# WangFeng18/3d-gaussian-splatting

Hardware: AMD Instinct MI355X
Metric: render_fps (higher is better)
Workload: dtype f32; 1 GPU; cfg5: 2400000 Gaussians, 1920x1080, no SH, forward render, one frame in flight, one view per GPU -- north-star target scene (geometry of BASELINE configs[3]/[4]); n_gaussians=2400000, visible=1887982, tile_pairs=6950364, width=1920, height=1080, parallelism=view-sharded x1 (no data-path collective), frames_in_flight=1

## Files before the change

3d-gaussian-splatting_amd/csrc/gs_frame.hip:

```cpp
#include <math.h>
#include <stdarg.h>
#include <string.h>

#include <mutex>
#include <new>

#include "gs_common.h"
#include "gs_frame_layout.h"
#include "raster_bwd_common.h"

static thread_local char g_err[512] = "";

void gs_set_error(const char *fmt, ...) {
    va_list ap;
    va_start(ap, fmt);
    vsnprintf(g_err, sizeof(g_err), fmt, ap);
    va_end(ap);
}

extern "C" const char *gs_last_error(void) { return g_err; }
extern "C" int gs_abi_version(void) { return GS_ABI_VERSION; }
extern "C" int gs_culling(void) { return 0; }

static int tile_bits(int n_tiles) {
// ... 459 lines not shown
    GS_HIP(hipStreamWaitEvent(s, a->done, 0));
    *prepared = true;
    return 0;
}

extern "C" size_t gs_frame_contrib_workspace_bytes(int64_t max_pairs) {
    return max_pairs < 0 ? 0 : gs_contrib_workspace_bytes(max_pairs);
}

extern "C" int gs_frame_contrib(const gs_frame *f, const gs_contrib_opts *opts, gs_contrib_row *rows, void *workspace,
                                size_t workspace_bytes, gs_stream_t stream) {
    int rc = validate(f);
    if (rc) return rc;
    if ((rc = refuse_device_pose(f, __func__))) return rc;
    GS_CHECK_ARG(f->training && f->image_padded, "gs_frame_contrib needs a training forward (image_padded kept)");
    GS_CHECK_ARG(opts != nullptr, "opts is null");
    GS_CHECK_ARG(opts->w_min > 0.f && opts->w_min <= 1.f, "w_min must lie in (0, 1]");
    GS_CHECK_ARG(opts->accumulate == 0 || opts->accumulate == 1, "accumulate must be 0 or 1");
    GS_CHECK_ARG(f->N == 0 || rows != nullptr, "rows is null");
    GS_CHECK_ARG(((uintptr_t)rows & 15) == 0, "rows must be 16-byte aligned");
    GS_CHECK_ARG(workspace && ((uintptr_t)workspace & 255) == 0 &&
                     workspace_bytes >= gs_frame_contrib_workspace_bytes(f->max_pairs),
                 "workspace null, not 256-byte aligned or too small");
    if (f->N == 0) return 0;
    hipStream_t s = (hipStream_t)stream;
    gs_frame_ws ws = gs_frame_carve(f->workspace, f->N, f->max_pairs, f->width, f->height, f->color_dim, 1);
    uint64_t *skeys, *okeys;
    uint32_t *sids;
    sorted_buffers(f, ws, &skeys, &sids, &okeys);
    bool prepared = false;
    if ((rc = peek_prepared(f, s, &prepared))) return rc;
    return gs_stage_contrib(f, ws, sids, prepared, opts->w_min, opts->accumulate, rows, workspace, s);
}

static int zero_image(size_t bytes, const float **out) {
    static std::mutex mu;
    static struct { void *p; size_t bytes; } cache[64] = {};
    int dev = 0;
    GS_HIP(hipGetDevice(&dev));
    GS_CHECK_ARG(dev >= 0 && dev < 64, "device index out of range");
    std::lock_guard<std::mutex> lock(mu);
    if (cache[dev].bytes < bytes) {
        if (cache[dev].p) GS_HIP(hipFree(cache[dev].p));
        cache[dev].p = nullptr;
        cache[dev].bytes = 0;
        void *q = nullptr;
        GS_HIP(hipMalloc(&q, bytes));
        GS_HIP(hipMemset(q, 0, bytes));
        GS_HIP(hipDeviceSynchronize());
        cache[dev].p = q;
        cache[dev].bytes = bytes;
    }
    *out = (const float *)cache[dev].p;
    return 0;
}

static int frame_backward_adam_impl(const char *entry, const gs_frame *f, const float *grad_image, const gs_adam_fused *adam,
                                    hipStream_t s) {
    const bool aux = (f->flags & GS_FRAME_AUX) != 0, pose = (f->flags & GS_FRAME_POSE_GRAD) != 0;
    if (!(f->training && f->image_padded)) {
        gs_set_error("%s: invalid argument: %s needs a training forward (image_padded kept)", entry, entry);
        return GS_E_INVALID;
    }
    if (!(adam && (aux || grad_image))) {
        gs_set_error("%s: invalid argument: null pointer", entry);
        return GS_E_INVALID;
    }
    int rc = gs_validate_adam_fused(f, adam);
    if (rc) return rc;
    if (f->N == 0) return pose ? zero_pose_grad(f, s) : 0;
    if (!grad_image && (rc = zero_image(sizeof(float) * 3 * (size_t)f->width * (size_t)f->height, &grad_image))) return rc;
    gs_frame_ws ws = gs_frame_carve(f->workspace, f->N, f->max_pairs, f->width, f->height, f->color_dim, 1);
    if ((rc = raster_backward(f, ws, grad_image, s))) return rc;
    if ((rc = gs_stage_project_backward_adam(f, ws, adam, s))) return rc;
    return pose ? gs_stage_pose_finalize(f, ws, s) : 0;
}

static int refuse_flag(const char *entry, const char *flag) {
    gs_set_error("%s: %s frames are not supported (use gs_frame_backward + an optimizer step)", entry, flag);
    return GS_E_UNSUPPORTED;
}

extern "C" int gs_frame_backward_adam(const gs_frame *f, const float *grad_image, const gs_adam_fused *adam,
                                      gs_stream_t stream) {
    int rc = validate(f);
    if (rc) return rc;
    if ((rc = refuse_device_pose(f, __func__))) return rc;
    if (f->flags & GS_FRAME_AUX) return refuse_flag(__func__, "GS_FRAME_AUX");
    if (f->flags & GS_FRAME_POSE_GRAD) return refuse_flag(__func__, "GS_FRAME_POSE_GRAD");
    return frame_backward_adam_impl(__func__, f, grad_image, adam, (hipStream_t)stream);
}

extern "C" int gs_frame_backward_adam_aux(const gs_frame *f, const float *grad_image, const gs_adam_fused *adam,
                                          gs_stream_t stream) {
    int rc = validate(f);
    if (rc) return rc;
    if ((rc = refuse_device_pose(f, __func__))) return rc;
    GS_CHECK_ARG((f->flags & GS_FRAME_AUX) != 0, "the frame is not flagged GS_FRAME_AUX (gs_frame_backward_adam takes plain frames)");
    if (f->flags & GS_FRAME_POSE_GRAD) return refuse_flag(__func__, "GS_FRAME_POSE_GRAD");
    return frame_backward_adam_impl(__func__, f, grad_image, adam, (hipStream_t)stream);
}

extern "C" int gs_frame_backward_adam_pose(const gs_frame *f, const float *grad_image, const gs_adam_fused *adam,
                                           gs_stream_t stream) {
    int rc = validate(f);
    if (rc) return rc;
    if ((rc = refuse_device_pose(f, __func__))) return rc;
    GS_CHECK_ARG((f->flags & GS_FRAME_POSE_GRAD) != 0,
                 "the frame is not flagged GS_FRAME_POSE_GRAD (gs_frame_backward_adam / _adam_aux take frames without a pose gradient)");
    if (f->color_dim != 3) return refuse_sh_pose(__func__);
    return frame_backward_adam_impl(__func__, f, grad_image, adam, (hipStream_t)stream);
}

extern "C" int gs_frame_backward_pose(const gs_frame *f, const float *grad_image, int32_t part, gs_stream_t stream) {
    int rc = validate(f);
    if (rc) return rc;
    GS_CHECK_ARG(f->training && f->image_padded, "gs_frame_backward_pose needs a training forward (image_padded kept)");
    GS_CHECK_ARG(part == 0 || part == GS_BWD_GEOMETRY, "part must be 0 or GS_BWD_GEOMETRY");
    GS_CHECK_ARG((f->flags & GS_FRAME_POSE_GRAD) != 0,
                 "the frame is not flagged GS_FRAME_POSE_GRAD (there is no other gradient this entry point writes)");
    if (f->color_dim != 3) return refuse_sh_pose(__func__);
    GS_CHECK_ARG(part == GS_BWD_GEOMETRY || grad_image, "null pointer");
    hipStream_t s = (hipStream_t)stream;
    if (f->N == 0) return zero_pose_grad(f, s);
    gs_frame_ws ws = gs_frame_carve(f->workspace, f->N, f->max_pairs, f->width, f->height, f->color_dim, 1);
    if (part == 0 && (rc = raster_backward(f, ws, grad_image, s))) return rc;
    if ((rc = gs_stage_pose_only_backward(f, ws, s))) return rc;
    return gs_stage_pose_finalize(f, ws, s);
}

extern "C" int gs_frame_backward_part(const gs_frame *f, const float *grad_image, float *grad_pos, float *grad_quat,
                                      float *grad_scale, float *grad_opa, float *grad_rgb, int32_t part,
                                      gs_stream_t stream) {
    GS_CHECK_ARG(part == GS_BWD_RASTER || part == GS_BWD_GEOMETRY || part == GS_BWD_COLOR,
                 "part must be GS_BWD_RASTER, GS_BWD_GEOMETRY or GS_BWD_COLOR");
    return frame_backward_impl(f, grad_image, grad_pos, grad_quat, grad_scale, grad_opa, grad_rgb, part,
                               (hipStream_t)stream, nullptr);
}

extern "C" int gs_frame_backward_slice(const gs_frame *f, float *grad_pos, float *grad_quat, float *grad_scale,
                                       float *grad_opa, float *grad_rgb, int32_t part, int64_t g_begin, int64_t g_end,
                                       gs_stream_t stream) {
    GS_CHECK_ARG(part == GS_BWD_GEOMETRY || part == GS_BWD_COLOR || part == (GS_BWD_GEOMETRY | GS_BWD_COLOR),
                 "part must be GS_BWD_GEOMETRY, GS_BWD_COLOR or both");
    int rc = validate(f);
    if (rc) return rc;
    if ((rc = refuse_device_pose(f, __func__))) return rc;
    if (f->flags & GS_FRAME_POSE_GRAD) {
        gs_set_error("gs_frame_backward_slice: GS_FRAME_POSE_GRAD frames are not supported (use gs_frame_backward or "
                     "gs_frame_backward_part)");
        return GS_E_UNSUPPORTED;
    }
    if (part == (GS_BWD_GEOMETRY | GS_BWD_COLOR)) {
        GS_CHECK_ARG(grad_pos && grad_quat && grad_scale && grad_opa && grad_rgb, "null pointer");
        return frame_backward_impl(f, nullptr, grad_pos, grad_quat, grad_scale, grad_opa, grad_rgb, -1,
                                   (hipStream_t)stream, nullptr, g_begin, g_end);
    }
    return frame_backward_impl(f, nullptr, grad_pos, grad_quat, grad_scale, grad_opa, grad_rgb, part,
                               (hipStream_t)stream, nullptr, g_begin, g_end);
}

extern "C" int gs_frame_backward_profile(const gs_frame *f, const float *grad_image, float *grad_pos,
                                         float *grad_quat, float *grad_scale, float *grad_opa, float *grad_rgb,
                                         float *stage_ms_host, gs_stream_t stream) {
    GS_CHECK_ARG(stage_ms_host != nullptr, "stage_ms_host is null");
    return frame_backward_impl(f, grad_image, grad_pos, grad_quat, grad_scale, grad_opa, grad_rgb, 0,
                               (hipStream_t)stream, stage_ms_host);
}

extern "C" int gs_frame_stats_async(const gs_frame *f, int64_t *stats_host, gs_stream_t stream) {
    int rc = validate(f);
    if (rc) return rc;
    GS_CHECK_ARG(stats_host != nullptr, "stats_host is null");
    gs_frame_ws ws = gs_frame_carve(f->workspace, f->N, f->max_pairs, f->width, f->height, f->color_dim, f->training);
    GS_HIP(hipMemcpyAsync(stats_host, ws.counters, sizeof(int64_t) * 4, hipMemcpyDeviceToHost, (hipStream_t)stream));
    return 0;
}

extern "C" int gs_frame_overflow_flag(const gs_frame *f, const void **device_counter) {
    int rc = validate(f);
    if (rc) return rc;
    GS_CHECK_ARG(device_counter != nullptr, "device_counter is null");
    gs_frame_ws ws = gs_frame_carve(f->workspace, f->N, f->max_pairs, f->width, f->height, f->color_dim, f->training);
    *device_counter = ws.counters + GS_CNT_OVERFLOW;
    return 0;
}

extern "C" int gs_frame_longest_list_async(const gs_frame *f, int64_t *longest_host, gs_stream_t stream) {
    int rc = validate(f);
    if (rc) return rc;
    GS_CHECK_ARG(longest_host != nullptr, "longest_host is null");
    gs_frame_ws ws = gs_frame_carve(f->workspace, f->N, f->max_pairs, f->width, f->height, f->color_dim, f->training);
    GS_HIP(hipMemcpyAsync(longest_host, ws.counters + GS_CNT_MAXLIST, sizeof(int64_t), hipMemcpyDeviceToHost,
                          (hipStream_t)stream));
    return 0;
}

extern "C" int gs_frame_stats_tagged_async(const gs_frame *f, uint32_t tag, int64_t *stats_host, gs_stream_t stream) {
    int rc = validate(f);
    if (rc) return rc;
    GS_CHECK_ARG(stats_host != nullptr, "stats_host is null");
    gs_frame_ws ws = gs_frame_carve(f->workspace, f->N, f->max_pairs, f->width, f->height, f->color_dim, f->training);
    GS_HIP(hipMemsetD32Async((hipDeviceptr_t)(ws.counters + GS_CNT_TAG), (int)tag, 2, (hipStream_t)stream));
    GS_HIP(hipMemcpyAsync(stats_host, ws.counters, sizeof(int64_t) * GS_STATS_TAGGED_N, hipMemcpyDeviceToHost,
                          (hipStream_t)stream));
    return 0;
}

extern "C" int gs_frame_cull_fallback_async(const gs_frame *f, int64_t *ran_past_host, gs_stream_t stream) {
    int rc = validate(f);
    if (rc) return rc;
    GS_CHECK_ARG(ran_past_host != nullptr, "ran_past_host is null");
    gs_frame_ws ws = gs_frame_carve(f->workspace, f->N, f->max_pairs, f->width, f->height, f->color_dim, f->training);
    GS_HIP(hipMemcpyAsync(ran_past_host, ws.counters + GS_CNT_RANPAST, sizeof(int64_t), hipMemcpyDeviceToHost,
                          (hipStream_t)stream));
    return 0;
}

extern "C" int gs_frame_is_occlusion_culled(const gs_frame *f, int32_t *culled) {
    GS_CHECK_ARG(f && culled, "null argument");
    *culled = (effective_sort_mode(f) == 2 && gs_frame_occlusion_cull(f)) ? 1 : 0;
    return 0;
}

extern "C" int gs_frame_cull_second_pass(const gs_frame *f, int32_t *enqueued) {
    GS_CHECK_ARG(f && enqueued, "null argument");
    if (int rc = refuse_cull_repeat(f)) return rc;
    *enqueued = cull_second_pass(f) ? 1 : 0;
    return 0;
}

extern "C" int gs_frame_reads_scene_pack(const gs_frame *f) {
    if (!f || f->training || f->N <= 0 || effective_sort_mode(f) != 2) return 0;
    return gs_frame_uses_strips(f) ? 1 : 0;
}

extern "C" int gs_frame_debug_tile_nproc(const gs_frame *f, const uint32_t **tile_nproc) {
    int rc = validate(f);
    if (rc) return rc;
    GS_CHECK_ARG(tile_nproc != nullptr, "tile_nproc is null");
    GS_CHECK_ARG(f->training, "the per-tile processed counts are kept by training forwards only");
    gs_frame_ws ws = gs_frame_carve(f->workspace, f->N, f->max_pairs, f->width, f->height, f->color_dim, 1);
    *tile_nproc = ws.tile_nproc;
    return 0;
}

extern "C" int gs_frame_debug_bwd_exec_rows(const gs_frame *f, const uint32_t **exec_rows, int32_t *n_slots) {
    int rc = validate(f);
    if (rc) return rc;
    GS_CHECK_ARG(exec_rows != nullptr && n_slots != nullptr, "null pointer");
    GS_CHECK_ARG(f->training, "the executed-row counters are kept by training frames only");
    gs_frame_ws ws = gs_frame_carve(f->workspace, f->N, f->max_pairs, f->width, f->height, f->color_dim, 1);
    *exec_rows = ws.bwd_exec_rows;
    *n_slots = gs_bwd_mfma_slots(f->color_dim, gs_frame_geometry(f).n_tiles, ws.max_buckets);
    return 0;
}

extern "C" int gs_frame_binning_variant(const gs_frame *f) {
    int rc = validate(f);
    if (rc) return rc < 0 ? rc : -rc;
    const int mode = effective_sort_mode(f);
    if (mode != 2) return mode;
    if (gs_frame_uses_strips(f)) return 4;
    return (f->flags & GS_FRAME_SLICE_SORT) ? 3 : 2;
}

extern "C" int gs_frame_debug_rects(const gs_frame *f, const uint32_t **rects) {
    int rc = validate(f);
    if (rc) return rc;
    GS_CHECK_ARG(rects != nullptr, "rects is null");
    gs_frame_ws ws = gs_frame_carve(f->workspace, f->N, f->max_pairs, f->width, f->height, f->color_dim, f->training);
    *rects = reinterpret_cast<const uint32_t *>(ws.rects);
    return 0;
}

extern "C" int gs_frame_debug_cull_stage(const gs_frame *f, const uint64_t **entries, const uint32_t **tags,
                                         const uint32_t **slice_entries, int32_t *slices, int64_t *cap) {
    int rc = validate(f);
    if (rc) return rc;
    GS_CHECK_ARG(entries && tags && slice_entries && slices && cap, "null pointer");
    GS_CHECK_ARG(effective_sort_mode(f) == 2 && gs_frame_occlusion_cull(f), "not an occlusion-culled frame");
    gs_frame_ws ws = gs_frame_carve(f->workspace, f->N, f->max_pairs, f->width, f->height, f->color_dim, f->training);
    gs_frame_geom G = gs_frame_geometry(f);
    const gs_strip_plan plan = gs_strip_plan_for(f->N, G.ntx, G.nty);
    *entries = ws.keys_b;
    *tags = ws.vals_b;
    *slice_entries = ws.slice_entries;
    *slices = (int32_t)plan.slices;
    *cap = gs_cull_stage_cap(f->max_pairs, plan.slices);
    return 0;
}

extern "C" int gs_frame_debug_cut_table(const gs_frame *f, const uint32_t **cut, int32_t *n_tiles) {
    int rc = validate(f);
    if (rc) return rc;
    GS_CHECK_ARG(cut && n_tiles, "null pointer");
    GS_CHECK_ARG(!f->training, "the cut table is written by inference forwards only");
    gs_frame_ws ws = gs_frame_carve(f->workspace, f->N, f->max_pairs, f->width, f->height, f->color_dim, f->training);
    *cut = ws.cut;
    *n_tiles = gs_frame_geometry(f).n_tiles;
    return 0;
}

extern "C" int gs_frame_debug_views(const gs_frame *f, const uint64_t **sorted_keys, const uint32_t **sorted_ids,
                                    const int32_t **tile_ranges, const float **rec_geom, const float **rec_cov,
                                    const float **rec_color, const uint32_t **tiles_touched) {
    int rc = validate(f);
    if (rc) return rc;
    if ((rc = refuse_device_pose(f, __func__))) return rc;
    gs_frame_ws ws = gs_frame_carve(f->workspace, f->N, f->max_pairs, f->width, f->height, f->color_dim, f->training);
    uint64_t *skeys, *okeys;
    uint32_t *sids;
    sorted_buffers(f, ws, &skeys, &sids, &okeys);
    if (sorted_keys)
        *sorted_keys = (effective_sort_mode(f) == 2 && !(f->flags & GS_FRAME_EMIT_SORTED_KEYS)) ? nullptr : skeys;
    if (sorted_ids) *sorted_ids = sids;
    if (tile_ranges) *tile_ranges = ws.tile_ranges;
    if (rec_geom) *rec_geom = (const float *)ws.rec_geom;
    if (rec_cov) *rec_cov = (const float *)ws.rec_cov;
    if (rec_color) *rec_color = (const float *)ws.rec_color;
    if (tiles_touched) *tiles_touched = ws.tiles_touched;
    return 0;
}

#ifdef GS_DIAG_CKPT
extern "C" __attribute__((visibility("default"))) int gs_diag_ckpt(const gs_frame *f, const float **ckpt,
                                                                   int64_t *max_buckets) {
    int rc = validate(f);
    if (rc) return rc;
    gs_frame_ws ws = gs_frame_carve(f->workspace, f->N, f->max_pairs, f->width, f->height, f->color_dim, 1);
    *ckpt = reinterpret_cast<const float *>(ws.ckpt);
    *max_buckets = ws.max_buckets;
    return 0;
}
#endif
```

3d-gaussian-splatting_amd/csrc/gs_frame_layout.h:

```cpp
#pragma once
#include "gs_common.h"

enum { GS_CNT_VISIBLE = 0, GS_CNT_PAIRS = 1, GS_CNT_OVERFLOW = 2, GS_CNT_BUCKETS = 3, GS_CNT_TICKET = 4, GS_CNT_ENTRIES = 5, GS_CNT_BIG = 6, GS_CNT_SEGS = 7, GS_CNT_GROUPS = 8, GS_CNT_MAXLIST = 9, GS_CNT_RANPAST = 10, GS_CNT_TAG = 11, GS_CNT_EXCESS = 12, GS_CNT_MAXWALK = 13, GS_CNT_EXCESS_WALK = 14, GS_CNT_N = 16 };

#define GS_BUCKET 64
#define GS_SORT_TILE 2048
#define GS_BIN_SLICES 256
#define GS_BIN_MAX_TILES 32768
#define GS_BIN_MAX_SLICES 1024
#define GS_BIN_LDS_BYTES 160000

struct gs_bin_plan {
    int lds_sort;
    uint32_t slices;
    uint32_t per_slice;
    uint32_t cap;
};
static inline gs_bin_plan gs_bin_plan_for(int64_t N, int64_t max_pairs, int n_tiles, int want_lds_sort = 1) {
    gs_bin_plan p;
    const int64_t room = (int64_t)GS_BIN_LDS_BYTES - 4 * (int64_t)n_tiles;
    p.cap = room > 0 ? (uint32_t)(room / 8 / 64 * 64) : 0;
    p.lds_sort = want_lds_sort && p.cap >= 4096;
    const int64_t n = N > 0 ? N : 1;
    int64_t S = GS_BIN_SLICES;
    if (p.lds_sort) {
        const int64_t want = gs_div_up(max_pairs > 0 ? max_pairs : 1, (int64_t)p.cap * 95 / 100);
        S = gs_div_up(want, GS_BIN_SLICES) * GS_BIN_SLICES;
        if (S > GS_BIN_MAX_SLICES) S = GS_BIN_MAX_SLICES;
    }
    const int64_t per = gs_div_up(gs_div_up(n, S), 256) * 256;
    p.per_slice = (uint32_t)per;
    p.slices = (uint32_t)gs_div_up(n, per);
    return p;
}

#ifndef GS_STRIP_W
#define GS_STRIP_W 8
#endif
#define GS_STRIP_ID_BITS 26
#define GS_STRIP_MAX 8192
#define GS_LONGEST_MIN 1024
#ifndef GS_LONG_MIN
#define GS_LONG_MIN 512
#endif
#ifndef GS_SEG_LEN
#define GS_SEG_LEN 512
#endif
static inline bool gs_frame_long_lists(const gs_frame *f, int n_tiles) {
    (void)n_tiles;
    return (f->flags & GS_FRAME_LONG_LISTS) != 0;
}
static inline size_t gs_cull_pyramid_bytes(int ntx, int nty) {
    const int nsx = (ntx + 7) / 8;
    size_t b = (size_t)nsx * 8 * nty * 4;
    int w = ntx, h = nty;
    for (int l = 1; l < 4; ++l) {
        w = (w + 1) / 2, h = (h + 1) / 2;
        b += (size_t)w * h * 4;
    }
    return b;
}
static inline uint32_t gs_cull_stage_cap(int64_t max_pairs, uint32_t slices) {
    const int64_t c = max_pairs / (int64_t)(slices ? slices : 1);
    return c < 0x7fffffff ? (uint32_t)c : 0x7fffffffu;
}
#define GS_STAGE_OVER 0xffffffffu
#define GS_NO_CUT 0xffffffffu
#define GS_CUT_MARGIN 0.0625f
#define GS_CUT_DILATE_SCALE 1.375f
#define GS_CUT_DILATE_SCALE_NEAR 1.125f
static inline bool gs_frame_occlusion_cull(const gs_frame *f);

static inline bool gs_frame_long_sort(const gs_frame *f) {
    return (f->flags & (GS_FRAME_LONG_LISTS | GS_FRAME_LONG_SORT)) != 0;
}
static inline int64_t gs_seg_items_cap(int64_t max_pairs, int n_tiles) { return max_pairs / GS_SEG_LEN + n_tiles; }
static inline int64_t gs_group_queue_cap(int64_t max_pairs, int n_tiles) { return max_pairs / 256 + 4 * (int64_t)n_tiles; }
#define GS_STRIP_SORT_CAP 2048
struct gs_strip_geom {
    uint32_t ntx, nty, nsx, NS;
};
struct gs_strip_plan {
    int ok;
    gs_strip_geom geom;
    uint32_t slices;
    uint32_t per_slice;
    uint32_t cap;
};
static inline gs_strip_plan gs_strip_plan_for(int64_t N, int ntx, int nty) {
    gs_strip_plan p;
    p.geom.ntx = (uint32_t)ntx;
    p.geom.nty = (uint32_t)nty;
    p.geom.nsx = (uint32_t)((ntx + GS_STRIP_W - 1) / GS_STRIP_W);
    p.geom.NS = p.geom.nsx * (uint32_t)nty;
    p.ok = N < (1ll << GS_STRIP_ID_BITS) && p.geom.NS <= GS_STRIP_MAX;
    const int64_t n = N > 0 ? N : 1;
    const int64_t per = gs_div_up(gs_div_up(n, GS_BIN_SLICES), 256) * 256;
    p.per_slice = (uint32_t)per;
    p.slices = (uint32_t)gs_div_up(n, per);
    p.cap = p.ok ? (uint32_t)(((int64_t)GS_BIN_LDS_BYTES - 8 * (int64_t)p.geom.NS) / 8) : 0;
    return p;
}

#ifndef GS_STRIP_AUTO_MIN_N
#define GS_STRIP_AUTO_MIN_N 131072
#endif
static inline bool gs_frame_uses_strips(const gs_frame *f) {
    if (f->sort_mode != 2 || (f->flags & (GS_FRAME_SLICE_SORT | GS_FRAME_TABLE_BIN))) return false;
    const int ntx = (f->width + GS_TILE - 1) / GS_TILE, nty = (f->height + GS_TILE - 1) / GS_TILE;
    if (!gs_strip_plan_for(f->N, ntx, nty).ok) return false;
    if (f->flags & GS_FRAME_STRIP_BIN) return true;
    if (f->flags & (GS_FRAME_LONG_LISTS | GS_FRAME_LONG_SORT)) return true;
    return f->N >= GS_STRIP_AUTO_MIN_N || ntx * nty > GS_BIN_MAX_TILES;
}

static inline bool gs_frame_occlusion_cull(const gs_frame *f) {
    if (!((f->flags & GS_FRAME_OCCLUSION_CULL) && !f->training && f->N > 0 && f->tile_culling_method != 0 &&
          !(f->flags & (GS_FRAME_EMIT_SORTED_KEYS | GS_FRAME_LONG_LISTS | GS_FRAME_SERIAL_LONG_LISTS)) &&
          gs_frame_uses_strips(f)))
        return false;
    const int ntx = (f->width + GS_TILE - 1) / GS_TILE, nty = (f->height + GS_TILE - 1) / GS_TILE;
    const int64_t ns = (int64_t)((ntx + GS_STRIP_W - 1) / GS_STRIP_W) * nty;
    const int64_t room = (int64_t)GS_BIN_LDS_BYTES - 8 * 4096;
    return 8 * ns + (int64_t)gs_cull_pyramid_bytes(ntx, nty) + 2 * 16384 + 16 <= room;
}
static inline const gs_frame_scene *gs_frame_scene_fields(const gs_frame *f) {
    return reinterpret_cast<const gs_frame_scene *>(f);
}
static inline const gs_frame_pp *gs_frame_pp_fields(const gs_frame *f) { return reinterpret_cast<const gs_frame_pp *>(f); }
static inline const float *gs_frame_pose_dev(const gs_frame *f) {
    return (f->flags & GS_FRAME_DEVICE_POSE) ? reinterpret_cast<const gs_frame_dp *>(f)->pose_dev : nullptr;
}
static inline bool gs_frame_scene_pack(const gs_frame *f) {
    return (f->flags & GS_FRAME_SCENE_PACK) && !f->training && f->N > 0 && gs_frame_uses_strips(f);
}
static inline bool gs_frame_fused_table_count(const gs_frame *f) {
    const int ntx = (f->width + GS_TILE - 1) / GS_TILE, nty = (f->height + GS_TILE - 1) / GS_TILE;
    return f->sort_mode == 2 && !gs_frame_uses_strips(f) && !(f->flags & GS_FRAME_SLICE_SORT) &&
           ntx * nty <= GS_BIN_MAX_TILES;
}

static constexpr int gs_row_floats(int color_dim) {
    return color_dim == 3 ? 16 : color_dim == 27 ? 48 : color_dim == 48 ? 64 : (7 + color_dim + 3) / 4 * 4;
}
static constexpr int gs_row_geo(int color_dim, int m) { return color_dim == 27 ? (m < 4 ? 12 + m : 28 + (m - 4)) : m; }
static constexpr int gs_row_col(int color_dim, int c) {
    return color_dim == 27 ? 16 * (c / 9) + c % 9 : color_dim == 48 ? 16 + c : 7 + c;
}
static constexpr int gs_row_aux_depth(int color_dim) { return color_dim == 3 ? 10 : color_dim == 27 ? 31 : 7; }
static constexpr int gs_row_compact(int color_dim, int f) {
    if (color_dim == 27) {
        const int line = f / 16, o = f % 16;
        if (line > 2) return -1;
        if (o < 9) return 7 + 9 * line + o;
        if (o < 12) return -1;
        return line == 0 ? o - 12 : (line == 1 && o < 15) ? 4 + (o - 12) : -1;
    }
    if (color_dim == 48) return f < 7 ? f : f < 16 ? -1 : f < 64 ? 7 + (f - 16) : -1;
    return f < 7 + color_dim ? f : -1;
}
#define GS_BWD_EXEC_SLOTS 8
#define GS_MFMA_ITEM_BUCKETS 8

struct gs_frame_geom {
    int padW, padH, ntx, nty, n_tiles, crop_top, crop_left;
    float tlx, tly, leftmost, topmost;
};

static inline gs_frame_geom gs_frame_geometry_i(int W, int H) {
    gs_frame_geom G;
    G.padW = (W + GS_TILE - 1) / GS_TILE * GS_TILE;
    G.padH = (H + GS_TILE - 1) / GS_TILE * GS_TILE;
    G.ntx = G.padW / GS_TILE;
    G.nty = G.padH / GS_TILE;
    G.n_tiles = G.ntx * G.nty;
    G.crop_top = (G.padH - H) / 2;
    G.crop_left = (G.padW - W) / 2;
    G.tlx = G.tly = G.leftmost = G.topmost = 0.f;
    return G;
}
static inline gs_frame_geom gs_frame_geometry(const gs_frame *f) {
    gs_frame_geom G = gs_frame_geometry_i(f->width, f->height);
    G.tlx = f->tile_length_x;
    G.tly = f->tile_length_y;
    G.leftmost = f->leftmost;
    G.topmost = f->topmost;
    return G;
}
inline GsDistCull gs_frame_dist_cull(const gs_frame *f) {
    const gs_frame_geom G = gs_frame_geometry(f);
    return {(float)(G.padW / 2), (float)(G.padH / 2), f->focal_x, f->focal_y, f->thresh};
}

struct gs_frame_ws {
    unsigned long long *counters;
    float4 *rec_geom;
    float4 *rec_cov;
    float4 *rec_color;
    float4 *rec_conic;
    uint32_t *tiles_touched;
    uint4 *rects;
    uint32_t *slice_entries;
    uint32_t *block_sums;
    uint32_t *block_vis;
    uint32_t *block_offsets;
    uint32_t *pair_offsets;
    uint64_t *keys_a, *keys_b;
    uint32_t *vals_a, *vals_b;
    void *sort_tmp;
    size_t sort_tmp_bytes;
    int32_t *tile_ranges;
    uint32_t *cut;
    uint32_t *cut_dilated;
    uint32_t *bin_table;
    uint32_t *tile_count;
    uint32_t *slice_pairs, *slice_vis;
    uint64_t *strip_table;
    uint64_t *strip_tot;
    uint64_t *strip_base;
    uint32_t *big_tiles;
    uint32_t *tile_cost;
    uint32_t *tile_order;
    uint4 *group_queue;
    float4 *cont_state;
    uint32_t *cont_flag;
    uint32_t *seg_item_base;
    uint2 *seg_items;
    float *seg_P;
    float4 *seg_C;
    uint32_t *seg_nproc;
    uint32_t *tile_nproc;
    uint32_t *bucket_offsets;
    uint4 *bucket_info;
    float4 *ckpt;
    float *rows;
    uint4 *mfma_items;
    uint32_t *mfma_n_items;
    uint32_t *bwd_exec_rows;
    uint64_t *stop_keys;
    int64_t max_buckets;
    size_t zero_bytes;
    size_t total_bytes;
};

static inline int64_t gs_max_buckets(int64_t max_pairs, int n_tiles) {
    return max_pairs / GS_BUCKET + n_tiles + 1;
}

static inline gs_frame_ws gs_frame_carve(void *base, int64_t N, int64_t max_pairs, int W, int H, int color_dim,
                                         int training) {
    gs_frame_ws ws;
    gs_frame_geom G = gs_frame_geometry_i(W, H);
    size_t off = 0;
    auto take = [&](size_t bytes) -> void * {
        void *p = base ? (void *)((char *)base + off) : nullptr;
        off += gs_align_up(bytes ? bytes : 1, 256);
        return p;
    };
    const int64_t nblk = gs_div_up(N > 0 ? N : 1, 256);
    ws.counters = (unsigned long long *)take(sizeof(unsigned long long) * GS_CNT_N);
    ws.tile_ranges = (int32_t *)take(sizeof(int32_t) * 2 * G.n_tiles);
    ws.zero_bytes = off;
    ws.cut = (uint32_t *)take(sizeof(uint32_t) * G.n_tiles);
    ws.cut_dilated = (uint32_t *)take(sizeof(uint32_t) * G.n_tiles);
    ws.rec_geom = (float4 *)take(sizeof(float4) * GS_REC_STRIDE * N);
    ws.rec_cov = ws.rec_geom ? ws.rec_geom + 1 : nullptr;
    ws.rec_color = ws.rec_geom ? ws.rec_geom + 2 : nullptr;
    ws.rec_conic = ws.rec_geom ? ws.rec_geom + 3 : nullptr;
    ws.tiles_touched = (uint32_t *)take(sizeof(uint32_t) * N);
    ws.rects = (uint4 *)take(sizeof(uint4) * N);
    ws.slice_entries = (uint32_t *)take(sizeof(uint32_t) * GS_BIN_MAX_SLICES);
    ws.block_sums = (uint32_t *)take(sizeof(uint32_t) * nblk);
    ws.block_vis = (uint32_t *)take(sizeof(uint32_t) * nblk);
    ws.block_offsets = (uint32_t *)take(sizeof(uint32_t) * nblk);
    ws.pair_offsets = (uint32_t *)take(sizeof(uint32_t) * N);
    ws.keys_a = (uint64_t *)take(sizeof(uint64_t) * max_pairs);
    ws.keys_b = (uint64_t *)take(sizeof(uint64_t) * max_pairs);
    ws.vals_a = (uint32_t *)take(sizeof(uint32_t) * max_pairs);
    ws.vals_b = (uint32_t *)take(sizeof(uint32_t) * max_pairs);
    ws.sort_tmp_bytes = gs_sort_pairs_tmp_bytes(max_pairs);
    ws.sort_tmp = take(ws.sort_tmp_bytes);
    {
        const gs_bin_plan plan = gs_bin_plan_for(N, max_pairs, G.n_tiles);
        const size_t rows = plan.lds_sort && plan.slices > GS_BIN_SLICES ? plan.slices : GS_BIN_SLICES;
        ws.bin_table = (uint32_t *)take(sizeof(uint32_t) * rows * ((size_t)G.n_tiles + 1));
    }
    ws.tile_count = (uint32_t *)take(sizeof(uint32_t) * G.n_tiles);
    ws.slice_pairs = (uint32_t *)take(sizeof(uint32_t) * GS_BIN_MAX_SLICES);
    ws.slice_vis = (uint32_t *)take(sizeof(uint32_t) * GS_BIN_MAX_SLICES);
    {
        const gs_strip_plan sp = gs_strip_plan_for(N, G.ntx, G.nty);
        const size_t ns = sp.ok ? sp.geom.NS : 1;
        ws.strip_table = (uint64_t *)take(sizeof(uint64_t) * 2 * GS_BIN_SLICES * ns);
        ws.strip_tot = (uint64_t *)take(sizeof(uint64_t) * ns);
        ws.strip_base = (uint64_t *)take(sizeof(uint64_t) * ns);
        ws.big_tiles = (uint32_t *)take(sizeof(uint32_t) * (sp.ok ? (size_t)G.n_tiles : 1));
        ws.tile_cost = (uint32_t *)take(sizeof(uint32_t) * (sp.ok ? (size_t)G.n_tiles : 1));
        ws.tile_order = (uint32_t *)take(sizeof(uint32_t) * (sp.ok ? (size_t)G.n_tiles : 1));
    }
    if (gs_strip_plan_for(N, G.ntx, G.nty).ok) {
        const size_t cap = (size_t)gs_seg_items_cap(max_pairs, G.n_tiles);
        ws.group_queue = (uint4 *)take(sizeof(uint4) * (size_t)gs_group_queue_cap(max_pairs, G.n_tiles));
        ws.cont_state = (float4 *)take(sizeof(float4) * 256 * (size_t)G.n_tiles);
        ws.cont_flag = (uint32_t *)take(sizeof(uint32_t) * G.n_tiles);
        ws.seg_item_base = (uint32_t *)take(sizeof(uint32_t) * ((size_t)G.n_tiles + 1));
        ws.seg_items = (uint2 *)take(sizeof(uint2) * cap);
        ws.seg_P = (float *)take(sizeof(float) * 256 * cap);
        ws.seg_C = (float4 *)take(sizeof(float4) * 256 * cap);
        ws.seg_nproc = (uint32_t *)take(sizeof(uint32_t) * cap);
    } else {
        ws.group_queue = nullptr;
        ws.cont_state = nullptr;
        ws.cont_flag = nullptr;
        ws.seg_item_base = nullptr;
        ws.seg_items = nullptr;
        ws.seg_P = nullptr;
        ws.seg_C = nullptr;
        ws.seg_nproc = nullptr;
    }
    ws.max_buckets = gs_max_buckets(max_pairs, G.n_tiles);
    if (training) {
        ws.tile_nproc = (uint32_t *)take(sizeof(uint32_t) * G.n_tiles);
        ws.bucket_offsets = (uint32_t *)take(sizeof(uint32_t) * (G.n_tiles + 1));
        ws.bucket_info = (uint4 *)take(sizeof(uint4) * (size_t)(ws.max_buckets + 8));
        ws.ckpt = (float4 *)take(sizeof(float4) * 256 * (size_t)ws.max_buckets);
        ws.rows = (float *)take(sizeof(float) * (size_t)gs_row_floats(color_dim) * max_pairs);
        ws.bwd_exec_rows = (uint32_t *)take(sizeof(uint32_t) * GS_BWD_EXEC_SLOTS * (size_t)G.n_tiles);
        ws.mfma_items = (uint4 *)take(sizeof(uint4) * (color_dim == 3 ? 1 : (size_t)(G.n_tiles + ws.max_buckets / GS_MFMA_ITEM_BUCKETS + 8)));
        ws.mfma_n_items = (uint32_t *)take(sizeof(uint32_t));
        ws.stop_keys = (uint64_t *)take(sizeof(uint64_t) * G.n_tiles);
    } else {
        ws.tile_nproc = nullptr;
        ws.bucket_offsets = nullptr;
        ws.bucket_info = nullptr;
        ws.ckpt = nullptr;
        ws.rows = nullptr;
        ws.bwd_exec_rows = nullptr;
        ws.mfma_items = nullptr;
        ws.mfma_n_items = nullptr;
        ws.stop_keys = nullptr;
    }
    ws.total_bytes = off;
    return ws;
}

struct gs_frame_aux_ws {
    float2 *ckpt;
    size_t total_bytes;
};
static inline gs_frame_aux_ws gs_frame_aux_carve(void *base, int64_t max_pairs, int W, int H, int training) {
    gs_frame_aux_ws a;
    const gs_frame_geom G = gs_frame_geometry_i(W, H);
    size_t off = 256;
    a.ckpt = nullptr;
    if (training) {
        a.ckpt = base ? (float2 *)((char *)base + off) : nullptr;
        off += gs_align_up(sizeof(float2) * 256 * (size_t)gs_max_buckets(max_pairs, G.n_tiles), 256);
    }
    a.total_bytes = off;
    return a;
}
static inline gs_frame_aux_ws gs_frame_aux(const gs_frame *f) {
    return gs_frame_aux_carve((f->flags & GS_FRAME_AUX) ? f->aux_workspace : nullptr, f->max_pairs, f->width, f->height,
                              f->training);
}

struct gs_frame_pose_ws {
    float *proj, *aux;
    int64_t rows;
    size_t total_bytes;
};
static inline gs_frame_pose_ws gs_frame_pose_carve(void *base, int64_t N) {
    gs_frame_pose_ws p;
    p.rows = gs_div_up(N > 0 ? N : 0, 256);
    p.proj = base ? (float *)((char *)base + 256) : nullptr;
    p.aux = p.proj ? p.proj + p.rows * 12 : nullptr;
    p.total_bytes = 256 + gs_align_up(sizeof(float) * 12 * 2 * (size_t)p.rows, 256);
    return p;
}

static inline const uint32_t *gs_frame_cut_table(const gs_frame *f, const gs_frame_ws &ws) {
    return (f->flags & GS_FRAME_CULL_DILATE) ? ws.cut_dilated : ws.cut;
}
int gs_stage_cut_dilate(const gs_frame *f, const gs_frame_ws &ws, hipStream_t stream);
int gs_stage_project(const gs_frame *f, const gs_frame_ws &ws, hipStream_t stream, int slice_begin = 0, int slice_end = -1,
                     bool second_pass = false);
int gs_stage_project_backward(const gs_frame *f, const gs_frame_ws &ws, float *grad_pos, float *grad_quat,
                              float *grad_scale, float *grad_opa, float *grad_rgb, int part, int64_t g_begin,
                              int64_t g_end, hipStream_t stream);
int gs_stage_project_backward_adam(const gs_frame *f, const gs_frame_ws &ws, const gs_adam_fused *a, hipStream_t stream);
int gs_validate_adam_fused(const gs_frame *f, const gs_adam_fused *a);
int gs_stage_scan_emit(const gs_frame *f, const gs_frame_ws &ws, hipStream_t stream);
int gs_stage_tile_sort(const gs_frame *f, const gs_frame_ws &ws, uint64_t *keys, uint32_t *ids, uint64_t *scratch,
                       hipStream_t stream);
int gs_stage_tile_bin(const gs_frame *f, const gs_frame_ws &ws, hipStream_t stream);
int gs_stage_strip_bin(const gs_frame *f, const gs_frame_ws &ws, hipStream_t stream, bool second_pass = false);
int gs_stage_strip_sort(const gs_frame *f, const gs_frame_ws &ws, const uint64_t *entries, uint64_t *scratch,
                        uint64_t *keys_out, uint32_t *ids_out, hipStream_t stream, bool second_pass = false);
int gs_stage_tile_sort_packed(const gs_frame *f, const gs_frame_ws &ws, uint64_t *packed, uint64_t *keys_out,
                              uint32_t *ids_out, hipStream_t stream);
int gs_stage_tile_sort_gather(const gs_frame *f, const gs_frame_ws &ws, const uint64_t *slice_pairs_buf,
                              uint64_t *big_scratch, uint64_t *keys_out, uint32_t *ids_out, hipStream_t stream);
int gs_stage_tile_ranges(const gs_frame *f, const gs_frame_ws &ws, const uint64_t *sorted_keys, hipStream_t stream);
int gs_stage_raster_forward(const gs_frame *f, const gs_frame_ws &ws, const uint32_t *sorted_ids, hipStream_t stream,
                            bool second_pass = false);
int gs_stage_backward_prepare(const gs_frame *f, const gs_frame_ws &ws, const uint32_t *sorted_ids, hipStream_t stream);
int gs_stage_sh_big_rows(const gs_frame *f, const gs_frame_ws &ws, hipStream_t stream);
int gs_stage_contrib_prepare(const gs_frame *f, const gs_frame_ws &ws, const uint32_t *sorted_ids, bool prepared,
                             unsigned long long *n_buckets_own, hipStream_t stream);
int gs_stage_contrib(const gs_frame *f, const gs_frame_ws &ws, const uint32_t *sorted_ids, bool prepared, float w_min,
                     int accumulate, gs_contrib_row *rows, void *workspace, hipStream_t stream);
size_t gs_contrib_workspace_bytes(int64_t max_pairs);
int gs_stage_aux_depth_backward(const gs_frame *f, const gs_frame_ws &ws, float *grad_pos, int64_t g_begin, int64_t g_end,
                                hipStream_t stream);
int gs_stage_project_backward_pose(const gs_frame *f, const gs_frame_ws &ws, float *grad_pos, float *grad_quat,
                                   float *grad_scale, float *grad_opa, float *grad_rgb, int part, hipStream_t stream);
int gs_stage_aux_depth_pose_backward(const gs_frame *f, const gs_frame_ws &ws, float *grad_pos, hipStream_t stream);
int gs_stage_pose_only_backward(const gs_frame *f, const gs_frame_ws &ws, hipStream_t stream);
int gs_stage_pose_finalize(const gs_frame *f, const gs_frame_ws &ws, hipStream_t stream);
int gs_stage_raster_backward(const gs_frame *f, const gs_frame_ws &ws, const uint32_t *sorted_ids,
                             const float *grad_image, hipStream_t stream, bool prepared);
```

3d-gaussian-splatting_amd/csrc/raster_fwd.hip:

```cpp
#include <stdlib.h>

#include <atomic>
#include <type_traits>

#include "raster_common.h"

namespace {

typedef float f2 __attribute__((ext_vector_type(2)));

constexpr int FWD_THREADS = 64;
constexpr int NPP = 2;
#ifndef GS_FWD_WAVES_PER_SIMD
#define GS_FWD_WAVES_PER_SIMD 8
#endif

template <int CDIM>
struct FwdSmem {
    static constexpr int CH = 64;
    static constexpr int NB = CDIM / 3;
    static constexpr int SHS = CDIM == 27 ? 28 : CDIM + 4;
    enum { X, Y, A, B, C, NLOP, DH, DL, NFIELD };
    static constexpr int NBUF = 1;
    float f[NBUF][NFIELD][CH] __attribute__((aligned(16)));
    float sh[NBUF][CH][SHS] __attribute__((aligned(16)));
};
template <>
struct FwdSmem<3> {
    static constexpr int CH = 64;
    enum { X, Y, A, B, C, NLOP, R, G, BL, DH, DL, NFIELD };
    static constexpr int NBUF = 2;
    float f[NBUF][NFIELD][CH] __attribute__((aligned(16)));
};

__device__ __forceinline__ f2 splat(float v) { return f2{v, v}; }
__device__ __forceinline__ f2 pk_fma(f2 a, f2 b, f2 c) { return __builtin_elementwise_fma(a, b, c); }

extern "C" __device__ float gs_fmul_legacy(float, float) __asm("llvm.amdgcn.fmul.legacy");
__device__ __forceinline__ float mul_legacy(float a, float b) { return gs_fmul_legacy(a, b); }

#define GS_LIVE_SCALE 1.2676506002282294e30f
__device__ __forceinline__ f2 live_mask(f2 t, f2 scale, f2 bias) {
    f2 m;
    asm("v_pk_fma_f32 %0, %1, %2, %3 clamp" : "=v"(m) : "v"(t), "v"(scale), "v"(bias));
    return m;
}

#ifndef GS_FWD_RGB_WPE
#define GS_FWD_RGB_WPE 4
#endif
#ifndef GS_FWD_SH27_WPE
#define GS_FWD_SH27_WPE 3
#endif
#ifndef GS_FWD_SH48_WPE
#define GS_FWD_SH48_WPE 2
#endif
struct AuxFwdOut {
    float2 *padded;
    float *depth;
    float *alpha;
    float2 *ckpt;
};

template <int CDIM, bool FRAME, bool CKPT, bool SIG, bool WN, bool EXACT, bool AUX>
__device__ __forceinline__ void raster_forward_body(RasterSrc S, RasterGeom G,
                                                    const int32_t *__restrict__ ranges,
                                                    float *__restrict__ out_padded,
                                                    float *__restrict__ out_image,
                                                    float4 *__restrict__ ckpt,
                                                    uint32_t *__restrict__ tile_nproc,
                                                    uint32_t n_tiles,
                                                    float4 *__restrict__ cont_state,
                                                    uint32_t *__restrict__ cont_flag,
                                                    const uint32_t *__restrict__ tile_order,
                                                    uint32_t *__restrict__ tile_cost,
                                                    const uint32_t *cut_in, uint32_t *cut_out,
                                                    unsigned long long *__restrict__ ranpast,
                                                    const unsigned long long *__restrict__ gate,
                                                    const AuxFwdOut &X) {
    static_assert(!AUX || (FRAME && !SIG && !WN && !EXACT), "depth / alpha maps belong to the frame path");
    static_assert(!(EXACT && FRAME), "the exact-exp flavour belongs to the reference API (gs_draw, fast = 0)");
    if (FRAME && gate && *gate == 0) return;
    using SM = FwdSmem<CDIM>;
    constexpr int CH = SM::CH;
#ifndef GS_FWD_GROUP
#define GS_FWD_GROUP 4
#endif
    constexpr uint32_t GROUP = CDIM == 3 ? GS_FWD_GROUP : 4;
    static_assert(GROUP == 4 || GROUP == 2, "GROUP");
#ifndef GS_FWD_LIVE_EVERY
#define GS_FWD_LIVE_EVERY 8
#endif
    constexpr uint32_t LIVE_EVERY = CDIM == 3 ? GS_FWD_LIVE_EVERY : 4;
    __shared__ SM sm;
    __shared__ float s_dep[AUX ? SM::NBUF : 1][AUX ? CH : 1] __attribute__((aligned(16)));
    const int lane = threadIdx.x;

    auto range_of = [&](uint32_t t, uint32_t &s0, uint32_t &cnt) {
        s0 = cnt = 0;
        if (t < n_tiles) {
            s0 = (uint32_t)(FRAME ? ranges[2 * t] : ranges[t]);
            cnt = (uint32_t)(FRAME ? ranges[2 * t + 1] : ranges[t + 1]) - s0;
        }
    };
    auto tile_at = [&](uint32_t li) {
        return li < n_tiles ? (tile_order ? (uint32_t)__builtin_amdgcn_readfirstlane(tile_order[li]) : li) : n_tiles;
    };
    auto next_index = [&](uint32_t li) { return li + gridDim.x; };
    uint32_t li = blockIdx.x, nli = next_index(li);
    uint32_t tile = tile_at(li), ntile = tile_at(nli), start, n, nstart, nn;
    range_of(tile, start, n);
    range_of(ntile, nstart, nn);

    GaussianRec g;
    float r0 = 0, r1 = 0, r2 = 0;
    float4 cq = make_float4(0.f, 0.f, 0.f, 0.f);
    float dz = 0.f;
    uint32_t gid = 0, gj = 0;
    bool have = false;
    auto fetch = [&](uint32_t s0, uint32_t cnt, uint32_t base) {
        have = base + lane < cnt;
        if (have) {
            gj = s0 + base + lane;
            gid = raster_load<FRAME>(S, gj, g);
            if (FRAME) cq = S.conic4[(size_t)gid * GS_REC_STRIDE];
            if constexpr (AUX) dz = S.geom[(size_t)gid * GS_REC_STRIDE].z;
            if (CDIM == 3) raster_load_rgb<FRAME>(S, gj, gid, r0, r1, r2);
        }
    };
    fetch(start, n, 0);
    int k = 0;

    for (; li < n_tiles; li = nli, nli = next_index(nli), tile = ntile, ntile = tile_at(nli), start = nstart, n = nn,
                         range_of(ntile, nstart, nn)) {
    const uint32_t tx = tile % (uint32_t)G.ntx, ty = tile / (uint32_t)G.ntx;
    const uint32_t id_x = tx * 16 + (lane & 15), id_y0 = ty * 16 + (lane >> 4);
    const float px = raster_pixel_coord(id_x, G.padW, G.focal_x);
    f2 py2[NPP];
#pragma unroll
    for (int h = 0; h < NPP; ++h)
        py2[h] = f2{raster_pixel_coord(id_y0 + 8 * h, G.padH, G.focal_y),
                    raster_pixel_coord(id_y0 + 8 * h + 4, G.padH, G.focal_y)};
    constexpr int NB = CDIM > 3 ? CDIM / 3 : 1;
    f2 SH[NPP][NB];
    if (CDIM > 3) {
#pragma unroll
        for (int h = 0; h < NPP; ++h) {
            float a9[NB], b9[NB];
            raster_pixel_sh<NB>(id_x, id_y0 + 8 * h, G, a9);
            raster_pixel_sh<NB>(id_x, id_y0 + 8 * h + 4, G, b9);
            constexpr float KS = -GS_LOG2E;
#pragma unroll
            for (int k9 = 0; k9 < NB; ++k9) SH[h][k9] = f2{KS * a9[k9], KS * b9[k9]};
        }
    }

    f2 T[NPP], cr[NPP], cg[NPP], cb[NPP], accw[NPP];
#pragma unroll
    for (int h = 0; h < NPP; ++h) {
        T[h] = f2{1.0f, 1.0f};
        cr[h] = cg[h] = cb[h] = accw[h] = f2{0.f, 0.f};
    }
    f2 cd[AUX ? NPP : 1], ca[AUX ? NPP : 1];
    if constexpr (AUX) {
#pragma unroll
        for (int h = 0; h < NPP; ++h) cd[h] = ca[h] = f2{0.f, 0.f};
    }
    f2 live_scale = splat(GS_LIVE_SCALE), live_bias = splat(-GS_T_STOP * GS_LIVE_SCALE);
    asm volatile("" : "+v"(live_scale), "+v"(live_bias));
    uint32_t nproc = 0, steps = 0;

    auto write_ckpt = [&](uint32_t idx_in_tile) {
        float4 *c = ckpt + raster_ckpt_slot(start, tile, idx_in_tile / GS_BUCKET) * 256;
#pragma unroll
        for (int h = 0; h < NPP; ++h) {
            c[128 * h + lane] = make_float4(T[h].x, cr[h].x, cg[h].x, cb[h].x);
            c[128 * h + 64 + lane] = make_float4(T[h].y, cr[h].y, cg[h].y, cb[h].y);
        }
        if constexpr (AUX) {
            float2 *a = X.ckpt + raster_ckpt_slot(start, tile, idx_in_tile / GS_BUCKET) * 256;
#pragma unroll
            for (int h = 0; h < NPP; ++h) {
                a[128 * h + lane] = make_float2(cd[h].x, ca[h].x);
                a[128 * h + 64 + lane] = make_float2(cd[h].y, ca[h].y);
            }
        }
    };
    auto any_live = [&]() {
        f2 sum = T[0];
#pragma unroll
        for (int h = 1; h < NPP; ++h) sum += T[h];
        return __ballot(sum.x + sum.y > 0.0f) != 0ull;
    };

    bool done = false, staged_next = false;
    bool continues = false;
    for (uint32_t base = 0; base < n && !done; base += CH, ++k) {
        if (FRAME && cont_flag && base == (uint32_t)GS_LONG_MIN) {
            if (any_live()) {
                float4 *c = cont_state + (size_t)tile * 256;
#pragma unroll
                for (int h = 0; h < NPP; ++h) {
                    c[128 * h + lane] = make_float4(T[h].x, cr[h].x, cg[h].x, cb[h].x);
                    c[128 * h + 64 + lane] = make_float4(T[h].y, cr[h].y, cg[h].y, cb[h].y);
                }
                continues = true;
            }
            if (continues) break;
        }
        const int buf = k & (SM::NBUF - 1);
        bool suspicious = false;
        if (have) {
            float A, B, C;
            if (FRAME) {
                A = cq.x;
                B = cq.y;
                C = cq.z;
            } else {
                raster_conic(g, A, B, C);
            }
            {
                const float chk = ((g.x + g.y) + (A + B + C)) + ((r0 + r1 + r2) + g.opa);
                suspicious = !(fabsf(chk) < 3.0e38f) || !(A >= 0.f && A < 1.0e8f) || !(C >= 0.f && C < 1.0e8f) ||
                             !(4.f * A * C >= B * B) ||
                             !FRAME || CDIM != 3;
            }
            float opa = g.opa;
            if (SIG)
                opa *= 1.5707963268f * rsqrtf(raster_det(g.a, g.b, g.c, g.d) + 1e-7f);
            sm.f[buf][SM::X][lane] = g.x;
            sm.f[buf][SM::Y][lane] = g.y;
            if constexpr (EXACT) {
                const double den = (double)(2.0f * raster_det(g.a, g.b, g.c, g.d)) + 1e-14;
                const float dh = (float)den;
                sm.f[buf][SM::A][lane] = g.a;
                sm.f[buf][SM::B][lane] = g.b + g.c;
                sm.f[buf][SM::C][lane] = g.d;
                sm.f[buf][SM::DH][lane] = dh;
                sm.f[buf][SM::DL][lane] = (float)(den - (double)dh);
            } else {
                sm.f[buf][SM::A][lane] = A;
                sm.f[buf][SM::B][lane] = B;
                sm.f[buf][SM::C][lane] = C;
            }
            sm.f[buf][SM::NLOP][lane] = FRAME ? -__log2f(opa) : opa;
            if constexpr (AUX) s_dep[buf][lane] = dz;
            if constexpr (CDIM == 3) {
                if (r0 != r0 || r1 != r1 || r2 != r2) {
                    sm.f[buf][SM::NLOP][lane] = __builtin_nanf("");
                    r0 = r1 = r2 = 0.f;
                }
                sm.f[buf][SM::R][lane] = r0;
                sm.f[buf][SM::G][lane] = r1;
                sm.f[buf][SM::BL][lane] = r2;
            } else {
                const float *src = raster_sh_ptr<FRAME, CDIM>(S, gj, gid);
#pragma unroll
                for (int q = 0; q < CDIM; ++q) sm.sh[buf][lane][q] = src[q];
            }
        } else if (base + lane < ((n + (GROUP - 1u)) & ~(GROUP - 1u))) {
#pragma unroll
            for (int q = 0; q < SM::NFIELD; ++q)
                sm.f[buf][q][lane] = (FRAME && q == SM::NLOP) ? 1e30f : (EXACT && q == SM::DH) ? 1.0f : 0.f;
            if constexpr (AUX) s_dep[buf][lane] = 0.f;
            if constexpr (CDIM > 3) {
#pragma unroll
                for (int q = 0; q < CDIM; ++q) sm.sh[buf][lane][q] = 0.f;
            }
        }
        __builtin_amdgcn_fence(__ATOMIC_ACQ_REL, "wavefront");
        __builtin_amdgcn_wave_barrier();
        staged_next = base + CH >= n;
        if (staged_next)
            fetch(nstart, nn, 0);
        else
            fetch(start, n, base + CH);
        const uint32_t cnt = (n - base) < (uint32_t)CH ? (n - base) : (uint32_t)CH;
        if (CKPT && base > 0) write_ckpt(base);
        const bool chunk_legacy = __ballot(suspicious) != 0ull;
        auto composite_chunk = [&](auto legacy_tag) {
        constexpr bool LEGACY = decltype(legacy_tag)::value;
        uint32_t stop = cnt;
#pragma unroll 1
        for (uint32_t i = 0; i < cnt; i += GROUP) {
            if ((i & (LIVE_EVERY - 1)) == 0 && !any_live()) {
                done = true;
                stop = i;
                break;
            }
            {
            constexpr uint32_t i4 = 0;
            struct Vg {
                float v[GROUP];
            };
            auto ld4 = [&](int q) {
                Vg r;
                if constexpr (GROUP == 4) {
                    const float4 t = *(const float4 *)__builtin_assume_aligned(&sm.f[buf][q][i + i4], 16);
                    r.v[0] = t.x; r.v[1] = t.y; r.v[2] = t.z; r.v[3] = t.w;
                } else {
                    const float2 t = *(const float2 *)__builtin_assume_aligned(&sm.f[buf][q][i + i4], 8);
                    r.v[0] = t.x; r.v[1] = t.y;
                }
                return r;
            };
            const Vg X = ld4(SM::X), Y = ld4(SM::Y), A4 = ld4(SM::A), B4 = ld4(SM::B), C4 = ld4(SM::C);
            const Vg O4 = ld4(SM::NLOP);
            Vg DH4 = {}, DL4 = {};
            if constexpr (EXACT) {
                DH4 = ld4(SM::DH);
                DL4 = ld4(SM::DL);
            }
            Vg R4 = {}, G4 = {}, L4 = {}, D4 = {};
            if constexpr (AUX) {
                static_assert(GROUP == 4, "AUX: the depths are read four at a time");
                const float4 t = *(const float4 *)__builtin_assume_aligned(&s_dep[buf][i + i4], 16);
                D4.v[0] = t.x; D4.v[1] = t.y; D4.v[2] = t.z; D4.v[3] = t.w;
            }
            if constexpr (CDIM == 3) {
                R4 = ld4(SM::R);
                G4 = ld4(SM::G);
                L4 = ld4(SM::BL);
            }
#pragma unroll
            for (int u = 0; u < (int)GROUP; ++u) {
                const float gx = X.v[u], gy = Y.v[u], cA = A4.v[u], cB = B4.v[u], cC = C4.v[u], nlop = O4.v[u];
                const float dx = px - gx;
                const float bdx = cB * dx;
                const float f = FRAME ? fmaf(cA * dx, dx, nlop) : cA * dx * dx;
#pragma unroll
                for (int h = 0; h < NPP; ++h) {
                    const f2 dy = py2[h] - splat(gy);
                    f2 al;
                    if constexpr (EXACT) {
                        const double den = (double)DH4.v[u] + (double)DL4.v[u];
                        auto exact_alpha = [&](float y) {
                            const float t1 = __fmul_rn(__fmul_rn(cC, dx), dx);
                            const float t2 = __fmul_rn(__fmul_rn(cB, dx), y);
                            const float t3 = __fmul_rn(__fmul_rn(cA, y), y);
                            const float num = -__fadd_rn(__fsub_rn(t1, t2), t3);
                            return (float)exp((double)num / den);
                        };
                        al.x = exact_alpha(dy.x);
                        al.y = exact_alpha(dy.y);
                    } else {
                        const f2 q = pk_fma(pk_fma(splat(cC), dy, splat(-bdx)), dy, splat(f));
                        al.x = gs_exp2(-q.x);
                        al.y = gs_exp2(-q.y);
                    }
                    if (!FRAME) al = al * splat(nlop);
                    if (SIG) {
                        al.x = gs_squash_alpha(al.x);
                        al.y = gs_squash_alpha(al.y);
                    }
                    f2 w;
                    if constexpr (LEGACY && FRAME && CDIM == 3) {
                        al.x = T[h].x == 0.f ? 0.f : al.x;
                        al.y = T[h].y == 0.f ? 0.f : al.y;
                        w = al * T[h];
                    } else if constexpr (LEGACY)
                        w = f2{mul_legacy(al.x, T[h].x), mul_legacy(al.y, T[h].y)};
                    else
                        w = al * T[h];
                    if constexpr (CDIM == 3) {
                        cr[h] = pk_fma(splat(R4.v[u]), w, cr[h]);
                        cg[h] = pk_fma(splat(G4.v[u]), w, cg[h]);
                        cb[h] = pk_fma(splat(L4.v[u]), w, cb[h]);
                    } else {
                        const float *co = sm.sh[buf][i + i4 + u];
                        f2 v0 = {0.f, 0.f}, v1 = {0.f, 0.f}, v2 = {0.f, 0.f};
#pragma unroll
                        for (int k9 = 0; k9 < NB; ++k9) {
                            v0 = pk_fma(SH[h][k9], splat(co[k9]), v0);
                            v1 = pk_fma(SH[h][k9], splat(co[NB + k9]), v1);
                            v2 = pk_fma(SH[h][k9], splat(co[2 * NB + k9]), v2);
                        }
                        auto sg = [](float v) { return gs_rcp(1.0f + gs_exp2(v)); };
                        const f2 c0 = {sg(v0.x), sg(v0.y)}, c1 = {sg(v1.x), sg(v1.y)}, c2 = {sg(v2.x), sg(v2.y)};
                        cr[h] = pk_fma(w, c0, cr[h]);
                        cg[h] = pk_fma(w, c1, cg[h]);
                        cb[h] = pk_fma(w, c2, cb[h]);
                    }
                    if (WN) accw[h] += w;
                    if constexpr (AUX) {
                        cd[h] = pk_fma(splat(D4.v[u]), w, cd[h]);
                        f2 wr = w;
                        asm("" : "+v"(wr));
                        ca[h] += wr;
                    }
                    const f2 t = T[h] - w;
                    T[h] = t * live_mask(t, live_scale, live_bias);
                }
            }
            }
        }
        return stop;
        };
        steps = base + (chunk_legacy ? composite_chunk(std::true_type{}) : composite_chunk(std::false_type{}));
        nproc = base + cnt;
    }
    if (!staged_next) fetch(nstart, nn, 0);
    if (FRAME && !CKPT && cut_out) {
        const bool sat = !continues && steps > 0 && (done || !any_live());
        if (lane == 0) {
            uint32_t c = GS_NO_CUT, dlast = GS_NO_CUT;
            if (sat) {
                const uint32_t last = S.ids[start + steps - 1];
                const float zl = S.geom[(size_t)last * GS_REC_STRIDE].z;
                dlast = __float_as_uint(zl);
                c = __float_as_uint(zl * (1.0f + GS_CUT_MARGIN));
            }
            if (cut_in) {
                const uint32_t ci = cut_in[tile];
                if (ci != GS_NO_CUT && dlast > ci) *ranpast = 1ull;
            }
            cut_out[tile] = c;
        }
    }
    if (tile_nproc && lane == 0) tile_nproc[tile] = nproc;
    if (FRAME && tile_cost && lane == 0) tile_cost[tile] = steps;
    if (FRAME && ranpast && lane == 0 && steps > (uint32_t)GS_LONG_MIN) {
        atomicAdd(ranpast + (GS_CNT_EXCESS_WALK - GS_CNT_RANPAST), (unsigned long long)(steps - (uint32_t)GS_LONG_MIN));
        if (steps > (uint32_t)GS_LONGEST_MIN) atomicMax(ranpast + (GS_CNT_MAXWALK - GS_CNT_RANPAST), (unsigned long long)steps);
    }
    if (FRAME && cont_flag && lane == 0) cont_flag[tile] = continues ? 1u : 0u;

#pragma unroll
    for (int h = 0; h < NPP; ++h)
#pragma unroll
        for (int e = 0; e < 2; ++e) {
            const uint32_t id_y = id_y0 + 8 * h + 4 * e;
            float aw = e ? accw[h].y : accw[h].x;
            if (!WN || aw < 0.01f) aw = 1.0f;
            const float o0 = (e ? cr[h].y : cr[h].x) / aw, o1 = (e ? cg[h].y : cg[h].x) / aw,
                        o2 = (e ? cb[h].y : cb[h].x) / aw;
            if constexpr (AUX) {
                const float dv = e ? cd[h].y : cd[h].x, av = e ? ca[h].y : ca[h].x;
                if (X.padded) X.padded[(size_t)id_y * G.padW + id_x] = make_float2(dv, av);
                const int ox = (int)id_x - G.crop_left, oy = (int)id_y - G.crop_top;
                if (ox >= 0 && ox < G.width && oy >= 0 && oy < G.height) {
                    if (X.depth) X.depth[(size_t)oy * G.width + ox] = dv;
                    if (X.alpha) X.alpha[(size_t)oy * G.width + ox] = av;
                }
            }
            if (out_padded) {
                float *o = out_padded + ((size_t)id_y * G.padW + id_x) * 3;
                o[0] = o0;
                o[1] = o1;
                o[2] = o2;
            }
            if (out_image) {
                const int ox = (int)id_x - G.crop_left, oy = (int)id_y - G.crop_top;
                if (ox >= 0 && ox < G.width && oy >= 0 && oy < G.height) {
                    float *o = out_image + ((size_t)oy * G.width + ox) * 3;
                    o[0] = o0 > 1.f ? 1.f : (o0 < 0.f ? 0.f : o0);
                    o[1] = o1 > 1.f ? 1.f : (o1 < 0.f ? 0.f : o1);
                    o[2] = o2 > 1.f ? 1.f : (o2 < 0.f ? 0.f : o2);
                }
            }
        }
    }
}

template <int CDIM, bool FRAME, bool CKPT, bool SIG, bool WN, bool EXACT = false>
__global__ void __launch_bounds__(FWD_THREADS)
__attribute__((amdgpu_waves_per_eu(CDIM == 48 ? GS_FWD_SH48_WPE : CDIM == 27 ? GS_FWD_SH27_WPE
                                               : (SIG || WN || EXACT) ? 1 : GS_FWD_RGB_WPE)))
raster_forward_kernel(RasterSrc S, RasterGeom G, const int32_t *__restrict__ ranges, float *__restrict__ out_padded,
                      float *__restrict__ out_image, float4 *__restrict__ ckpt, uint32_t *__restrict__ tile_nproc,
                      uint32_t n_tiles, float4 *__restrict__ cont_state, uint32_t *__restrict__ cont_flag,
                      const uint32_t *__restrict__ tile_order, uint32_t *__restrict__ tile_cost, const uint32_t *cut_in,
                      uint32_t *cut_out, unsigned long long *__restrict__ ranpast,
                      const unsigned long long *__restrict__ gate) {
    raster_forward_body<CDIM, FRAME, CKPT, SIG, WN, EXACT, false>(S, G, ranges, out_padded, out_image, ckpt, tile_nproc,
                                                                  n_tiles, cont_state, cont_flag, tile_order, tile_cost,
                                                                  cut_in, cut_out, ranpast, gate, AuxFwdOut{});
}

#ifndef GS_FWD_AUX_RGB_WPE
#define GS_FWD_AUX_RGB_WPE 3
#endif
#ifndef GS_FWD_AUX_SH27_WPE
#define GS_FWD_AUX_SH27_WPE GS_FWD_SH27_WPE
#endif
template <int CDIM, bool CKPT>
__global__ void __launch_bounds__(FWD_THREADS)
__attribute__((amdgpu_waves_per_eu(CDIM == 48 ? GS_FWD_SH48_WPE : CDIM == 27 ? GS_FWD_AUX_SH27_WPE : GS_FWD_AUX_RGB_WPE)))
raster_aux_forward_kernel(RasterSrc S, RasterGeom G, const int32_t *__restrict__ ranges, float *__restrict__ out_padded,
                          float *__restrict__ out_image, float4 *__restrict__ ckpt, uint32_t *__restrict__ tile_nproc,
                          uint32_t n_tiles, const uint32_t *__restrict__ tile_order, uint32_t *__restrict__ tile_cost,
                          const uint32_t *cut_in, uint32_t *cut_out, unsigned long long *__restrict__ ranpast,
                          const unsigned long long *__restrict__ gate, AuxFwdOut X) {
    raster_forward_body<CDIM, true, CKPT, false, false, false, true>(S, G, ranges, out_padded, out_image, ckpt, tile_nproc,
                                                                     n_tiles, nullptr, nullptr, tile_order, tile_cost,
                                                                     cut_in, cut_out, ranpast, gate, X);
}

__global__ void __launch_bounds__(1024) seg_scan_kernel(const uint32_t *__restrict__ cont_flag,
                                                        const int32_t *__restrict__ ranges, uint32_t n_tiles,
                                                        uint32_t items_cap, uint32_t *__restrict__ item_base,
                                                        uint2 *__restrict__ items,
                                                        unsigned long long *__restrict__ n_items) {
    __shared__ uint32_t s_wave[16];
    __shared__ uint32_t s_carry;
    if (threadIdx.x == 0) s_carry = 0;
    __syncthreads();
    const int lane = threadIdx.x & 63, wave = threadIdx.x >> 6;
    for (uint32_t base = 0; base < n_tiles; base += 1024) {
        const uint32_t t = base + threadIdx.x;
        uint32_t ns = 0;
        if (t < n_tiles && cont_flag[t]) {
            const uint32_t n = (uint32_t)(ranges[2 * t + 1] - ranges[2 * t]);
            ns = (n - GS_LONG_MIN + GS_SEG_LEN - 1) / GS_SEG_LEN;
        }
        const uint32_t incl = gs_wave_incl_scan_u32(ns);
        if (lane == 63) s_wave[wave] = incl;
        __syncthreads();
        uint32_t off = s_carry, tot = 0;
#pragma unroll
        for (int w = 0; w < 16; ++w) {
            off += w < wave ? s_wave[w] : 0;
            tot += s_wave[w];
        }
        const uint32_t first = off + incl - ns;
        if (t < n_tiles) {
            item_base[t] = first;
            for (uint32_t q = 0; q < ns && first + q < items_cap; ++q) items[first + q] = make_uint2(t, q);
        }
        __syncthreads();
        if (threadIdx.x == 0) s_carry += tot;
        __syncthreads();
    }
    if (threadIdx.x == 0) {
        item_base[n_tiles] = s_carry;
        *n_items = s_carry < items_cap ? s_carry : items_cap;
    }
}

template <int CDIM, bool CKPT, int PHASE>
__global__ void __launch_bounds__(FWD_THREADS) raster_segment_kernel(
    RasterSrc S, RasterGeom G, const int32_t *__restrict__ ranges, const uint2 *__restrict__ items,
    const unsigned long long *__restrict__ n_items, const float4 *__restrict__ cont_state, float *__restrict__ seg_P,
    float4 *__restrict__ seg_C, uint32_t *__restrict__ seg_nproc, float4 *__restrict__ ckpt) {
    using SM = FwdSmem<CDIM>;
    constexpr int CH = SM::CH;
    constexpr int NB = CDIM > 3 ? CDIM / 3 : 1;
    __shared__ SM sm;
    const int lane = threadIdx.x;
    const uint32_t item = blockIdx.x;
    if (item >= (uint32_t)*n_items) return;
    const uint2 it = items[item];
    const uint32_t tile = it.x, seg = it.y;
    const uint32_t start = (uint32_t)ranges[2 * tile], n_all = (uint32_t)ranges[2 * tile + 1] - start;
    const uint32_t seg_begin = GS_LONG_MIN + seg * GS_SEG_LEN;
    const uint32_t n = n_all - seg_begin < (uint32_t)GS_SEG_LEN ? n_all - seg_begin : (uint32_t)GS_SEG_LEN;
    const uint32_t tx = tile % (uint32_t)G.ntx, ty = tile / (uint32_t)G.ntx;
    const uint32_t id_x = tx * 16 + (lane & 15), id_y0 = ty * 16 + (lane >> 4);
    const float px = raster_pixel_coord(id_x, G.padW, G.focal_x);
    f2 py2[NPP], SH[NPP][NB];
#pragma unroll
    for (int h = 0; h < NPP; ++h) {
        py2[h] = f2{raster_pixel_coord(id_y0 + 8 * h, G.padH, G.focal_y),
                    raster_pixel_coord(id_y0 + 8 * h + 4, G.padH, G.focal_y)};
        if (CDIM > 3 && PHASE == 2) {
            float a9[NB], b9[NB];
            raster_pixel_sh<NB>(id_x, id_y0 + 8 * h, G, a9);
            raster_pixel_sh<NB>(id_x, id_y0 + 8 * h + 4, G, b9);
            constexpr float KS = -GS_LOG2E;
#pragma unroll
            for (int k9 = 0; k9 < NB; ++k9) SH[h][k9] = f2{KS * a9[k9], KS * b9[k9]};
        }
    }
    f2 T[NPP], cr[NPP], cg[NPP], cb[NPP];
#pragma unroll
    for (int h = 0; h < NPP; ++h) {
        T[h] = f2{1.0f, 1.0f};
        cr[h] = cg[h] = cb[h] = f2{0.f, 0.f};
    }
    if (PHASE == 2) {
        const float4 *c0 = cont_state + (size_t)tile * 256;
        const float *Pp = seg_P + (size_t)(item - seg) * 256;
#pragma unroll
        for (int h = 0; h < NPP; ++h) {
            float t0 = c0[128 * h + lane].x, t1 = c0[128 * h + 64 + lane].x;
            for (uint32_t q = 0; q < seg; ++q) {
                t0 *= Pp[(size_t)q * 256 + 128 * h + lane];
                t1 *= Pp[(size_t)q * 256 + 128 * h + 64 + lane];
            }
            T[h] = f2{t0 > GS_T_STOP ? t0 : 0.f, t1 > GS_T_STOP ? t1 : 0.f};
        }
    }
    auto any_live = [&]() {
        f2 sum = T[0];
#pragma unroll
        for (int h = 1; h < NPP; ++h) sum += T[h];
        return __ballot(sum.x + sum.y > 0.0f) != 0ull;
    };
    f2 live_scale = splat(GS_LIVE_SCALE), live_bias = splat(-GS_T_STOP * GS_LIVE_SCALE);
    asm volatile("" : "+v"(live_scale), "+v"(live_bias));
    uint32_t nproc = 0;
    bool done = PHASE == 2 && !any_live();
    for (uint32_t base = 0; base < n && !done; base += CH) {
        {
            const bool have = base + lane < n;
            __builtin_amdgcn_fence(__ATOMIC_ACQ_REL, "wavefront");
            __builtin_amdgcn_wave_barrier();
            if (have) {
                GaussianRec g;
                const uint32_t gj = start + seg_begin + base + lane;
                const uint32_t gid = raster_load<true>(S, gj, g);
                const float4 cq = S.conic4[(size_t)gid * GS_REC_STRIDE];
                sm.f[0][SM::X][lane] = g.x;
                sm.f[0][SM::Y][lane] = g.y;
                sm.f[0][SM::A][lane] = cq.x;
                sm.f[0][SM::B][lane] = cq.y;
                sm.f[0][SM::C][lane] = cq.z;
                sm.f[0][SM::NLOP][lane] = -__log2f(g.opa);
                if constexpr (CDIM == 3) {
                    float r0, r1, r2;
                    raster_load_rgb<true>(S, gj, gid, r0, r1, r2);
                    if (r0 != r0 || r1 != r1 || r2 != r2) {
                        sm.f[0][SM::NLOP][lane] = __builtin_nanf("");
                        r0 = r1 = r2 = 0.f;
                    }
                    sm.f[0][SM::R][lane] = r0;
                    sm.f[0][SM::G][lane] = r1;
                    sm.f[0][SM::BL][lane] = r2;
                } else if (PHASE == 2) {
                    const float *src = raster_sh_ptr<true, CDIM>(S, gj, gid);
#pragma unroll
                    for (int q = 0; q < CDIM; ++q) sm.sh[0][lane][q] = src[q];
                }
            }
            __builtin_amdgcn_fence(__ATOMIC_ACQ_REL, "wavefront");
            __builtin_amdgcn_wave_barrier();
        }
        const uint32_t cnt = (n - base) < (uint32_t)CH ? (n - base) : (uint32_t)CH;
        if (PHASE == 2 && CKPT) {
            float4 *c = ckpt + raster_ckpt_slot(start, tile, (seg_begin + base) / GS_BUCKET) * 256;
#pragma unroll
            for (int h = 0; h < NPP; ++h) {
                c[128 * h + lane] = make_float4(T[h].x, cr[h].x, cg[h].x, cb[h].x);
                c[128 * h + 64 + lane] = make_float4(T[h].y, cr[h].y, cg[h].y, cb[h].y);
            }
        }
#pragma unroll 1
        for (uint32_t i = 0; i < cnt; ++i) {
            if (PHASE == 2 && (i & 7) == 0 && !any_live()) {
                done = true;
                break;
            }
            const float gx = sm.f[0][SM::X][i], gy = sm.f[0][SM::Y][i], cA = sm.f[0][SM::A][i], cB = sm.f[0][SM::B][i];
            const float cC = sm.f[0][SM::C][i], nlop = sm.f[0][SM::NLOP][i];
            const float dx = px - gx;
            const float bdx = cB * dx;
            const float f = fmaf(cA * dx, dx, nlop);
#pragma unroll
            for (int h = 0; h < NPP; ++h) {
                const f2 dy = py2[h] - splat(gy);
                const f2 q = pk_fma(pk_fma(splat(cC), dy, splat(-bdx)), dy, splat(f));
                const f2 al = {gs_exp2(-q.x), gs_exp2(-q.y)};
                const f2 w = {mul_legacy(al.x, T[h].x), mul_legacy(al.y, T[h].y)};
                if (PHASE == 2) {
                    if constexpr (CDIM == 3) {
                        cr[h] = pk_fma(splat(sm.f[0][SM::R][i]), w, cr[h]);
                        cg[h] = pk_fma(splat(sm.f[0][SM::G][i]), w, cg[h]);
                        cb[h] = pk_fma(splat(sm.f[0][SM::BL][i]), w, cb[h]);
                    } else {
                        const float *co = sm.sh[0][i];
                        f2 v0 = {0.f, 0.f}, v1 = {0.f, 0.f}, v2 = {0.f, 0.f};
#pragma unroll
                        for (int k9 = 0; k9 < NB; ++k9) {
                            v0 = pk_fma(SH[h][k9], splat(co[k9]), v0);
                            v1 = pk_fma(SH[h][k9], splat(co[NB + k9]), v1);
                            v2 = pk_fma(SH[h][k9], splat(co[2 * NB + k9]), v2);
                        }
                        auto sg = [](float v) { return gs_rcp(1.0f + gs_exp2(v)); };
                        const f2 c0 = {sg(v0.x), sg(v0.y)}, c1 = {sg(v1.x), sg(v1.y)}, c2 = {sg(v2.x), sg(v2.y)};
                        cr[h] = pk_fma(w, c0, cr[h]);
                        cg[h] = pk_fma(w, c1, cg[h]);
                        cb[h] = pk_fma(w, c2, cb[h]);
                    }
                }
                const f2 t = T[h] - w;
                T[h] = PHASE == 2 ? t * live_mask(t, live_scale, live_bias) : t;
            }
        }
        nproc = base + cnt;
    }
    if (PHASE == 1) {
        float *P = seg_P + (size_t)item * 256;
#pragma unroll
        for (int h = 0; h < NPP; ++h) {
            P[128 * h + lane] = T[h].x;
            P[128 * h + 64 + lane] = T[h].y;
        }
    } else {
        float4 *C = seg_C + (size_t)item * 256;
#pragma unroll
        for (int h = 0; h < NPP; ++h) {
            C[128 * h + lane] = make_float4(T[h].x, cr[h].x, cg[h].x, cb[h].x);
            C[128 * h + 64 + lane] = make_float4(T[h].y, cr[h].y, cg[h].y, cb[h].y);
        }
        if (lane == 0) seg_nproc[item] = nproc;
    }
}

template <bool CKPT>
__global__ void __launch_bounds__(256) seg_combine_kernel(RasterGeom G, const int32_t *__restrict__ ranges,
                                                          const uint32_t *__restrict__ cont_flag,
                                                          const uint32_t *__restrict__ item_base,
                                                          const float4 *__restrict__ cont_state,
                                                          const float4 *__restrict__ seg_C,
                                                          const uint32_t *__restrict__ seg_nproc,
                                                          float4 *__restrict__ ckpt, uint32_t *__restrict__ tile_nproc,
                                                          float *__restrict__ out_padded, float *__restrict__ out_image) {
    constexpr uint32_t SEGS_PER_BLOCK = 8;
    const uint32_t tile = blockIdx.x;
    if (!cont_flag[tile]) return;
    const uint32_t i0 = item_base[tile], i1 = item_base[tile + 1];
    const uint32_t nseg = i1 - i0;
    if (blockIdx.y > 0 && (!CKPT || blockIdx.y * SEGS_PER_BLOCK >= nseg)) return;
    const uint32_t p = threadIdx.x, lane = p & 63, k = p >> 6;
    const uint32_t start = (uint32_t)ranges[2 * tile], n_all = (uint32_t)ranges[2 * tile + 1] - start;
    const float4 s0 = cont_state[(size_t)tile * 256 + p];
    float c0 = s0.y, c1 = s0.z, c2 = s0.w;
    uint32_t nproc = GS_LONG_MIN;
    for (uint32_t sidx = 0; sidx < nseg; ++sidx) {
        const uint32_t it = i0 + sidx;
        const uint32_t np = seg_nproc[it];
        if (np == 0) break;
        const uint32_t seg_begin = GS_LONG_MIN + sidx * GS_SEG_LEN;
        if (CKPT && (sidx / SEGS_PER_BLOCK) % gridDim.y == blockIdx.y) {
            for (uint32_t b = 0; b * GS_BUCKET < np; ++b) {
                float4 *c = ckpt + raster_ckpt_slot(start, tile, seg_begin / GS_BUCKET + b) * 256 + p;
                float4 v = *c;
                v.y += c0;
                v.z += c1;
                v.w += c2;
                *c = v;
            }
        }
        const float4 sc = seg_C[(size_t)it * 256 + p];
        c0 += sc.y;
        c1 += sc.z;
        c2 += sc.w;
        nproc += np;
        const uint32_t seg_len = n_all - seg_begin < (uint32_t)GS_SEG_LEN ? n_all - seg_begin : (uint32_t)GS_SEG_LEN;
        if (np < seg_len) break;
    }
    if (blockIdx.y > 0) return;
    if (tile_nproc && p == 0) tile_nproc[tile] = nproc;
    const uint32_t tx = tile % (uint32_t)G.ntx, ty = tile / (uint32_t)G.ntx;
    const uint32_t id_x = tx * 16 + (lane & 15), id_y2 = ty * 16 + (lane >> 4) + 8 * (k >> 1) + 4 * (k & 1);
    if (out_padded) {
        float *o = out_padded + ((size_t)id_y2 * G.padW + id_x) * 3;
        o[0] = c0;
        o[1] = c1;
        o[2] = c2;
    }
    if (out_image) {
        const int ox = (int)id_x - G.crop_left, oy = (int)id_y2 - G.crop_top;
        if (ox >= 0 && ox < G.width && oy >= 0 && oy < G.height) {
            float *o = out_image + ((size_t)oy * G.width + ox) * 3;
            o[0] = c0 > 1.f ? 1.f : (c0 < 0.f ? 0.f : c0);
            o[1] = c1 > 1.f ? 1.f : (c1 < 0.f ? 0.f : c1);
            o[2] = c2 > 1.f ? 1.f : (c2 < 0.f ? 0.f : c2);
        }
    }
}

struct FwdPlan {
    int slots;
    int order;
};
static const FwdPlan &fwd_plan() {
    static const FwdPlan plan = [] {
        FwdPlan p;
        hipDeviceProp_t prop;
        int dev = 0, wps = GS_FWD_WAVES_PER_SIMD, cus = 256;
        if (const char *e = getenv("GS_FWD_WAVES_PER_SIMD")) wps = atoi(e) > 0 ? atoi(e) : wps;
        if (hipGetDevice(&dev) == hipSuccess && hipGetDeviceProperties(&prop, dev) == hipSuccess)
            cus = prop.multiProcessorCount;
        p.slots = cus * 4 * wps;
        const char *o = getenv("GS_FWD_ORDER");
        p.order = o ? atoi(o) != 0 : 1;
        return p;
    }();
    return plan;
}
static uint32_t fwd_grid(uint32_t n_tiles) {
    const FwdPlan &p = fwd_plan();
    const uint32_t rounds = (n_tiles + p.slots - 1) / p.slots;
    return rounds ? (n_tiles + rounds - 1) / rounds : 1;
}

template <int CDIM, bool FRAME, bool CKPT, bool SIG, bool EXACT = false>
void launch_fwd(const RasterSrc &S, const RasterGeom &G, const int32_t *ranges, float *out_padded, float *out_image,
                float4 *ckpt, uint32_t *tile_nproc, int wn, hipStream_t stream, float4 *cont_state = nullptr,
                uint32_t *cont_flag = nullptr, const uint32_t *tile_order = nullptr, uint32_t *tile_cost = nullptr,
                const uint32_t *cut_in = nullptr, uint32_t *cut_out = nullptr, unsigned long long *ranpast = nullptr,
                const unsigned long long *gate = nullptr) {
    if (!fwd_plan().order) tile_order = nullptr;
    const uint32_t T = (uint32_t)(G.ntx * G.nty);
    const uint32_t grid = gate ? (T < 1024u ? T : 1024u) : fwd_grid(T);
    if (wn)
        hipLaunchKernelGGL((raster_forward_kernel<CDIM, FRAME, CKPT, SIG, true, EXACT>), dim3(grid), dim3(FWD_THREADS),
                           0, stream, S, G, ranges, out_padded, out_image, ckpt, tile_nproc, T, cont_state, cont_flag,
                           tile_order, tile_cost, cut_in, cut_out, ranpast, gate);
    else
        hipLaunchKernelGGL((raster_forward_kernel<CDIM, FRAME, CKPT, SIG, false, EXACT>), dim3(grid), dim3(FWD_THREADS),
                           0, stream, S, G, ranges, out_padded, out_image, ckpt, tile_nproc, T, cont_state, cont_flag,
                           tile_order, tile_cost, cut_in, cut_out, ranpast, gate);
}

}

template <int CDIM, bool CKPT>
static void fwd_ref_dispatch(const RasterSrc &S, const RasterGeom &G, const int32_t *accum, float *res, int sigmoid,
                             int weight_normalize, int exact, float4 *ckpt, uint32_t *tile_nproc, hipStream_t stream) {
    if (sigmoid) {
        if (exact)
            launch_fwd<CDIM, false, CKPT, true, true>(S, G, accum, res, nullptr, ckpt, tile_nproc, weight_normalize, stream);
        else
            launch_fwd<CDIM, false, CKPT, true, false>(S, G, accum, res, nullptr, ckpt, tile_nproc, weight_normalize, stream);
    } else {
        if (exact)
            launch_fwd<CDIM, false, CKPT, false, true>(S, G, accum, res, nullptr, ckpt, tile_nproc, weight_normalize, stream);
        else
            launch_fwd<CDIM, false, CKPT, false, false>(S, G, accum, res, nullptr, ckpt, tile_nproc, weight_normalize, stream);
    }
}
int gs_raster_forward_ref(const RasterSrc &S, const RasterGeom &G, const int32_t *accum, float *res, int use_sh,
                          int sigmoid, int weight_normalize, float4 *ckpt, uint32_t *tile_nproc,
                          hipStream_t stream, int exact) {
    if (ckpt) {
        if (use_sh)
            fwd_ref_dispatch<27, true>(S, G, accum, res, sigmoid, weight_normalize, exact, ckpt, tile_nproc, stream);
        else
            fwd_ref_dispatch<3, true>(S, G, accum, res, sigmoid, weight_normalize, exact, ckpt, tile_nproc, stream);
    } else {
        if (use_sh)
            fwd_ref_dispatch<27, false>(S, G, accum, res, sigmoid, weight_normalize, exact, nullptr, nullptr, stream);
        else
            fwd_ref_dispatch<3, false>(S, G, accum, res, sigmoid, weight_normalize, exact, nullptr, nullptr, stream);
    }
    return 0;
}

int gs_ref_raster_args(const char *entry, const float *pos, const float *rgb, const float *opa, const float *cov, int32_t h,
                       int32_t w, float focal_x, float focal_y, int use_sh_coeff, const float *rays_o,
                       const float *lefttop_pos, const float *vec_dx, const float *vec_dy, RasterSrc &S, RasterGeom &G) {
    S = {};
    S.pos = pos;
    S.rgb = rgb;
    S.opa = opa;
    S.cov = cov;
    G = {};
    G.padW = w;
    G.padH = h;
    G.ntx = w / 16;
    G.nty = h / 16;
    G.focal_x = focal_x;
    G.focal_y = focal_y;
    if (use_sh_coeff) {
        if (!(rays_o && lefttop_pos && vec_dx && vec_dy)) {
            gs_set_error("%s: invalid argument: %s", entry, "SH needs the ray basis");
            return GS_E_INVALID;
        }
        G.dev_rays_o = rays_o;
        G.dev_lefttop = lefttop_pos;
        G.dev_vdx = vec_dx;
        G.dev_vdy = vec_dy;
    }
    return 0;
}

extern "C" int gs_draw(const float *pos, const float *rgb, const float *opa, const float *cov,
                       const int32_t *tile_n_point_accum, float *res, int32_t h, int32_t w, int64_t M,
                       float focal_x, float focal_y, int weight_normalize, int sigmoid, int fast,
                       const float *rays_o, const float *lefttop_pos, const float *vec_dx, const float *vec_dy,
                       int use_sh_coeff, gs_stream_t stream) {
    GS_CHECK_ARG(h > 0 && w > 0 && (h % 16) == 0 && (w % 16) == 0, "h, w must be positive multiples of 16");
    GS_CHECK_ARG(M >= 0, "M < 0");
    GS_CHECK_ARG(tile_n_point_accum && res, "null pointer");
    GS_CHECK_ARG(M == 0 || (pos && rgb && opa && cov), "null pointer");
    GS_CHECK_ARG(((uintptr_t)cov & 15) == 0, "cov must be 16-byte aligned");
    RasterSrc S;
    RasterGeom G;
    int rc = gs_ref_raster_args(__func__, pos, rgb, opa, cov, h, w, focal_x, focal_y, use_sh_coeff, rays_o, lefttop_pos, vec_dx,
                                vec_dy, S, G);
    if (rc) return rc;
    rc = gs_raster_forward_ref(S, G, tile_n_point_accum, res, use_sh_coeff, sigmoid, weight_normalize, nullptr, nullptr,
                               (hipStream_t)stream, fast ? 0 : 1);
    if (rc) {
        gs_set_error("gs_draw: unsupported flag combination");
        return rc;
    }
    GS_CHECK_LAUNCH();
    return 0;
}

int gs_stage_raster_forward(const gs_frame *f, const gs_frame_ws &ws, const uint32_t *sorted_ids,
                            hipStream_t stream, bool second_pass) {
    gs_frame_geom FG = gs_frame_geometry(f);
    RasterSrc S;
    RasterGeom G;
    gs_frame_raster_args(f, ws, sorted_ids, S, G);
    const bool aux = (f->flags & GS_FRAME_AUX) != 0;
    const bool dense = gs_frame_long_lists(f, FG.n_tiles) && ws.cont_state != nullptr &&
                       !(f->flags & GS_FRAME_SERIAL_LONG_LISTS) && !aux;
    float4 *cs = dense ? ws.cont_state : nullptr;
    uint32_t *cf = dense ? ws.cont_flag : nullptr;
    const bool ordered = gs_frame_uses_strips(f) && f->N > 0 && ws.tile_order != nullptr;
    const uint32_t *order = ordered ? ws.tile_order : nullptr;
    uint32_t *cost = ordered ? ws.tile_cost : nullptr;
    const bool culled = gs_frame_occlusion_cull(f);
    const uint32_t *cut_in = culled && !second_pass ? gs_frame_cut_table(f, ws) : nullptr;
    unsigned long long *ranpast = ws.counters + GS_CNT_RANPAST;
    const unsigned long long *gate = second_pass ? ranpast : nullptr;
    if (aux) {
        if (!fwd_plan().order) order = nullptr;
        const uint32_t T = (uint32_t)FG.n_tiles;
        const uint32_t grid = gate ? (T < 1024u ? T : 1024u) : fwd_grid(T);
        const gs_frame_aux_ws aw = gs_frame_aux(f);
        AuxFwdOut X = {(float2 *)f->aux_padded, f->depth, f->alpha, aw.ckpt};
        gs_for_color_dim(f->color_dim, [&](auto cd) {
            constexpr int CD = decltype(cd)::value;
            if (f->training)
                hipLaunchKernelGGL((raster_aux_forward_kernel<CD, true>), dim3(grid), dim3(FWD_THREADS), 0, stream, S, G,
                                   ws.tile_ranges, f->image_padded, f->image, ws.ckpt, ws.tile_nproc, T, order, cost, nullptr,
                                   nullptr, ranpast, nullptr, X);
            else
                hipLaunchKernelGGL((raster_aux_forward_kernel<CD, false>), dim3(grid), dim3(FWD_THREADS), 0, stream, S, G,
                                   ws.tile_ranges, f->image_padded, f->image, nullptr, nullptr, T, order, cost, cut_in, ws.cut,
                                   ranpast, gate, X);
        });
    } else {
        gs_for_color_dim(f->color_dim, [&](auto cd) {
            constexpr int CD = decltype(cd)::value;
            if (f->training)
                launch_fwd<CD, true, true, false>(S, G, ws.tile_ranges, f->image_padded, f->image, ws.ckpt, ws.tile_nproc, 0,
                                                  stream, cs, cf, order, cost, nullptr, nullptr, ranpast, nullptr);
            else
                launch_fwd<CD, true, false, false>(S, G, ws.tile_ranges, f->image_padded, f->image, nullptr, nullptr, 0, stream,
                                                   cs, cf, order, cost, cut_in, ws.cut, ranpast, gate);
        });
    }
    GS_CHECK_LAUNCH();
    if (dense) {
        const uint32_t T = (uint32_t)FG.n_tiles, cap = (uint32_t)gs_seg_items_cap(f->max_pairs, FG.n_tiles);
        unsigned long long *n_items = ws.counters + GS_CNT_SEGS;
        hipLaunchKernelGGL(seg_scan_kernel, dim3(1), dim3(1024), 0, stream, ws.cont_flag, ws.tile_ranges, T, cap,
                           ws.seg_item_base, ws.seg_items, n_items);
        GS_CHECK_LAUNCH();
        gs_for_color_dim(f->color_dim, [&](auto cd) {
            constexpr int CD = decltype(cd)::value;
            auto launch = [&](auto ck) {
                constexpr bool CK = decltype(ck)::value;
                hipLaunchKernelGGL((raster_segment_kernel<CD, CK, 1>), dim3(cap), dim3(FWD_THREADS), 0, stream, S, G,
                                   ws.tile_ranges, ws.seg_items, n_items, ws.cont_state, ws.seg_P, ws.seg_C, ws.seg_nproc, ws.ckpt);
                hipLaunchKernelGGL((raster_segment_kernel<CD, CK, 2>), dim3(cap), dim3(FWD_THREADS), 0, stream, S, G,
                                   ws.tile_ranges, ws.seg_items, n_items, ws.cont_state, ws.seg_P, ws.seg_C, ws.seg_nproc, ws.ckpt);
                hipLaunchKernelGGL((seg_combine_kernel<CK>), dim3(T, CK ? 16 : 1), dim3(256), 0, stream, G, ws.tile_ranges,
                                   ws.cont_flag, ws.seg_item_base, ws.cont_state, ws.seg_C, ws.seg_nproc, ws.ckpt, ws.tile_nproc,
                                   f->image_padded, f->image);
            };
            if (f->training)
                launch(std::true_type{});
            else
                launch(std::false_type{});
        });
    }
    GS_CHECK_LAUNCH();
    return 0;
}
```

3d-gaussian-splatting_amd/gaussian/_lib.py:

```python
from __future__ import annotations

import ctypes as C
import os

_HERE = os.path.dirname(os.path.abspath(__file__))
LIB_PATH = os.environ.get("GS_AMD_LIB") or os.path.join(os.path.dirname(_HERE), "csrc", "libgs_amd.so")

if not os.path.exists(LIB_PATH):
    raise ImportError(
        f"libgs_amd.so not found at {LIB_PATH}: build it with `python __graft_entry__.py` "
        "(hipcc --offload-arch=gfx950).  There is no CPU fallback for the rasterizer.")

lib = C.CDLL(LIB_PATH)

vp, i64, i32, f32, ci, sz = C.c_void_p, C.c_int64, C.c_int32, C.c_float, C.c_int, C.c_size_t


class GsFrame(C.Structure):

    _fields_ = [
        ("N", i64), ("color_dim", i32), ("scale_activation", i32),
        ("pos", vp), ("quat", vp), ("scale", vp), ("opa", vp), ("rgb", vp),
        ("rot", f32 * 9), ("tran", f32 * 3),
        ("near_plane", f32), ("half_width", f32), ("half_height", f32),
        ("width", i32), ("height", i32),
        ("focal_x", f32), ("focal_y", f32),
        ("tile_length_x", f32), ("tile_length_y", f32), ("leftmost", f32), ("topmost", f32),
        ("thresh", f32),
        ("rays_o", f32 * 3), ("lefttop", f32 * 3), ("vec_dx", f32 * 3), ("vec_dy", f32 * 3),
        ("max_pairs", i64), ("workspace", vp), ("workspace_bytes", sz),
        ("image", vp), ("image_padded", vp),
        ("training", i32), ("sort_mode", i32), ("tile_culling_method", i32),
        ("async_", vp), ("flags", i32),
        ("depth", vp), ("alpha", vp), ("aux_padded", vp), ("aux_workspace", vp), ("aux_workspace_bytes", sz),
        ("grad_depth", vp), ("grad_alpha", vp),
        ("grad_rot", vp), ("grad_tran", vp), ("pose_workspace", vp), ("pose_workspace_bytes", sz),
    ]


class GsFrameScene(GsFrame):

    _fields_ = [("scene_pack_a", vp), ("scene_pack_b", vp), ("scene_pack_a_bytes", sz), ("scene_pack_b_bytes", sz)]


class GsFramePP(GsFrameScene):

    _fields_ = [("pp_dx", C.c_double), ("pp_dy", C.c_double)]


class GsFrameDP(GsFramePP):

    _fields_ = [("pose_dev", vp)]


GS_FRAME_EMIT_SORTED_KEYS = 1
GS_FRAME_SLICE_SORT = 2
GS_FRAME_TABLE_BIN = 4
GS_FRAME_SERIAL_LONG_LISTS = 8
GS_FRAME_LONG_LISTS = 16
GS_FRAME_STRIP_BIN = 32
GS_FRAME_BWD_ROWS = 64
GS_FRAME_LONG_SORT = 128
GS_FRAME_OCCLUSION_CULL = 256
GS_FRAME_CULL_DILATE = 512
GS_FRAME_CULL_DILATE_NEAR = 1024
GS_FRAME_AUX = 2048
GS_FRAME_POSE_GRAD = 4096
GS_FRAME_SCENE_PACK = 8192
GS_FRAME_PRINCIPAL_POINT = 16384
GS_FRAME_DEVICE_POSE = 32768
GS_FRAME_CULL_REPEAT = 65536


def _sig(name, restype, *argtypes):
    fn = getattr(lib, name)
    fn.restype = restype
    fn.argtypes = list(argtypes)
    return fn


gs_last_error = _sig("gs_last_error", C.c_char_p)
gs_abi_version = _sig("gs_abi_version", ci)
gs_culling = _sig("gs_culling", ci)
gs_world2camera = _sig("gs_world2camera", ci, vp, vp, vp, vp, i64, vp)
gs_world2camera_backward = _sig("gs_world2camera_backward", ci, vp, vp, vp, i64, vp)
gs_jacobian = _sig("gs_jacobian", ci, vp, vp, i64, vp)
gs_global_culling = _sig("gs_global_culling", ci, vp, vp, vp, vp, vp, i64, f32, f32, f32, vp, vp, vp, vp)
gs_global_culling_backward = _sig("gs_global_culling_backward", ci, vp, vp, vp, vp, vp, i64, vp, vp, vp, vp, vp,
                                  vp, vp)
gs_calc_tile_list = _sig("gs_calc_tile_list", ci, vp, vp, i64, vp, vp, vp, vp, vp, vp, i64, f32, ci, f32, f32,
                         i32, i32, f32, f32, vp)
gs_gather_gaussians = _sig("gs_gather_gaussians", ci, vp, vp, vp, vp, i64, i64, i64, vp)
gs_draw = _sig("gs_draw", ci, vp, vp, vp, vp, vp, vp, i32, i32, i64, f32, f32, ci, ci, ci, vp, vp, vp, vp, ci, vp)
gs_draw_backward_workspace_bytes = _sig("gs_draw_backward_workspace_bytes", sz, i64, i32, i32)
gs_draw_backward = _sig("gs_draw_backward", ci, vp, vp, vp, vp, vp, vp, vp, vp, vp, vp, vp, i32, i32, i64, f32, f32,
                        ci, ci, ci, vp, vp, vp, vp, ci, vp, sz, vp)
gs_sort_pairs_tmp_bytes = _sig("gs_sort_pairs_tmp_bytes", sz, i64)
gs_sort_pairs = _sig("gs_sort_pairs", ci, vp, vp, vp, vp, vp, i64, ci, vp, sz, C.POINTER(ci), vp)
gs_sort_pairs_bits = _sig("gs_sort_pairs_bits", ci, vp, vp, vp, vp, vp, i64, ci, ci, vp, sz, C.POINTER(ci), vp)
gs_frame_workspace_bytes = _sig("gs_frame_workspace_bytes", sz, i64, i64, i32, i32, i32, i32)
gs_frame_aux_workspace_bytes = _sig("gs_frame_aux_workspace_bytes", sz, i64, i32, i32, i32)
gs_frame_pose_workspace_bytes = _sig("gs_frame_pose_workspace_bytes", sz, i64)
gs_scene_pack_bytes = _sig("gs_scene_pack_bytes", sz, i64, C.POINTER(sz), C.POINTER(sz))
gs_scene_pack_build = _sig("gs_scene_pack_build", ci, vp, vp, vp, vp, vp, i64, i32, i32, vp, vp, vp)
gs_frame_reads_scene_pack = _sig("gs_frame_reads_scene_pack", ci, C.POINTER(GsFrame))
gs_frame_forward = _sig("gs_frame_forward", ci, C.POINTER(GsFrame), vp)
gs_frame_backward = _sig("gs_frame_backward", ci, C.POINTER(GsFrame), vp, vp, vp, vp, vp, vp, vp)
gs_frame_backward_part = _sig("gs_frame_backward_part", ci, C.POINTER(GsFrame), vp, vp, vp, vp, vp, vp, i32, vp)
GS_BWD_RASTER, GS_BWD_GEOMETRY, GS_BWD_COLOR = 1, 2, 4
gs_frame_backward_slice = _sig("gs_frame_backward_slice", ci, C.POINTER(GsFrame), vp, vp, vp, vp, vp, i32, i64, i64, vp)
gs_frame_project_slices = _sig("gs_frame_project_slices", ci, C.POINTER(GsFrame), C.POINTER(i32), C.POINTER(i64))
gs_frame_forward_project = _sig("gs_frame_forward_project", ci, C.POINTER(GsFrame), i32, i32, vp)
gs_frame_forward_rest = _sig("gs_frame_forward_rest", ci, C.POINTER(GsFrame), vp)
gs_frame_forward_profile = _sig("gs_frame_forward_profile", ci, C.POINTER(GsFrame), C.POINTER(f32), vp)
gs_frame_backward_profile = _sig("gs_frame_backward_profile", ci, C.POINTER(GsFrame), vp, vp, vp, vp, vp, vp,
                                 C.POINTER(f32), vp)
gs_frame_stats_async = _sig("gs_frame_stats_async", ci, C.POINTER(GsFrame), vp, vp)
gs_frame_longest_list_async = _sig("gs_frame_longest_list_async", ci, C.POINTER(GsFrame), vp, vp)
gs_frame_stats_tagged_async = _sig("gs_frame_stats_tagged_async", ci, C.POINTER(GsFrame), C.c_uint32, vp, vp)
gs_frame_cull_fallback_async = _sig("gs_frame_cull_fallback_async", ci, C.POINTER(GsFrame), vp, vp)
gs_frame_is_occlusion_culled = _sig("gs_frame_is_occlusion_culled", ci, C.POINTER(GsFrame), C.POINTER(C.c_int32))
gs_frame_cull_second_pass = _sig("gs_frame_cull_second_pass", ci, C.POINTER(GsFrame), C.POINTER(C.c_int32))
gs_frame_debug_cut_table = _sig("gs_frame_debug_cut_table", ci, C.POINTER(GsFrame), C.POINTER(vp), C.POINTER(C.c_int32))
GS_STATS_TAGGED_N = 15
gs_frame_debug_views = _sig("gs_frame_debug_views", ci, C.POINTER(GsFrame), C.POINTER(vp), C.POINTER(vp),
                            C.POINTER(vp), C.POINTER(vp), C.POINTER(vp), C.POINTER(vp), C.POINTER(vp))

gs_frame_binning_variant = _sig("gs_frame_binning_variant", ci, C.POINTER(GsFrame))
gs_frame_debug_rects = _sig("gs_frame_debug_rects", ci, C.POINTER(GsFrame), C.POINTER(vp))
gs_frame_debug_cull_stage = _sig("gs_frame_debug_cull_stage", ci, C.POINTER(GsFrame), C.POINTER(vp), C.POINTER(vp), C.POINTER(vp),
                                 C.POINTER(i32), C.POINTER(i64))
class GsAdamFused(C.Structure):

    _fields_ = [("exp_avg", vp * 5), ("exp_avg_sq", vp * 5), ("lr", C.c_float * 5),
                ("beta1", C.c_float), ("beta2", C.c_float), ("eps", C.c_float), ("step", i64),
                ("grad_stat", vp), ("stat_mode", i32), ("skip_if_nonzero", vp)]


gs_frame_backward_adam = _sig("gs_frame_backward_adam", ci, C.POINTER(GsFrame), vp, C.POINTER(GsAdamFused), vp)
gs_frame_backward_adam_aux = _sig("gs_frame_backward_adam_aux", ci, C.POINTER(GsFrame), vp, C.POINTER(GsAdamFused), vp)
gs_frame_backward_adam_pose = _sig("gs_frame_backward_adam_pose", ci, C.POINTER(GsFrame), vp, C.POINTER(GsAdamFused), vp)
gs_frame_backward_pose = _sig("gs_frame_backward_pose", ci, C.POINTER(GsFrame), vp, i32, vp)
gs_frame_debug_tile_nproc = _sig("gs_frame_debug_tile_nproc", ci, C.POINTER(GsFrame), C.POINTER(vp))
gs_frame_debug_bwd_exec_rows = _sig("gs_frame_debug_bwd_exec_rows", ci, C.POINTER(GsFrame), C.POINTER(vp), C.POINTER(C.c_int32))

gs_adam_step = _sig("gs_adam_step", ci, vp, vp, vp, vp, i64, i32, C.POINTER(i64), C.POINTER(f32), f32, f32, f32, i64,
                    vp, i64, i64, i32, vp)
gs_adam_step_range = _sig("gs_adam_step_range", ci, vp, vp, vp, vp, i64, i64, i64, i32, C.POINTER(i64), C.POINTER(f32),
                          f32, f32, f32, i64, vp, i64, i64, i32, vp)
gs_adam_step_sharded = _sig("gs_adam_step_sharded", ci, vp, vp, vp, vp, i64, i64, i64, i64, i32, C.POINTER(i64),
                            C.POINTER(f32), f32, f32, f32, i64, vp, i64, i64, i32, vp, vp)
gs_adam_step_multi = _sig("gs_adam_step_multi", ci, vp, vp, vp, vp, i64, i32, C.POINTER(i64), C.POINTER(i64),
                          C.POINTER(i64), i32, C.POINTER(i64), C.POINTER(f32), f32, f32, f32, i64, vp, i64, i64, i32, vp,
                          f32, vp)
gs_frame_overflow_flag = _sig("gs_frame_overflow_flag", ci, C.POINTER(GsFrame), C.POINTER(vp))
gs_grad_stat_update = _sig("gs_grad_stat_update", ci, vp, vp, i64, i32, vp)
gs_frame_async_create = _sig("gs_frame_async_create", ci, C.POINTER(vp))
gs_frame_async_wait = _sig("gs_frame_async_wait", ci, vp, vp)
gs_frame_async_destroy = _sig("gs_frame_async_destroy", ci, vp)
gs_loss_workspace_bytes = _sig("gs_loss_workspace_bytes", sz, i32, i32)
gs_loss_l1_ssim = _sig("gs_loss_l1_ssim", ci, vp, vp, i32, i32, f32, vp, vp, vp, sz, vp)
gs_loss_depth_workspace_bytes = _sig("gs_loss_depth_workspace_bytes", sz, i32, i32)
gs_loss_depth = _sig("gs_loss_depth", ci, vp, vp, vp, i32, i32, i32, f32, f32, vp, vp, vp, vp, sz, vp)
gs_loss_track_workspace_bytes = _sig("gs_loss_track_workspace_bytes", sz, i32, i32)
gs_loss_track = _sig("gs_loss_track", ci, vp, vp, vp, vp, vp, i32, i32, f32, f32, f32, f32, f32, vp, vp, vp, vp, vp, sz, vp)
gs_loss_track_gated_workspace_bytes = _sig("gs_loss_track_gated_workspace_bytes", sz, i32, i32)
gs_loss_track_gated = _sig("gs_loss_track_gated", ci, vp, vp, vp, vp, vp, i32, i32, f32, f32, f32, f32, f32, f32, f32, i32, f32,
                           vp, vp, vp, vp, vp, vp, vp, sz, vp)
gs_track_gate_mask_workspace_bytes = _sig("gs_track_gate_mask_workspace_bytes", sz, i32, i32)
gs_track_gate_mask = _sig("gs_track_gate_mask", ci, vp, vp, vp, vp, vp, i32, i32, f32, f32, f32, f32, f32, i32, vp, vp, vp, vp,
                          vp, vp, sz, vp)
gs_loss_l1_ssim_weighted = _sig("gs_loss_l1_ssim_weighted", ci, vp, vp, vp, i32, i32, f32, C.c_double, C.c_double, vp, vp, vp,
                                sz, vp)


class GsDensifyOpts(C.Structure):

    _fields_ = [("taus", f32), ("delete_thresh", f32), ("grad_thresh", f32), ("clone_dt", f32),
                ("scale_activation", i32), ("grad_aggregation", i32), ("use_clone", i32), ("use_split", i32),
                ("color_dim", i32)]


gs_densify_workspace_bytes = _sig("gs_densify_workspace_bytes", sz, i64)
gs_densify_classify = _sig("gs_densify_classify", ci, vp, vp, vp, i64, C.POINTER(GsDensifyOpts), vp, vp, sz, vp)
gs_densify_apply = _sig("gs_densify_apply", ci, vp, vp, vp, vp, vp, vp, i64, C.POINTER(GsDensifyOpts), vp, vp, i64,
                        vp, vp, vp, vp, vp, i64, vp, vp, sz, vp)


class GsSeedOpts(C.Structure):

    _fields_ = [("stride", i32), ("alpha_thresh", f32), ("front_rel", f32), ("scale_factor", f32), ("opa_init", f32),
                ("scale_activation", i32), ("color_dim", i32)]


class GsSeedCamera(C.Structure):

    _fields_ = [("rot", f32 * 9), ("tran", f32 * 3), ("focal_x", f32), ("focal_y", f32), ("width", i32), ("height", i32)]


class GsSeedCameraPP(C.Structure):

    _fields_ = [("cam", GsSeedCamera), ("pp_dx", f32), ("pp_dy", f32)]


gs_seed_workspace_bytes = _sig("gs_seed_workspace_bytes", sz, i32, i32)
gs_seed_classify = _sig("gs_seed_classify", ci, vp, vp, vp, i32, i32, C.POINTER(GsSeedOpts), vp, vp, sz, vp)
gs_seed_apply = _sig("gs_seed_apply", ci, vp, vp, C.POINTER(GsSeedCamera), C.POINTER(GsSeedOpts), vp, vp, vp, vp, vp, i64,
                     i64, vp, vp, sz, vp)
gs_seed_apply_pp = _sig("gs_seed_apply_pp", ci, vp, vp, C.POINTER(GsSeedCameraPP), C.POINTER(GsSeedOpts), vp, vp, vp, vp, vp,
                        i64, i64, vp, vp, sz, vp)

GS_OVERLAP_MAX_VIEWS = 256


class GsOverlapOpts(C.Structure):

    _fields_ = [("stride", i32), ("near", f32), ("border", i32)]


gs_view_overlap_workspace_bytes = _sig("gs_view_overlap_workspace_bytes", sz, i32, i32, i32, i32)
gs_view_overlap_check_view = _sig("gs_view_overlap_check_view", ci, C.POINTER(GsSeedCamera), i32)
gs_view_overlap = _sig("gs_view_overlap", ci, vp, C.POINTER(GsSeedCamera), vp, i32, C.POINTER(GsOverlapOpts), vp, vp, sz, vp)
gs_view_overlap_pp = _sig("gs_view_overlap_pp", ci, vp, C.POINTER(GsSeedCameraPP), vp, vp, i32, C.POINTER(GsOverlapOpts), vp,
                          vp, sz, vp)

GS_REDUNDANCY_BINS = 8
gs_view_redundancy_workspace_bytes = _sig("gs_view_redundancy_workspace_bytes", sz, i32, i32, i32)
gs_view_redundancy = _sig("gs_view_redundancy", ci, vp, C.POINTER(GsSeedCamera), vp, i32, i32, C.POINTER(GsOverlapOpts), vp, vp,
                          sz, vp)
gs_view_redundancy_pp = _sig("gs_view_redundancy_pp", ci, vp, C.POINTER(GsSeedCameraPP), vp, vp, i32, i32,
                             C.POINTER(GsOverlapOpts), vp, vp, sz, vp)

GS_PRUNE_MAX_ARRAYS = 16


class GsPruneOpts(C.Structure):

    _fields_ = [("opa_logit_min", f32), ("scale_max", f32), ("scale_activation", i32)]


class GsPruneArrays(C.Structure):

    _fields_ = [("n", i32), ("width", i32 * GS_PRUNE_MAX_ARRAYS), ("src", vp * GS_PRUNE_MAX_ARRAYS),
                ("dst", vp * GS_PRUNE_MAX_ARRAYS)]


gs_prune_workspace_bytes = _sig("gs_prune_workspace_bytes", sz, i64)
gs_prune_classify = _sig("gs_prune_classify", ci, vp, vp, i64, C.POINTER(GsPruneOpts), vp, vp, sz, vp)
gs_prune_apply = _sig("gs_prune_apply", ci, C.POINTER(GsPruneArrays), i64, i64, i64, vp, vp, sz, vp)
gs_densify_apply_state = _sig("gs_densify_apply_state", ci, C.POINTER(GsPruneArrays), i64, i64, vp, vp, sz, vp)


class GsContribOpts(C.Structure):

    _fields_ = [("w_min", f32), ("accumulate", i32)]


class GsPruneContribOpts(C.Structure):

    _fields_ = [("weight_max_min", f32), ("pixels_min", C.c_uint32), ("views_min", C.c_uint32)]


gs_frame_contrib_workspace_bytes = _sig("gs_frame_contrib_workspace_bytes", sz, i64)
gs_frame_contrib = _sig("gs_frame_contrib", ci, C.POINTER(GsFrame), C.POINTER(GsContribOpts), vp, vp, sz, vp)
gs_prune_classify_contrib = _sig("gs_prune_classify_contrib", ci, vp, vp, vp, i64, C.POINTER(GsPruneOpts),
                                 C.POINTER(GsPruneContribOpts), vp, vp, sz, vp)

GS_PYRAMID_MAX_LEVELS = 4


class GsPyramidOpts(C.Structure):

    _fields_ = [("min_valid", i32), ("edge_rel", f32)]


gs_pyramid_down = _sig("gs_pyramid_down", ci, vp, vp, i32, i32, C.POINTER(GsPyramidOpts), vp, vp, vp)

GS_ICP_LOG_DOUBLES = 40
GS_ICP_OK, GS_ICP_TOO_FEW, GS_ICP_NOT_POSITIVE = 0, 1, 2


class GsIcpModelOpts(C.Structure):

    _fields_ = [("alpha_min", f32), ("edge_rel", f32), ("normal_step", i32)]


class GsIcpOpts(C.Structure):

    _fields_ = [("stride", i32), ("dist_max", f32), ("cos_min", f32), ("min_count", i32), ("damping", C.c_double)]


class GsIcpState(C.Structure):

    _fields_ = [("R", C.c_double * 9), ("t", C.c_double * 3), ("iteration", i32), ("reserved", i32)]


gs_icp_model_bytes = _sig("gs_icp_model_bytes", sz, i32, i32)
gs_icp_workspace_bytes = _sig("gs_icp_workspace_bytes", sz, i32, i32, i32)
gs_icp_log_bytes = _sig("gs_icp_log_bytes", sz, i32)
gs_icp_model_maps = _sig("gs_icp_model_maps", ci, vp, vp, C.POINTER(GsSeedCameraPP), C.POINTER(GsIcpModelOpts), vp, vp, vp)
gs_icp_reset = _sig("gs_icp_reset", ci, vp, vp, i32, C.POINTER(C.c_double), C.POINTER(C.c_double), vp)
gs_icp_step = _sig("gs_icp_step", ci, vp, C.POINTER(GsSeedCameraPP), vp, vp, C.POINTER(GsSeedCameraPP), C.POINTER(GsIcpOpts),
                   vp, vp, i32, i32, vp, sz, vp)

GS_POSE_LOG_HEAD = 24


class GsPoseState(C.Structure):

    _fields_ = [("R", C.c_double * 9), ("t", C.c_double * 3), ("m", C.c_double * 6), ("v", C.c_double * 6),
                ("best_R", C.c_double * 9), ("best_t", C.c_double * 3), ("best_loss", C.c_double),
                ("steps", i32), ("best_row", i32), ("skipped", i32), ("bad", i32)]


class GsPoseStepOpts(C.Structure):

    _fields_ = [("lr_rot", C.c_double), ("lr_tran", C.c_double), ("lr_scale", C.c_double), ("beta1", C.c_double),
                ("beta2", C.c_double), ("eps", C.c_double), ("track_best", i32), ("n_values", i32)]


gs_pose_log_bytes = _sig("gs_pose_log_bytes", sz, i32, i32)
gs_pose_reset = _sig("gs_pose_reset", ci, vp, vp, vp, i32, i32, C.POINTER(C.c_double), C.POINTER(C.c_double), vp)
gs_pose_step = _sig("gs_pose_step", ci, vp, vp, vp, vp, C.POINTER(GsPoseStepOpts), vp, vp, vp, i32, i32, vp)

EXPORTS = [
    "gs_last_error", "gs_abi_version", "gs_culling", "gs_world2camera", "gs_world2camera_backward",
    "gs_jacobian", "gs_global_culling", "gs_global_culling_backward", "gs_calc_tile_list",
    "gs_gather_gaussians", "gs_draw", "gs_draw_backward_workspace_bytes", "gs_draw_backward",
    "gs_sort_pairs_tmp_bytes", "gs_sort_pairs", "gs_sort_pairs_bits", "gs_frame_workspace_bytes",
    "gs_frame_aux_workspace_bytes", "gs_frame_pose_workspace_bytes", "gs_frame_forward",
    "gs_frame_stats_async", "gs_frame_longest_list_async", "gs_frame_stats_tagged_async", "gs_frame_cull_fallback_async", "gs_frame_is_occlusion_culled", "gs_frame_cull_second_pass", "gs_frame_debug_cut_table", "gs_frame_debug_views", "gs_frame_debug_rects", "gs_frame_debug_cull_stage", "gs_frame_binning_variant", "gs_frame_debug_tile_nproc", "gs_frame_debug_bwd_exec_rows", "gs_frame_backward", "gs_frame_backward_adam", "gs_frame_forward_profile",
    "gs_frame_backward_part", "gs_frame_async_create", "gs_frame_async_wait", "gs_frame_async_destroy",
    "gs_frame_backward_slice", "gs_frame_project_slices", "gs_frame_forward_project", "gs_frame_forward_rest",
    "gs_adam_step_multi",
    "gs_frame_backward_profile", "gs_adam_step", "gs_adam_step_range", "gs_adam_step_sharded", "gs_frame_overflow_flag", "gs_grad_stat_update", "gs_loss_workspace_bytes", "gs_loss_l1_ssim",
    "gs_loss_depth_workspace_bytes", "gs_loss_depth", "gs_frame_backward_adam_aux", "gs_frame_backward_adam_pose",
    "gs_frame_backward_pose",
    "gs_densify_workspace_bytes", "gs_densify_classify", "gs_densify_apply", "gs_densify_apply_state",
    "gs_seed_workspace_bytes", "gs_seed_classify", "gs_seed_apply",
    "gs_loss_track_workspace_bytes", "gs_loss_track",
    "gs_loss_track_gated_workspace_bytes", "gs_loss_track_gated",
    "gs_track_gate_mask_workspace_bytes", "gs_track_gate_mask", "gs_loss_l1_ssim_weighted",
    "gs_view_overlap_workspace_bytes", "gs_view_overlap_check_view", "gs_view_overlap",
    "gs_scene_pack_bytes", "gs_scene_pack_build", "gs_frame_reads_scene_pack",
    "gs_prune_workspace_bytes", "gs_prune_classify", "gs_prune_apply",
    "gs_seed_apply_pp", "gs_view_overlap_pp",
    "gs_frame_contrib_workspace_bytes", "gs_frame_contrib", "gs_prune_classify_contrib",
    "gs_pyramid_down",
    "gs_icp_model_bytes", "gs_icp_workspace_bytes", "gs_icp_log_bytes", "gs_icp_model_maps", "gs_icp_reset", "gs_icp_step",
    "gs_view_redundancy_workspace_bytes", "gs_view_redundancy", "gs_view_redundancy_pp",
    "gs_pose_log_bytes", "gs_pose_reset", "gs_pose_step",
]


def check(rc: int, what: str):
    if rc != 0:
        msg = gs_last_error()
        raise RuntimeError(f"{what} failed (code {rc}): {msg.decode() if msg else ''}")


def call(name: str, *args):
    check(globals()[name](*args), name)
```

3d-gaussian-splatting_amd/gs_frame.py:

```python
from __future__ import annotations

import copy
import ctypes as C
import os
import sys
import warnings
import weakref
from dataclasses import dataclass
from typing import Optional

import numpy as np
import torch

from gaussian import _lib
from gs_call import check_tensor, require_hip
from gs_geometry import RayBasis, TileGrid, pose_ctypes, principal_point_offset

SCALE_ACT = {"abs": 0, "exp": 1}
TILE_CULLING = {"dist": 0, "prob": 1, "prob2": 2}


@dataclass
class FrameStats:
    visible: int
# ... 566 lines not shown
            if self.auto_grow == "async" and self._async_event is None:
                _lib.check(_lib.gs_frame_stats_tagged_async(C.byref(f), self._frame_serial & 0xffffffff,
                                                            self._async_host.data_ptr(), stream),
                           "gs_frame_stats_tagged_async")
                self._async_event = torch.cuda.Event()
                self._async_event.record(self._stream())
                self._async_serial = self._frame_serial
            break
        return image, padded

    def _aux_outputs(self, f, training):
        g = self._grid
        depth = torch.empty(g.height, g.width, device=self.device, dtype=torch.float32)
        alpha = torch.empty(g.height, g.width, device=self.device, dtype=torch.float32)
        aux_padded = torch.empty(g.padded_height, g.padded_width, 2, device=self.device,
                                 dtype=torch.float32) if training else None
        f.depth, f.alpha = depth.data_ptr(), alpha.data_ptr()
        f.aux_padded = aux_padded.data_ptr() if aux_padded is not None else None
        f.grad_depth = f.grad_alpha = None
        return depth, alpha, aux_padded

    def forward_begin(self, pos, quat, scale, opa, rgb, camera, slice_begin: int, slice_end: int,
                      expect_per_slice: int = None) -> bool:
        with torch.cuda.device(self.device):
            stream = self._stream().cuda_stream
            if slice_begin == 0:
                self._begun = None
                cur = self._frame
                if (cur is None or not cur.training or self.auto_grow is True or not self._checked_once
                        or cur.max_pairs != self.max_pairs or cur.N != pos.shape[0]):
                    return False
                self._pack_cur = None
                self._repeat_drop()
                f = self._describe(pos, quat, scale, opa, rgb, camera, True)
                if f.workspace != cur.workspace:
                    return False
                n_sl, per = C.c_int32(), C.c_int64()
                g = self._grid
                image = torch.empty(g.height, g.width, 3, device=self.device, dtype=torch.float32)
                padded = torch.empty(g.padded_height, g.padded_width, 3, device=self.device, dtype=torch.float32)
                f.image, f.image_padded = image.data_ptr(), padded.data_ptr()
                _lib.check(_lib.gs_frame_project_slices(C.byref(f), C.byref(n_sl), C.byref(per)), "gs_frame_project_slices")
                if n_sl.value == 0:
                    return False
                if expect_per_slice is not None and int(expect_per_slice) != per.value:
                    import warnings

                    warnings.warn(f"forward_begin: the caller cut the Gaussian array into project slices of "
                                  f"{expect_per_slice}, the library's plan says {per.value}; rendering from scratch")
                    return False
                self._begun = {"f": f, "image": image, "padded": padded, "keep": (pos, quat, scale, opa, rgb),
                               "camera": camera, "slices": n_sl.value, "per_slice": per.value, "done": 0}
            b = getattr(self, "_begun", None)
            if b is None:
                return False
            if expect_per_slice is not None and int(expect_per_slice) != b["per_slice"]:
                self._begun = None
                return False
            slice_end = min(int(slice_end), b["slices"])
            if slice_end <= slice_begin:
                return True
            _lib.check(_lib.gs_frame_forward_project(C.byref(b["f"]), int(slice_begin), slice_end, stream),
                       "gs_frame_forward_project")
            b["done"] += slice_end - slice_begin
            return True

    def begun_frame_matches(self, pos, quat, scale, opa, rgb, camera) -> bool:
        b = getattr(self, "_begun", None)
        return (b is not None and b["done"] == b["slices"] and b["camera"] is camera
                and all(x is y for x, y in zip(b["keep"], (pos, quat, scale, opa, rgb))))

    def forward_abandon(self):
        self._begun = None

    def forward_finish(self):
        b = getattr(self, "_begun", None)
        if b is None or b["done"] != b["slices"]:
            raise RuntimeError("forward_finish() needs a frame whose project stage was issued completely")
        self._begun = None
        with torch.cuda.device(self.device):
            stream = self._stream().cuda_stream
            if self.auto_grow == "async":
                self._poll_async_counters()
            f = b["f"]
            rows = self.bwd_rows or (self.bwd_rows is None and self._bwd_rows_seen)
            f.flags = (f.flags & ~_lib.GS_FRAME_BWD_ROWS) | (_lib.GS_FRAME_BWD_ROWS if rows else 0)
            _lib.check(_lib.gs_frame_forward_rest(C.byref(f), stream), "gs_frame_forward_rest")
            self._repeat_drop()
            self._frame = f
            self._frame_serial += 1
            self._keep = (*b["keep"], b["image"], b["padded"])
            self._note_cut_table(f)
            if self.auto_grow == "async" and self._async_event is None:
                _lib.check(_lib.gs_frame_stats_tagged_async(C.byref(f), self._frame_serial & 0xffffffff,
                                                            self._async_host.data_ptr(), stream),
                           "gs_frame_stats_tagged_async")
                self._async_event = torch.cuda.Event()
                self._async_event.record(self._stream())
                self._async_serial = self._frame_serial
        return b["image"], b["padded"]

    def backward_slice(self, out, g_begin: int, g_end: int, part: int = None):
        f = self._training_frame("backward_slice")
        if part is None:
            part = _lib.GS_BWD_GEOMETRY | _lib.GS_BWD_COLOR
        with torch.cuda.device(self.device):
            _lib.check(_lib.gs_frame_backward_slice(C.byref(f), *(t.data_ptr() for t in out), int(part), int(g_begin),
                                                    int(g_end), self._stream().cuda_stream), "gs_frame_backward_slice")
        return out

    def _aux_grad_maps(self, f, grad_depth, grad_alpha):
        maps = []
        for name, t in (("grad_depth", grad_depth), ("grad_alpha", grad_alpha)):
            if t is not None:
                t = t.contiguous()
                if t.dtype != torch.float32 or tuple(t.shape) != (f.height, f.width):
                    raise RuntimeError(f"{name} must be float32 [H,W]")
            maps.append(t)
        grad_depth, grad_alpha = maps
        f.grad_depth = grad_depth.data_ptr() if grad_depth is not None else None
        f.grad_alpha = grad_alpha.data_ptr() if grad_alpha is not None else None
        return grad_depth, grad_alpha

    @staticmethod
    def _checked_grad_image(f, grad_image, none_ok: bool):
        if grad_image is None:
            if not none_ok:
                raise RuntimeError("grad_image may be None for frames rendered with aux=True only")
            return None
        grad_image = grad_image.contiguous()
        if grad_image.dtype != torch.float32 or tuple(grad_image.shape) != (f.height, f.width, 3):
            raise RuntimeError("grad_image must be float32 [H,W,3]")
        return grad_image

    def backward_adam(self, grad_image, adam, grad_depth=None, grad_alpha=None, grad_pose=None):
        f = self._training_frame("backward_adam")
        aux = bool(f.flags & _lib.GS_FRAME_AUX)
        if not aux and (grad_depth is not None or grad_alpha is not None):
            raise RuntimeError("grad_depth / grad_alpha need a preceding forward(..., aux=True)")
        for ptr, t in zip((f.pos, f.quat, f.scale, f.opa, f.rgb), self._keep[:5]):
            if int(ptr or 0) != t.data_ptr():
                raise RuntimeError("backward_adam(): the frame was rendered from tensors that are no longer alive")
        if aux:
            grad_depth, grad_alpha = self._aux_grad_maps(f, grad_depth, grad_alpha)
        grad_image = self._checked_grad_image(f, grad_image, none_ok=aux)
        if grad_pose is not None:
            f = self._pose_frame(f, grad_pose, 0)
        name = "gs_frame_backward_adam" + ("_pose" if grad_pose is not None else "_aux" if aux else "")
        with torch.cuda.device(self.device):
            _lib.call(name, C.byref(f), grad_image.data_ptr() if grad_image is not None else None, C.byref(adam),
                      self._stream().cuda_stream)
        torch.autograd.graph.increment_version(self._keep[:5])
        self._bwd_serial = self._frame_serial

    def backward(self, grad_image, out=None, part: int = 0, grad_depth=None, grad_alpha=None, grad_pose=None):
        f = self._training_frame("backward")
        pos, quat, scale, opa, rgb = self._keep[:5]
        if out is None:
            out = tuple(torch.empty_like(t) for t in (pos, quat, scale, opa, rgb))
        grad_image, grad_depth, grad_alpha = self._raster_inputs(f, part, grad_image, grad_depth, grad_alpha)
        for t, ref in zip(out, (pos, quat, scale, opa, rgb)):
            if t.shape != ref.shape or t.dtype != torch.float32 or not t.is_contiguous():
                raise RuntimeError("gradient destinations must match the parameters")
        if grad_pose is not None:
            f = self._pose_frame(f, grad_pose, part)
        with torch.cuda.device(self.device):
            if part == 0:
                _lib.check(_lib.gs_frame_backward(C.byref(f), grad_image.data_ptr(), *(t.data_ptr() for t in out),
                                                  self._stream().cuda_stream), "gs_frame_backward")
            else:
                _lib.check(_lib.gs_frame_backward_part(C.byref(f), grad_image.data_ptr() if grad_image is not None
                                                       else None, *(t.data_ptr() for t in out), int(part),
                                                       self._stream().cuda_stream), "gs_frame_backward_part")
        if part in (0, _lib.GS_BWD_RASTER):
            self._bwd_serial = self._frame_serial
        return out

    def backward_pose(self, grad_image, grad_pose, part: int = 0, grad_depth=None, grad_alpha=None, pose_dev=None):
        f = self._training_frame("backward_pose")
        if pose_dev is not None and pose_dev is not self._pose_dev_keep:
            raise RuntimeError("backward_pose(pose_dev=...) must be the tensor the frame's forward was given")
        grad_image, grad_depth, grad_alpha = self._raster_inputs(f, part, grad_image, grad_depth, grad_alpha)
        f = self._pose_frame(f, grad_pose, part)
        with torch.cuda.device(self.device):
            _lib.call("gs_frame_backward_pose", C.byref(f), grad_image.data_ptr() if grad_image is not None else None,
                      int(part), self._stream().cuda_stream)
        if part == 0:
            self._bwd_serial = self._frame_serial
        return grad_pose

    def _training_frame(self, who: str):
        f = self._frame
        if f is None or not f.training:
            raise RuntimeError(f"{who}() needs a preceding forward(training=True)")
        return f

    def _raster_inputs(self, f, part, grad_image, grad_depth, grad_alpha):
        aux = bool(f.flags & _lib.GS_FRAME_AUX)
        if not aux and (grad_depth is not None or grad_alpha is not None):
            raise RuntimeError("grad_depth / grad_alpha need a preceding forward(..., aux=True)")
        if part in (0, _lib.GS_BWD_RASTER):
            if aux:
                grad_depth, grad_alpha = self._aux_grad_maps(f, grad_depth, grad_alpha)
            grad_image = self._checked_grad_image(f, grad_image, none_ok=aux)
            if grad_image is None:
                grad_image = torch.zeros(f.height, f.width, 3, device=self.device, dtype=torch.float32)
        return grad_image, grad_depth, grad_alpha

    def _pose_frame(self, f, grad_pose, part):
        if part not in (0, _lib.GS_BWD_GEOMETRY):
            raise RuntimeError("grad_pose is written by backward(part=0) or backward(part=GS_BWD_GEOMETRY) only")
        if int(f.color_dim) != 3:
            raise RuntimeError("pose gradients need rgb colours: with SH colours the image also depends on the pose through "
                               "each pixel's ray direction, which the backward does not differentiate")
        grad_rot, grad_tran = grad_pose
        for name, t, shape in (("grad_rot", grad_rot, (3, 3)), ("grad_tran", grad_tran, (3,))):
            check_tensor(name, t, shape, device=self.device)
        need = _lib.gs_frame_pose_workspace_bytes(int(f.N))
        if self._pose_ws is None or self._pose_ws.numel() < need + 256:
            self._pose_ws = torch.empty(int(need) + 256, dtype=torch.uint8, device=self.device)
        g = _lib.GsFrameDP()
        C.memmove(C.byref(g), C.byref(f), C.sizeof(_lib.GsFrameDP))
        base = self._pose_ws.data_ptr()
        g.pose_workspace = (base + 255) // 256 * 256
        g.pose_workspace_bytes = self._pose_ws.numel() - (g.pose_workspace - base)
        g.grad_rot, g.grad_tran = grad_rot.data_ptr(), grad_tran.data_ptr()
        g.flags |= _lib.GS_FRAME_POSE_GRAD
        return g

    def profile_forward(self, pos, quat, scale, opa, rgb, camera, training: Optional[bool] = None, aux: bool = False):
        training = self.training if training is None else training
        self._begun = None
        with torch.cuda.device(self.device):
            self._scene_pack_step(pos, quat, scale, opa, rgb, training)
        f = self._describe(pos, quat, scale, opa, rgb, camera, training, aux)
        with torch.cuda.device(self.device):
            self._repeat_step(f, training, aux)
        g = self._grid
        image = torch.empty(g.height, g.width, 3, device=self.device, dtype=torch.float32)
        padded = torch.empty(g.padded_height, g.padded_width, 3, device=self.device,
                             dtype=torch.float32) if training else None
        f.image = image.data_ptr()
        f.image_padded = padded.data_ptr() if padded is not None else None
        self._aux_keep = self._aux_outputs(f, training) if aux else None
        ms = (C.c_float * 6)()
        with torch.cuda.device(self.device):
            _lib.call("gs_frame_forward_profile", C.byref(f), ms, self._stream().cuda_stream)
        self._frame = f
        self._frame_serial += 1
        self._note_cut_table(f)
        self._keep = (pos, quat, scale, opa, rgb, image, padded)
        return dict(zip(("project", "scan_emit", "sort", "ranges", "raster", "total"), (float(x) for x in ms)))

    def profile_backward(self, grad_image):
        f = self._frame
        if f is None or not f.training:
            raise RuntimeError("profile_backward() needs a preceding training forward")
        pos, quat, scale, opa, rgb = self._keep[:5]
        out = tuple(torch.empty_like(t) for t in (pos, quat, scale, opa, rgb))
        ms = (C.c_float * 3)()
        with torch.cuda.device(self.device):
            _lib.call("gs_frame_backward_profile", C.byref(f), grad_image.contiguous().data_ptr(),
                      *(t.data_ptr() for t in out), ms, self._stream().cuda_stream)
        self._bwd_serial = self._frame_serial
        return dict(zip(("raster_bwd", "project_bwd", "total"), (float(x) for x in ms)))

    def stats(self) -> FrameStats:
        if self._frame is None:
            raise RuntimeError("no frame rendered yet")
        stream = self._stream()
        tag = self._frame_serial & 0xffffffff
        _lib.call("gs_frame_stats_tagged_async", C.byref(self._frame), tag, self._stats_host.data_ptr(), stream.cuda_stream)
        stream.synchronize()
        h = self._stats_host.tolist()
        v, m, o, b, longest, ran_past, walk, xwalk = (int(h[k]) for k in (0, 1, 2, 3, 9, 10, 13, 14))
        assert (int(h[11]) & 0xffffffff) == tag, "gs_frame_stats_tagged_async: the tag did not come back"
        self._note_lists(longest, m, walk, xwalk)
        bwd_done = getattr(self, "_bwd_serial", -1) == self._frame_serial and int(self._frame.color_dim) == 3
        if bwd_done:
            self._note_buckets(b)
        culled = bool(self._frame.flags & _lib.GS_FRAME_OCCLUSION_CULL)
        flagged = culled and bool(self._frame.flags & _lib.GS_FRAME_CULL_REPEAT)
        if flagged and ran_past:
            self._broken_promise(self._frame_serial, self._repeat_epoch)
        return FrameStats(v, m, o, (b & 0xffffffff) if bwd_done else 0, longest, (b >> 32) if bwd_done else 0,
                          bool(ran_past) and culled and not flagged, bool(ran_past) and flagged)

    def binning_variant(self) -> str:
        if self._frame is None:
            raise RuntimeError("no frame rendered yet")
        v = _lib.gs_frame_binning_variant(C.byref(self._frame))
        if v < 0:
            raise RuntimeError(f"gs_frame_binning_variant failed (code {v})")
        return ("radix64", "radix_tile_bits", "table", "slice", "strip")[v]

    def overflow_flag(self) -> Optional[int]:
        if self._frame is None:
            return None
        ptr = C.c_void_p()
        _lib.call("gs_frame_overflow_flag", C.byref(self._frame), C.byref(ptr))
        return ptr.value

    def cut_table(self) -> torch.Tensor:
        f = self._frame
        if f is None:
            raise RuntimeError("no frame rendered yet")
        ptr, n = C.c_void_p(), C.c_int32()
        _lib.call("gs_frame_debug_cut_table", C.byref(f), C.byref(ptr), C.byref(n))
        off = ptr.value - self._ws.data_ptr()
        return self._ws[off:off + 4 * n.value].view(torch.int32)

    def _rects(self, allow_culled: bool = False) -> torch.Tensor:
        f = self._frame
        if f is None:
            raise RuntimeError("no frame rendered yet")
        culled = C.c_int32(0)
        _lib.call("gs_frame_is_occlusion_culled", C.byref(f), C.byref(culled))
        if culled.value and not allow_culled:
            raise RuntimeError("the rectangle records of an occlusion-culled frame cover its projected Gaussians only: "
                               "render with FrameRenderer(occlusion_cull=False) for debug_views()")
        ptr = C.c_void_p()
        _lib.call("gs_frame_debug_rects", C.byref(f), C.byref(ptr))
        off = ptr.value - self._ws.data_ptr()
        return self._ws[off:off + 16 * f.N].view(torch.int32).reshape(f.N, 4)

    def culling_mask(self) -> torch.Tensor:
        f = self._frame
        if f is None:
            raise RuntimeError("no frame rendered yet")
        culled = C.c_int32(0)
        _lib.call("gs_frame_is_occlusion_culled", C.byref(f), C.byref(culled))
        if culled.value:
            import gaussian
            pos, quat, scale = self._keep[:3]
            n = pos.shape[0]
            rot = torch.tensor(list(f.rot), dtype=torch.float32, device=self.device).reshape(3, 3)
            tran = torch.tensor(list(f.tran), dtype=torch.float32, device=self.device)
            mask = torch.zeros(n, dtype=torch.int64, device=self.device)
            pos_i = torch.empty_like(pos)
            pp = bool(f.flags & _lib.GS_FRAME_PRINCIPAL_POINT)
            half = (float("inf"), float("inf")) if pp else (float(f.half_width), float(f.half_height))
            with torch.cuda.device(self.device):
                gaussian.global_culling(pos, quat, scale, rot, tran, pos_i,
                                        torch.empty((n, 2, 2), dtype=torch.float32, device=self.device), mask,
                                        float(f.near_plane), *half)
            if pp:
                sx = float(np.float32(float(f.pp_dx) / float(f.focal_x))), float(np.float32(float(f.pp_dy) / float(f.focal_y)))
                inside = ((pos_i[:, 0] + sx[0]).abs() < float(f.half_width)) & ((pos_i[:, 1] + sx[1]).abs() < float(f.half_height))
                return (mask != 0) & inside
            return mask != 0
        return self._rects()[:, 2] != 0

    def composited_steps(self) -> int:
        f = self._frame
        if f is None or not f.training:
            raise RuntimeError("composited_steps() needs a preceding training forward")
        ptr = C.c_void_p()
        _lib.call("gs_frame_debug_tile_nproc", C.byref(f), C.byref(ptr))
        off = ptr.value - self._ws.data_ptr()
        T = self._grid.n_tiles
        return int(self._ws[off:off + 4 * T].view(torch.int32).to(torch.int64).sum().item())

    def contributions(self, w_min: float = CONTRIB_W_MIN, out: Optional[Contributions] = None,
                      accumulate: bool = False) -> Contributions:
        f = self._frame
        if f is None or not f.training:
            raise RuntimeError("contributions() needs a preceding training forward")
        n = int(f.N)
        if out is None:
            if accumulate:
                raise RuntimeError("contributions(accumulate=True) needs `out`")
            out = Contributions.empty(n, self.device, w_min)
        elif accumulate and float(out.w_min) != float(w_min):
            raise RuntimeError(f"contributions(accumulate=True): `out` was counted at w_min {out.w_min!r}, not {float(w_min)!r}")
        rows = out.rows
        check_tensor("contributions(): the rows of `out`", rows, (n, 4), device=self.device)
        need = int(_lib.gs_frame_contrib_workspace_bytes(int(f.max_pairs)))
        if self._contrib_ws is None or self._contrib_ws.numel() < need + 256:
            self._contrib_ws = torch.empty(need + 256, dtype=torch.uint8, device=self.device)
        base = (self._contrib_ws.data_ptr() + 255) // 256 * 256
        opts = _lib.GsContribOpts(float(w_min), 1 if accumulate else 0)
        with torch.cuda.device(self.device):
            _lib.call("gs_frame_contrib", C.byref(f), C.byref(opts), rows.data_ptr() or None, base, need,
                      self._stream().cuda_stream)
        out.w_min = float(w_min)
        return out

    def executed_row_steps(self) -> int:
        f = self._frame
        if f is None or not f.training:
            raise RuntimeError("executed_row_steps() needs a preceding training forward + backward")
        ptr, n = C.c_void_p(), C.c_int32()
        _lib.call("gs_frame_debug_bwd_exec_rows", C.byref(f), C.byref(ptr), C.byref(n))
        if n.value == 0:
            return 0
        off = ptr.value - self._ws.data_ptr()
        return int(self._ws[off:off + 4 * n.value].view(torch.int32).to(torch.int64).sum().item())

    def debug_views(self):
        f = self._frame
        ptrs = [C.c_void_p() for _ in range(7)]
        _lib.call("gs_frame_debug_views", C.byref(f), *[C.byref(p) for p in ptrs])
        st = self.stats()
        n, m, T = f.N, st.pairs, self._grid.n_tiles

        def view(ptr, nbytes, dtype, shape):
            off = ptr.value - self._ws.data_ptr()
            return self._ws[off:off + nbytes].view(dtype).reshape(shape)

        ids = view(ptrs[1], 4 * m, torch.int32, (m,))
        ranges = view(ptrs[2], 8 * T, torch.int32, (T, 2))
        if ptrs[0].value:
            keys = view(ptrs[0], 8 * m, torch.int64, (m,))
        else:
            counts = (ranges[:, 1] - ranges[:, 0]).to(torch.int64)
            tiles = torch.repeat_interleave(torch.arange(T, device=self.device, dtype=torch.int64), counts)
            depth = view(ptrs[3], 64 * n, torch.int32, (n, 16))[:, 2].to(torch.int64) & 0xffffffff
            keys = (tiles << 32) | depth[ids.to(torch.int64)]
        visible = self.culling_mask()
        raw = view(ptrs[3], 64 * n, torch.float32, (n, 16))
        rec = torch.where(visible.unsqueeze(1), raw, torch.zeros_like(raw))
        out = {
            "sorted_keys": keys,
            "sorted_ids": ids,
            "tile_ranges": ranges,
            "visible": visible,
            "rec_geom": rec[:, 0:4],
            "rec_cov": rec[:, 4:8],
            "tiles_touched": self._rects()[:, 3],
        }
        if f.color_dim == 3:
            out["rec_color"] = rec[:, 8:12]
        return out

    @staticmethod
    def _posed_camera(camera, pose, rgb):
        if pose is None:
            return camera, False
        rot, tran = pose
        if tuple(rot.shape) != (3, 3) or tuple(tran.shape) != (3,):
            raise RuntimeError("pose must be (rot [3,3], tran [3])")
        grad = torch.is_grad_enabled() and (rot.requires_grad or tran.requires_grad)
        if grad and (rgb.dim() != 2 or rgb.shape[1] != 3):
            raise RuntimeError("pose gradients need rgb colours ([N,3]): with SH colours the image also depends on the pose "
                               "through each pixel's ray direction, which the backward does not differentiate")
        cam = copy.copy(camera)
        cam.rot = rot.detach().to("cpu", torch.float32).numpy().astype(np.float32)
        cam.tran = tran.detach().to("cpu", torch.float32).numpy().astype(np.float32)
        return cam, grad

    def render(self, pos, quat, scale, opa, rgb, camera, pose=None):
        cam, pose_grad = self._posed_camera(camera, pose, rgb)
        if pose_grad:
            return _FrameFunction.apply(pos, quat, scale, opa, rgb, self, cam, pose[0], pose[1])
        if torch.is_grad_enabled() and any(t.requires_grad for t in (pos, quat, scale, opa, rgb)):
            return _FrameFunction.apply(pos, quat, scale, opa, rgb, self, cam)
        return self.forward(pos, quat, scale, opa, rgb, cam, training=False)[0]

    def render_aux(self, pos, quat, scale, opa, rgb, camera, pose=None):
        cam, pose_grad = self._posed_camera(camera, pose, rgb)
        if pose_grad:
            return _FrameAuxFunction.apply(pos, quat, scale, opa, rgb, self, cam, pose[0], pose[1])
        if torch.is_grad_enabled() and any(t.requires_grad for t in (pos, quat, scale, opa, rgb)):
            return _FrameAuxFunction.apply(pos, quat, scale, opa, rgb, self, cam)
        image, _, depth, alpha = self.forward(pos, quat, scale, opa, rgb, cam, training=False, aux=True)
        return image, depth, alpha


def _pose_grad_buffers(renderer):
    return (torch.empty(3, 3, device=renderer.device, dtype=torch.float32),
            torch.empty(3, device=renderer.device, dtype=torch.float32))


def _pose_grads_out(ctx, gp):
    if gp is None:
        return None, None
    return tuple(g.to(device=d, dtype=t) if need else None
                 for g, d, t, need in zip(gp, ctx.pose_devices, ctx.pose_dtypes, ctx.needs_input_grad[7:9]))


class _FrameFunction(torch.autograd.Function):
    @staticmethod
    def forward(ctx, pos, quat, scale, opa, rgb, renderer, camera, rot=None, tran=None):
        image, _ = renderer.forward(pos.detach(), quat.detach(), scale.detach(), opa.detach(), rgb.detach(), camera,
                                    training=True)
        ctx.renderer = renderer
        ctx.frame_serial = renderer._frame_serial
        ctx.has_pose = rot is not None
        if ctx.has_pose:
            ctx.pose_devices, ctx.pose_dtypes = (rot.device, tran.device), (rot.dtype, tran.dtype)
        return image

    @staticmethod
    def backward(ctx, grad_image):
        r = ctx.renderer
        if r._frame_serial != ctx.frame_serial:
            raise RuntimeError("FrameRenderer workspace was reused by another forward before backward()")
        gp = _pose_grad_buffers(r) if ctx.has_pose else None
        g = r.backward(grad_image, grad_pose=gp)
        if not ctx.has_pose:
            return (*g, None, None)
        return (*g, None, None, *_pose_grads_out(ctx, gp))


class _FrameAuxFunction(torch.autograd.Function):
    @staticmethod
    def forward(ctx, pos, quat, scale, opa, rgb, renderer, camera, rot=None, tran=None):
        image, _, depth, alpha = renderer.forward(pos.detach(), quat.detach(), scale.detach(), opa.detach(), rgb.detach(),
                                                  camera, training=True, aux=True)
        ctx.renderer = renderer
        ctx.frame_serial = renderer._frame_serial
        ctx.has_pose = rot is not None
        if ctx.has_pose:
            ctx.pose_devices, ctx.pose_dtypes = (rot.device, tran.device), (rot.dtype, tran.dtype)
        return image, depth, alpha

    @staticmethod
    def backward(ctx, grad_image, grad_depth, grad_alpha):
        r = ctx.renderer
        if r._frame_serial != ctx.frame_serial:
            raise RuntimeError("FrameRenderer workspace was reused by another forward before backward()")
        gp = _pose_grad_buffers(r) if ctx.has_pose else None
        g = r.backward(grad_image, grad_depth=grad_depth, grad_alpha=grad_alpha, grad_pose=gp)
        if not ctx.has_pose:
            return (*g, None, None)
        return (*g, None, None, *_pose_grads_out(ctx, gp))
```

include/gs_abi.h:

```cpp
#ifndef GS_ABI_H
#define GS_ABI_H

#include <stddef.h>
#include <stdint.h>

#ifdef __cplusplus
extern "C" {
#endif
#if defined(__GNUC__)
#pragma GCC visibility push(default)
#endif

#define GS_ABI_VERSION 8

#define GS_E_INVALID (-1)
#define GS_E_UNSUPPORTED (-2)
#define GS_E_CAPACITY (-3)

typedef void *gs_stream_t;

const char *gs_last_error(void);
int gs_abi_version(void);


int gs_culling(void);

int gs_world2camera(const float *pos, const float *rot, const float *tran, float *res, int64_t B,
                    gs_stream_t stream);

int gs_world2camera_backward(const float *grad_out, const float *rot, float *grad_inp, int64_t B,
                             gs_stream_t stream);

int gs_jacobian(const float *pos_cam, float *jac, int64_t B, gs_stream_t stream);

int gs_global_culling(const float *pos, const float *quat, const float *scale, const float *rot,
                      const float *tran, int64_t N, float near_plane, float half_width,
                      float half_height, float *res_pos, float *res_cov, int64_t *culling_mask,
                      gs_stream_t stream);

int gs_global_culling_backward(const float *pos, const float *quat, const float *scale,
                               const float *rot, const float *tran, int64_t N,
                               const float *gradout_pos, const float *gradout_cov,
                               const int64_t *culling_mask, float *gradinput_pos,
                               float *gradinput_quat, float *gradinput_scale, gs_stream_t stream);

int gs_calc_tile_list(const float *pos, const float *cov, int64_t n_point, const float *tile_top,
                      const float *tile_bottom, const float *tile_left, const float *tile_right,
                      int32_t *tile_n_point, int32_t *tile_gaussian_list,
                      int64_t max_points_per_tile, float thresh, int method, float tile_length_x,
                      float tile_length_y, int32_t n_tiles_x, int32_t n_tiles_y, float leftmost,
                      float topmost, gs_stream_t stream);

int gs_gather_gaussians(const int32_t *tile_n_point_accum, const int32_t *tile_gaussian_list,
                        int32_t *gathered_list, int32_t *tile_ids_for_points, int64_t n_tiles,
                        int64_t max_points_for_tile, int64_t list_row_size, gs_stream_t stream);

int gs_draw(const float *pos, const float *rgb, const float *opa, const float *cov,
            const int32_t *tile_n_point_accum, float *res, int32_t h, int32_t w, int64_t M,
            float focal_x, float focal_y, int weight_normalize, int sigmoid, int fast,
            const float *rays_o, const float *lefttop_pos, const float *vec_dx,
            const float *vec_dy, int use_sh_coeff, gs_stream_t stream);

size_t gs_draw_backward_workspace_bytes(int64_t M, int32_t h, int32_t w);
int gs_draw_backward(const float *pos, const float *rgb, const float *opa, const float *cov,
                     const int32_t *tile_n_point_accum, const float *output,
                     const float *grad_output, float *grad_pos, float *grad_rgb, float *grad_opa,
                     float *grad_cov, int32_t h, int32_t w, int64_t M, float focal_x,
                     float focal_y, int weight_normalize, int sigmoid, int fast,
                     const float *rays_o, const float *lefttop_pos, const float *vec_dx,
                     const float *vec_dy, int use_sh_coeff, void *workspace,
                     size_t workspace_bytes, gs_stream_t stream);


size_t gs_sort_pairs_tmp_bytes(int64_t capacity);
int gs_sort_pairs(uint64_t *keys0, uint32_t *vals0, uint64_t *keys1, uint32_t *vals1,
                  const uint32_t *d_count, int64_t capacity, int end_bit, void *tmp,
                  size_t tmp_bytes, int *sorted_in_buffer1, gs_stream_t stream);
int gs_sort_pairs_bits(uint64_t *keys0, uint32_t *vals0, uint64_t *keys1, uint32_t *vals1,
                       const uint32_t *d_count, int64_t capacity, int begin_bit, int end_bit,
                       void *tmp, size_t tmp_bytes, int *sorted_in_buffer1, gs_stream_t stream);

#define GS_FRAME_EMIT_SORTED_KEYS 1

#define GS_FRAME_SLICE_SORT 2

#define GS_FRAME_TABLE_BIN 4

#define GS_FRAME_SERIAL_LONG_LISTS 8

#define GS_FRAME_LONG_LISTS 16

#define GS_FRAME_STRIP_BIN 32
#define GS_FRAME_LONG_SORT 128
#define GS_FRAME_OCCLUSION_CULL 256
#define GS_FRAME_CULL_DILATE 512
#define GS_FRAME_CULL_DILATE_NEAR 1024
#define GS_FRAME_BWD_ROWS 64

#define GS_FRAME_AUX 2048

#define GS_FRAME_POSE_GRAD 4096

#define GS_FRAME_SCENE_PACK 8192

#define GS_FRAME_PRINCIPAL_POINT 16384

#define GS_FRAME_DEVICE_POSE 32768

#define GS_FRAME_CULL_REPEAT 65536

typedef struct gs_frame {
    int64_t N;
    int32_t color_dim;
    int32_t scale_activation;
    const float *pos;
    const float *quat;
    const float *scale;
    const float *opa;
    const float *rgb;
    float rot[9];
    float tran[3];
    float near_plane, half_width, half_height;
    int32_t width, height;
    float focal_x, focal_y;
    float tile_length_x, tile_length_y, leftmost, topmost;
    float thresh;
    float rays_o[3], lefttop[3], vec_dx[3], vec_dy[3];
    int64_t max_pairs;
    void *workspace;
    size_t workspace_bytes;
    float *image;
    float *image_padded;
    int32_t training;
    int32_t sort_mode;
    int32_t tile_culling_method;
    struct gs_frame_async *async;
    int32_t flags;
    float *depth, *alpha;
    float *aux_padded;
    void *aux_workspace;
    size_t aux_workspace_bytes;
    const float *grad_depth, *grad_alpha;
    float *grad_rot;
    float *grad_tran;
    void *pose_workspace;
    size_t pose_workspace_bytes;
} gs_frame;

typedef struct gs_frame_scene {
    gs_frame frame;
    const void *scene_pack_a;
    const void *scene_pack_b;
    size_t scene_pack_a_bytes, scene_pack_b_bytes;
} gs_frame_scene;

typedef struct gs_frame_pp {
    gs_frame_scene scene;
    double pp_dx, pp_dy;
} gs_frame_pp;

typedef struct gs_frame_dp {
    gs_frame_pp pp;
    const float *pose_dev;
} gs_frame_dp;

size_t gs_frame_workspace_bytes(int64_t N, int64_t max_pairs, int32_t width, int32_t height,
                                int32_t color_dim, int32_t training);

size_t gs_frame_aux_workspace_bytes(int64_t max_pairs, int32_t width, int32_t height, int32_t training);

size_t gs_frame_pose_workspace_bytes(int64_t N);

size_t gs_scene_pack_bytes(int64_t N, size_t *a_bytes, size_t *b_bytes);
int gs_scene_pack_build(const float *pos, const float *quat, const float *scale, const float *opa, const float *rgb, int64_t N,
                        int32_t color_dim, int32_t scale_activation, void *pack_a, void *pack_b, gs_stream_t stream);
int gs_frame_reads_scene_pack(const gs_frame *f);

int gs_frame_forward(const gs_frame *f, gs_stream_t stream);

typedef struct gs_frame_async gs_frame_async;
int gs_frame_async_create(gs_frame_async **out);
int gs_frame_async_wait(gs_frame_async *a, gs_stream_t stream);
int gs_frame_async_destroy(gs_frame_async *a);

#define GS_N_STAGES 6
int gs_frame_forward_profile(const gs_frame *f, float *stage_ms_host, gs_stream_t stream);
int gs_frame_backward_profile(const gs_frame *f, const float *grad_image, float *grad_pos,
                              float *grad_quat, float *grad_scale, float *grad_opa,
                              float *grad_rgb, float *stage_ms_host, gs_stream_t stream);

int gs_frame_stats_async(const gs_frame *f, int64_t *stats_host, gs_stream_t stream);

int gs_frame_longest_list_async(const gs_frame *f, int64_t *longest_host, gs_stream_t stream);

#define GS_STATS_TAGGED_N 15
int gs_frame_stats_tagged_async(const gs_frame *f, uint32_t tag, int64_t *stats_host, gs_stream_t stream);

int gs_frame_cull_fallback_async(const gs_frame *f, int64_t *ran_past_host, gs_stream_t stream);

int gs_frame_cull_second_pass(const gs_frame *f, int32_t *enqueued);

int gs_frame_is_occlusion_culled(const gs_frame *f, int32_t *culled);

int gs_frame_debug_views(const gs_frame *f, const uint64_t **sorted_keys,
                         const uint32_t **sorted_ids, const int32_t **tile_ranges,
                         const float **rec_geom, const float **rec_cov, const float **rec_color,
                         const uint32_t **tiles_touched);

int gs_frame_binning_variant(const gs_frame *f);

int gs_frame_debug_rects(const gs_frame *f, const uint32_t **rects);

int gs_frame_debug_cut_table(const gs_frame *f, const uint32_t **cut, int32_t *n_tiles);

int gs_frame_debug_cull_stage(const gs_frame *f, const uint64_t **entries, const uint32_t **tags,
                              const uint32_t **slice_entries, int32_t *slices, int64_t *cap);

int gs_frame_debug_tile_nproc(const gs_frame *f, const uint32_t **tile_nproc);

int gs_frame_debug_bwd_exec_rows(const gs_frame *f, const uint32_t **exec_rows, int32_t *n_slots);

int gs_frame_backward(const gs_frame *f, const float *grad_image, float *grad_pos,
                      float *grad_quat, float *grad_scale, float *grad_opa, float *grad_rgb,
                      gs_stream_t stream);

#define GS_BWD_RASTER 1
#define GS_BWD_GEOMETRY 2
#define GS_BWD_COLOR 4
int gs_frame_backward_part(const gs_frame *f, const float *grad_image, float *grad_pos, float *grad_quat,
                           float *grad_scale, float *grad_opa, float *grad_rgb, int32_t part, gs_stream_t stream);

int gs_frame_backward_slice(const gs_frame *f, float *grad_pos, float *grad_quat, float *grad_scale, float *grad_opa,
                            float *grad_rgb, int32_t part, int64_t g_begin, int64_t g_end, gs_stream_t stream);
int gs_frame_project_slices(const gs_frame *f, int32_t *slices, int64_t *per_slice);
int gs_frame_forward_project(const gs_frame *f, int32_t slice_begin, int32_t slice_end, gs_stream_t stream);
int gs_frame_forward_rest(const gs_frame *f, gs_stream_t stream);


int gs_adam_step(float *param, const float *grad, float *exp_avg, float *exp_avg_sq, int64_t n,
                 int32_t n_groups, const int64_t *group_end, const float *lr, float beta1, float beta2,
                 float eps, int64_t step, float *grad_stat, int64_t stat_begin, int64_t stat_end,
                 int32_t stat_mode, gs_stream_t stream);

int gs_adam_step_range(float *param, const float *grad, float *exp_avg, float *exp_avg_sq, int64_t n,
                       int64_t range_begin, int64_t range_end, int32_t n_groups, const int64_t *group_end,
                       const float *lr, float beta1, float beta2, float eps, int64_t step, float *grad_stat,
                       int64_t stat_begin, int64_t stat_end, int32_t stat_mode, gs_stream_t stream);

int gs_adam_step_sharded(float *param, const float *grad, float *exp_avg_shard, float *exp_avg_sq_shard, int64_t n,
                         int64_t range_begin, int64_t range_end, int64_t moment_base, int32_t n_groups,
                         const int64_t *group_end, const float *lr, float beta1, float beta2, float eps, int64_t step,
                         float *grad_stat, int64_t stat_begin, int64_t stat_end, int32_t stat_mode,
                         const void *skip_if_nonzero, gs_stream_t stream);

int gs_adam_step_multi(float *param, const float *grad, float *exp_avg, float *exp_avg_sq, int64_t n, int32_t n_ranges,
                       const int64_t *range_begin, const int64_t *range_end, const int64_t *moment_offset,
                       int32_t n_groups, const int64_t *group_end, const float *lr, float beta1, float beta2, float eps,
                       int64_t step, float *grad_stat, int64_t stat_begin, int64_t stat_end, int32_t stat_mode,
                       const void *skip_if_nonzero, float grad_scale, gs_stream_t stream);

typedef struct gs_adam_fused {
    float *exp_avg[5], *exp_avg_sq[5];
    float lr[5];
    float beta1, beta2, eps;
    int64_t step;
    float *grad_stat;
    int32_t stat_mode;
    const void *skip_if_nonzero;
} gs_adam_fused;
int gs_frame_backward_adam(const gs_frame *f, const float *grad_image, const gs_adam_fused *adam, gs_stream_t stream);

int gs_frame_backward_adam_aux(const gs_frame *f, const float *grad_image, const gs_adam_fused *adam, gs_stream_t stream);

int gs_frame_backward_adam_pose(const gs_frame *f, const float *grad_image, const gs_adam_fused *adam, gs_stream_t stream);

int gs_frame_backward_pose(const gs_frame *f, const float *grad_image, int32_t part, gs_stream_t stream);

int gs_frame_overflow_flag(const gs_frame *f, const void **device_counter);

int gs_grad_stat_update(const float *grad, float *stat, int64_t n, int32_t stat_mode, gs_stream_t stream);

size_t gs_loss_workspace_bytes(int32_t H, int32_t W);
int gs_loss_l1_ssim(const float *pred, const float *target, int32_t H, int32_t W, float ssim_weight,
                    float *grad, float *loss_out, void *workspace, size_t workspace_bytes,
                    gs_stream_t stream);

int gs_loss_l1_ssim_weighted(const float *pred, const float *target, const float *weight, int32_t H, int32_t W,
                             float ssim_weight, double weight_sum, double weight_sum_interior, float *grad, float *loss_out,
                             void *workspace, size_t workspace_bytes, gs_stream_t stream);

size_t gs_loss_depth_workspace_bytes(int32_t H, int32_t W);
int gs_loss_depth(const float *depth, const float *alpha, const float *target, int32_t H, int32_t W, int32_t mode,
                  float alpha_min, float scale, float *grad_depth, float *grad_alpha, float *loss_out, void *workspace,
                  size_t workspace_bytes, gs_stream_t stream);

size_t gs_loss_track_workspace_bytes(int32_t H, int32_t W);
int gs_loss_track(const float *image, const float *depth, const float *alpha, const float *target_image,
                  const float *target_range, int32_t H, int32_t W, float alpha_min, float color_weight, float depth_weight,
                  float depth_gate, float scale, float *grad_image, float *grad_depth, float *grad_alpha, float *values_out,
                  void *workspace, size_t workspace_bytes, gs_stream_t stream);

size_t gs_loss_track_gated_workspace_bytes(int32_t H, int32_t W);
int gs_loss_track_gated(const float *image, const float *depth, const float *alpha, const float *target_image,
                        const float *target_range, int32_t H, int32_t W, float alpha_min, float color_weight,
                        float depth_weight, float depth_gate_k, float color_gate_k, float depth_gate_floor,
                        float color_gate_floor, int32_t couple, float scale, float *grad_image, float *grad_depth,
                        float *grad_alpha, float *values_out, float *resid_depth, float *resid_color, void *workspace,
                        size_t workspace_bytes, gs_stream_t stream);

size_t gs_track_gate_mask_workspace_bytes(int32_t H, int32_t W);
int gs_track_gate_mask(const float *image, const float *depth, const float *alpha, const float *target_image,
                       const float *target_range, int32_t H, int32_t W, float alpha_min, float depth_gate_k,
                       float color_gate_k, float depth_gate_floor, float color_gate_floor, int32_t couple, float *range_out,
                       float *weight_out, float *values_out, float *resid_depth, float *resid_color, void *workspace,
                       size_t workspace_bytes, gs_stream_t stream);

#define GS_PYRAMID_MAX_LEVELS 4
typedef struct gs_pyramid_opts {
    int32_t min_valid;
    float edge_rel;
} gs_pyramid_opts;
int gs_pyramid_down(const float *image, const float *range, int32_t H, int32_t W, const gs_pyramid_opts *opts,
                    float *image_out, float *range_out, gs_stream_t stream);

typedef struct gs_densify_opts {
    float taus;
    float delete_thresh;
    float grad_thresh;
    float clone_dt;
    int32_t scale_activation;
    int32_t grad_aggregation;
    int32_t use_clone, use_split;
    int32_t color_dim;
} gs_densify_opts;
size_t gs_densify_workspace_bytes(int64_t N);
int gs_densify_classify(const float *scale, const float *opa, const float *grad, int64_t N,
                        const gs_densify_opts *opts, int64_t *counts_dev, void *workspace,
                        size_t workspace_bytes, gs_stream_t stream);
int gs_densify_apply(const float *pos, const float *quat, const float *scale, const float *opa,
                     const float *rgb, const float *grad, int64_t N, const gs_densify_opts *opts,
                     const float *eps1, const float *eps2, int64_t n_eps, float *out_pos, float *out_quat,
                     float *out_scale, float *out_opa, float *out_rgb, int64_t capacity,
                     const int64_t *counts_dev, void *workspace, size_t workspace_bytes, gs_stream_t stream);

typedef struct gs_seed_opts {
    int32_t stride;
    float alpha_thresh;
    float front_rel;
    float scale_factor;
    float opa_init;
    int32_t scale_activation;
    int32_t color_dim;
} gs_seed_opts;
typedef struct gs_seed_camera {
    float rot[9], tran[3];
    float focal_x, focal_y;
    int32_t width, height;
} gs_seed_camera;
size_t gs_seed_workspace_bytes(int32_t H, int32_t W);
int gs_seed_classify(const float *range, const float *depth, const float *alpha, int32_t H, int32_t W,
                     const gs_seed_opts *opts, int64_t *counts_dev, void *workspace, size_t workspace_bytes,
                     gs_stream_t stream);
int gs_seed_apply(const float *image, const float *range, const gs_seed_camera *cam, const gs_seed_opts *opts, float *pos,
                  float *quat, float *scale, float *opa, float *rgb, int64_t offset, int64_t capacity,
                  const int64_t *counts_dev, const void *workspace, size_t workspace_bytes, gs_stream_t stream);

typedef struct gs_seed_camera_pp {
    gs_seed_camera cam;
    float pp_dx, pp_dy;
} gs_seed_camera_pp;
int gs_seed_apply_pp(const float *image, const float *range, const gs_seed_camera_pp *cam, const gs_seed_opts *opts, float *pos,
                     float *quat, float *scale, float *opa, float *rgb, int64_t offset, int64_t capacity,
                     const int64_t *counts_dev, const void *workspace, size_t workspace_bytes, gs_stream_t stream);

#define GS_OVERLAP_MAX_VIEWS 256
typedef struct gs_overlap_opts {
    int32_t stride;
    float   near;
    int32_t border;
} gs_overlap_opts;
size_t gs_view_overlap_workspace_bytes(int32_t H, int32_t W, int32_t stride, int32_t n_views);
int gs_view_overlap_check_view(const gs_seed_camera *view, int32_t border);
int gs_view_overlap(const float *range, const gs_seed_camera *cam,
                    const gs_seed_camera *views_dev, int32_t n_views,
                    const gs_overlap_opts *opts, int64_t *counts_dev,
                    void *workspace, size_t workspace_bytes, gs_stream_t stream);
int gs_view_overlap_pp(const float *range, const gs_seed_camera_pp *cam, const gs_seed_camera *views_dev,
                       const float *view_pp_dev, int32_t n_views, const gs_overlap_opts *opts, int64_t *counts_dev,
                       void *workspace, size_t workspace_bytes, gs_stream_t stream);

#define GS_REDUNDANCY_BINS 8
size_t gs_view_redundancy_workspace_bytes(int32_t H, int32_t W, int32_t stride);
int gs_view_redundancy(const float *range, const gs_seed_camera *cam,
                       const gs_seed_camera *views_dev, int32_t n_views,
                       int32_t self_index,
                       const gs_overlap_opts *opts, int64_t *hist_dev,
                       void *workspace, size_t workspace_bytes, gs_stream_t stream);
int gs_view_redundancy_pp(const float *range, const gs_seed_camera_pp *cam, const gs_seed_camera *views_dev,
                          const float *view_pp_dev, int32_t n_views, int32_t self_index, const gs_overlap_opts *opts,
                          int64_t *hist_dev, void *workspace, size_t workspace_bytes, gs_stream_t stream);

#define GS_PRUNE_MAX_ARRAYS 16
typedef struct gs_prune_opts {
    float opa_logit_min;
    float scale_max;
    int32_t scale_activation;
} gs_prune_opts;
typedef struct gs_prune_arrays {
    int32_t n;
    int32_t width[GS_PRUNE_MAX_ARRAYS];
    const float *src[GS_PRUNE_MAX_ARRAYS];
    float *dst[GS_PRUNE_MAX_ARRAYS];
} gs_prune_arrays;
size_t gs_prune_workspace_bytes(int64_t N);
int gs_prune_classify(const float *scale, const float *opa, int64_t N, const gs_prune_opts *opts, int64_t *counts_dev,
                      void *workspace, size_t workspace_bytes, gs_stream_t stream);
int gs_prune_apply(const gs_prune_arrays *arrays, int64_t N, int64_t dst_offset, int64_t capacity,
                   const int64_t *counts_dev, const void *workspace, size_t workspace_bytes, gs_stream_t stream);

int gs_densify_apply_state(const gs_prune_arrays *arrays, int64_t N, int64_t capacity, const int64_t *counts_dev,
                           const void *workspace, size_t workspace_bytes, gs_stream_t stream);

typedef struct gs_contrib_row { float weight_sum, weight_max; uint32_t pixels, views; } gs_contrib_row;
typedef struct gs_contrib_opts { float w_min; int32_t accumulate; } gs_contrib_opts;
size_t gs_frame_contrib_workspace_bytes(int64_t max_pairs);
int gs_frame_contrib(const gs_frame *f, const gs_contrib_opts *opts, gs_contrib_row *rows ,
                     void *workspace, size_t workspace_bytes, gs_stream_t stream);

typedef struct gs_prune_contrib_opts { float weight_max_min; uint32_t pixels_min, views_min; } gs_prune_contrib_opts;
int gs_prune_classify_contrib(const float *scale, const float *opa, const gs_contrib_row *rows, int64_t N,
                              const gs_prune_opts *opts, const gs_prune_contrib_opts *copts, int64_t *counts_dev,
                              void *workspace, size_t workspace_bytes, gs_stream_t stream);

#define GS_ICP_LOG_DOUBLES 40
#define GS_ICP_OK 0
#define GS_ICP_TOO_FEW 1
#define GS_ICP_NOT_POSITIVE 2
typedef struct gs_icp_model_opts {
    float alpha_min;
    float edge_rel;
    int32_t normal_step;
} gs_icp_model_opts;
typedef struct gs_icp_opts {
    int32_t stride;
    float dist_max;
    float cos_min;
    int32_t min_count;
    double damping;
} gs_icp_opts;
typedef struct gs_icp_state {
    double R[9], t[3];
    int32_t iteration;
    int32_t reserved;
} gs_icp_state;
size_t gs_icp_model_bytes(int32_t H, int32_t W);
size_t gs_icp_workspace_bytes(int32_t H, int32_t W, int32_t stride);
size_t gs_icp_log_bytes(int32_t rows);
int gs_icp_model_maps(const float *depth, const float *alpha, const gs_seed_camera_pp *cam, const gs_icp_model_opts *opts,
                      float *vertex, float *normal, gs_stream_t stream);
int gs_icp_reset(gs_icp_state *state_dev, double *log_dev, int32_t log_rows, const double *rot ,
                 const double *tran , gs_stream_t stream);
int gs_icp_step(const float *range, const gs_seed_camera_pp *cam,
                const float *vertex, const float *normal, const gs_seed_camera_pp *model_cam,
                const gs_icp_opts *opts, gs_icp_state *state_dev, double *log_dev, int32_t log_rows, int32_t log_row,
                void *workspace, size_t workspace_bytes, gs_stream_t stream);

#define GS_POSE_LOG_HEAD 24
typedef struct gs_pose_state {
    double R[9], t[3];
    double m[6], v[6];
    double best_R[9], best_t[3], best_loss;
    int32_t steps;
    int32_t best_row;
    int32_t skipped;
    int32_t bad;
} gs_pose_state;
typedef struct gs_pose_step_opts {
    double lr_rot, lr_tran, lr_scale, beta1, beta2, eps;
    int32_t track_best;
    int32_t n_values;
} gs_pose_step_opts;
size_t gs_pose_log_bytes(int32_t rows, int32_t n_values);
int gs_pose_reset(gs_pose_state *state_dev, float *pose_dev, float *log_dev, int32_t log_rows, int32_t n_values,
                  const double *rot , const double *tran , gs_stream_t stream);
int gs_pose_step(const float *grad_rot_dev, const float *grad_tran_dev, const float *values_dev,
                 const void *skip_if_nonzero, const gs_pose_step_opts *opts, gs_pose_state *state_dev, float *pose_dev,
                 float *log_dev, int32_t log_rows, int32_t log_row, gs_stream_t stream);

#if defined(__GNUC__)
#pragma GCC visibility pop
#endif
#ifdef __cplusplus
}
#endif
#endif
```

Before: 4704 frames/s.

## Compact surviving pixels into half the lanes once few remain live in a tile

In the RGB inference forward kernel, once a tile has at most 128 pixels with nonzero transmittance and enough splats remain, the wave writes out the finished pixels and packs the live ones through LDS so each lane holds two live pixels instead of four. Compositing then continues with half the per-lane work, using a restructured transmittance update (fma plus live mask) and a two-group loop. The aim is to stop spending ALU on saturated pixels in long tile lists. In exchange it adds LDS shuffles, wave barriers, vote refreshes for legacy chunks, extra register pressure and more code in the hot loop. Debug accessors for the compaction step and tile cost are also added.

```diff
diff --git a/3d-gaussian-splatting_amd/csrc/gs_frame.hip b/3d-gaussian-splatting_amd/csrc/gs_frame.hip
--- a/3d-gaussian-splatting_amd/csrc/gs_frame.hip
+++ b/3d-gaussian-splatting_amd/csrc/gs_frame.hip
@@ -785,6 +785,29 @@
     return 0;
 }
 
+extern "C" int gs_frame_debug_tile_compact(const gs_frame *f, const uint32_t **at, int32_t *n_tiles) {
+    int rc = validate(f);
+    if (rc) return rc;
+    GS_CHECK_ARG(at && n_tiles, "null pointer");
+    GS_CHECK_ARG(!f->training && f->color_dim == 3 && !(f->flags & GS_FRAME_AUX),
+                 "the compact phase belongs to rgb inference frames without the depth / alpha maps");
+    gs_frame_ws ws = gs_frame_carve(f->workspace, f->N, f->max_pairs, f->width, f->height, f->color_dim, f->training);
+    *at = ws.tile_compact;
+    *n_tiles = gs_frame_geometry(f).n_tiles;
+    return 0;
+}
+
+extern "C" int gs_frame_debug_tile_cost(const gs_frame *f, const uint32_t **cost, int32_t *n_tiles) {
+    int rc = validate(f);
+    if (rc) return rc;
+    GS_CHECK_ARG(cost && n_tiles, "null pointer");
+    GS_CHECK_ARG(effective_sort_mode(f) == 2 && gs_frame_uses_strips(f), "the tile costs are recorded by frames of the strip variant");
+    gs_frame_ws ws = gs_frame_carve(f->workspace, f->N, f->max_pairs, f->width, f->height, f->color_dim, f->training);
+    *cost = ws.tile_cost;
+    *n_tiles = gs_frame_geometry(f).n_tiles;
+    return 0;
+}
+
 extern "C" int gs_frame_debug_views(const gs_frame *f, const uint64_t **sorted_keys, const uint32_t **sorted_ids,
                                     const int32_t **tile_ranges, const float **rec_geom, const float **rec_cov,
                                     const float **rec_color, const uint32_t **tiles_touched) {
diff --git a/3d-gaussian-splatting_amd/csrc/gs_frame_layout.h b/3d-gaussian-splatting_amd/csrc/gs_frame_layout.h
--- a/3d-gaussian-splatting_amd/csrc/gs_frame_layout.h
+++ b/3d-gaussian-splatting_amd/csrc/gs_frame_layout.h
@@ -221,6 +221,7 @@
     uint32_t *big_tiles;
     uint32_t *tile_cost;
     uint32_t *tile_order;
+    uint32_t *tile_compact;
     uint4 *group_queue;
     float4 *cont_state;
     uint32_t *cont_flag;
@@ -340,6 +341,7 @@
         ws.mfma_n_items = nullptr;
         ws.stop_keys = nullptr;
     }
+    ws.tile_compact = (uint32_t *)take(sizeof(uint32_t) * G.n_tiles);
     ws.total_bytes = off;
     return ws;
 }
diff --git a/3d-gaussian-splatting_amd/csrc/raster_fwd.hip b/3d-gaussian-splatting_amd/csrc/raster_fwd.hip
--- a/3d-gaussian-splatting_amd/csrc/raster_fwd.hip
+++ b/3d-gaussian-splatting_amd/csrc/raster_fwd.hip
@@ -49,6 +49,9 @@
 #ifndef GS_FWD_RGB_WPE
 #define GS_FWD_RGB_WPE 4
 #endif
+#ifndef GS_FWD_COMPACT_MIN
+#define GS_FWD_COMPACT_MIN 16
+#endif
 #ifndef GS_FWD_SH27_WPE
 #define GS_FWD_SH27_WPE 3
 #endif
@@ -62,7 +65,7 @@
     float2 *ckpt;
 };
 
-template <int CDIM, bool FRAME, bool CKPT, bool SIG, bool WN, bool EXACT, bool AUX>
+template <int CDIM, bool FRAME, bool CKPT, bool SIG, bool WN, bool EXACT, bool AUX, bool COMPACT = false>
 __device__ __forceinline__ void raster_forward_body(RasterSrc S, RasterGeom G,
                                                     const int32_t *__restrict__ ranges,
                                                     float *__restrict__ out_padded,
@@ -77,7 +80,10 @@
                                                     const uint32_t *cut_in, uint32_t *cut_out,
                                                     unsigned long long *__restrict__ ranpast,
                                                     const unsigned long long *__restrict__ gate,
-                                                    const AuxFwdOut &X) {
+                                                    const AuxFwdOut &X, uint32_t compact_min = 0,
+                                                    uint32_t *__restrict__ tile_compact = nullptr) {
+    static_assert(!COMPACT || (CDIM == 3 && FRAME && !CKPT && !SIG && !WN && !EXACT && !AUX),
+                  "the compact phase belongs to the rgb inference frame");
     static_assert(!AUX || (FRAME && !SIG && !WN && !EXACT), "depth / alpha maps belong to the frame path");
     static_assert(!(EXACT && FRAME), "the exact-exp flavour belongs to the reference API (gs_draw, fast = 0)");
     if (FRAME && gate && *gate == 0) return;
@@ -94,6 +100,9 @@
     constexpr uint32_t LIVE_EVERY = CDIM == 3 ? GS_FWD_LIVE_EVERY : 4;
     __shared__ SM sm;
     __shared__ float s_dep[AUX ? SM::NBUF : 1][AUX ? CH : 1] __attribute__((aligned(16)));
+    enum { KT, KR, KG, KB, KX, KY, KI, KFIELD };
+    constexpr int KCAP = 128;
+    __shared__ float s_cmp[COMPACT ? KFIELD : 1][COMPACT ? KCAP : 1] __attribute__((aligned(16)));
     const int lane = threadIdx.x;
 
     auto range_of = [&](uint32_t t, uint32_t &s0, uint32_t &cnt) {
@@ -170,6 +179,55 @@
     asm volatile("" : "+v"(live_scale), "+v"(live_bias));
     uint32_t nproc = 0, steps = 0;
 
+    auto write_pixel = [&](uint32_t id_xp, uint32_t id_y, float c0, float c1, float c2, float aw) {
+        if (!WN || aw < 0.01f) aw = 1.0f;
+        const float o0 = c0 / aw, o1 = c1 / aw, o2 = c2 / aw;
+        if (out_padded) {
+            float *o = out_padded + ((size_t)id_y * G.padW + id_xp) * 3;
+            o[0] = o0;
+            o[1] = o1;
+            o[2] = o2;
+        }
+        if (out_image) {
+            const int ox = (int)id_xp - G.crop_left, oy = (int)id_y - G.crop_top;
+            if (ox >= 0 && ox < G.width && oy >= 0 && oy < G.height) {
+                float *o = out_image + ((size_t)oy * G.width + ox) * 3;
+                o[0] = o0 > 1.f ? 1.f : (o0 < 0.f ? 0.f : o0);
+                o[1] = o1 > 1.f ? 1.f : (o1 < 0.f ? 0.f : o1);
+                o[2] = o2 > 1.f ? 1.f : (o2 < 0.f ? 0.f : o2);
+            }
+        }
+    };
+
+    bool compacted = false, seen_legacy = false;
+    uint32_t compact_at = 0xffffffffu;
+    f2 &vote = T[1], &px2 = cg[1], &py2c = cb[1];
+    auto cidx = [&]() { return __float_as_uint(cr[1].x); };
+    auto refresh_vote = [&]() {
+        if constexpr (COMPACT) {
+            uint32_t l = lane;
+            asm volatile("" : "+v"(l));
+            __builtin_amdgcn_fence(__ATOMIC_ACQ_REL, "wavefront");
+            __builtin_amdgcn_wave_barrier();
+            s_cmp[KT][l] = 0.f;
+            __builtin_amdgcn_fence(__ATOMIC_ACQ_REL, "wavefront");
+            __builtin_amdgcn_wave_barrier();
+            if (T[0].x != T[0].x) s_cmp[KT][cidx() & 63u] = 1.f;
+            if (T[0].y != T[0].y) s_cmp[KT][(cidx() >> 16) & 63u] = 1.f;
+            __builtin_amdgcn_fence(__ATOMIC_ACQ_REL, "wavefront");
+            __builtin_amdgcn_wave_barrier();
+            vote.x = 1.0f - s_cmp[KT][cidx() & 63u];
+            vote.y = 1.0f - s_cmp[KT][(cidx() >> 16) & 63u];
+            __builtin_amdgcn_fence(__ATOMIC_ACQ_REL, "wavefront");
+            __builtin_amdgcn_wave_barrier();
+        }
+    };
+    auto compact_live = [&](bool refresh) {
+        if (refresh) refresh_vote();
+        const f2 s = T[0] * vote;
+        return __ballot(__builtin_fmaxf(s.x, s.y) > 0.0f) != 0ull;
+    };
+
     auto write_ckpt = [&](uint32_t idx_in_tile) {
         float4 *c = ckpt + raster_ckpt_slot(start, tile, idx_in_tile / GS_BUCKET) * 256;
 #pragma unroll
@@ -191,6 +249,48 @@
 #pragma unroll
         for (int h = 1; h < NPP; ++h) sum += T[h];
         return __ballot(sum.x + sum.y > 0.0f) != 0ull;
+    };
+    auto hand_over = [&](const unsigned long long (&m)[4]) {
+        if constexpr (COMPACT) {
+            uint32_t first = 0;
+            uint32_t x_here = id_x, y_here = id_y0, l = lane;
+            asm volatile("" : "+v"(x_here), "+v"(y_here), "+v"(l));
+#pragma unroll
+            for (int q = 0; q < 4; ++q) {
+                const int h = q >> 1;
+                const bool e = q & 1;
+                const float t = e ? T[h].y : T[h].x, c0 = e ? cr[h].y : cr[h].x, c1 = e ? cg[h].y : cg[h].x,
+                            c2 = e ? cb[h].y : cb[h].x;
+                const uint32_t slot = first + __builtin_amdgcn_mbcnt_hi((uint32_t)(m[q] >> 32),
+                                                                        __builtin_amdgcn_mbcnt_lo((uint32_t)m[q], 0u));
+                if (t != 0.f) {
+                    s_cmp[KT][slot] = t;
+                    s_cmp[KR][slot] = c0;
+                    s_cmp[KG][slot] = c1;
+                    s_cmp[KB][slot] = c2;
+                    s_cmp[KX][slot] = px;
+                    s_cmp[KY][slot] = e ? py2[h].y : py2[h].x;
+                    s_cmp[KI][slot] = __uint_as_float(64u * q + l);
+                } else {
+                    write_pixel(x_here, y_here + 4 * q, c0, c1, c2, 1.0f);
+                }
+                first += (uint32_t)__popcll(m[q]);
+            }
+            __builtin_amdgcn_fence(__ATOMIC_ACQ_REL, "wavefront");
+            __builtin_amdgcn_wave_barrier();
+            const uint32_t live = first;
+            const bool a = l < live, b = l + 64u < live;
+            T[0] = f2{a ? s_cmp[KT][l] : 0.f, b ? s_cmp[KT][l + 64] : 0.f};
+            cr[0] = f2{a ? s_cmp[KR][l] : 0.f, b ? s_cmp[KR][l + 64] : 0.f};
+            cg[0] = f2{a ? s_cmp[KG][l] : 0.f, b ? s_cmp[KG][l + 64] : 0.f};
+            cb[0] = f2{a ? s_cmp[KB][l] : 0.f, b ? s_cmp[KB][l + 64] : 0.f};
+            px2 = f2{a ? s_cmp[KX][l] : 0.f, b ? s_cmp[KX][l + 64] : 0.f};
+            py2c = f2{a ? s_cmp[KY][l] : 0.f, b ? s_cmp[KY][l + 64] : 0.f};
+            cr[1] = f2{__uint_as_float((a ? __float_as_uint(s_cmp[KI][l]) : 0xffffu) |
+                                       ((b ? __float_as_uint(s_cmp[KI][l + 64]) : 0xffffu) << 16)), 0.f};
+            vote = f2{1.f, 1.f};
+            if (seen_legacy) refresh_vote();
+        }
     };
 
     bool done = false, staged_next = false;
@@ -199,10 +299,12 @@
         if (FRAME && cont_flag && base == (uint32_t)GS_LONG_MIN) {
             if (any_live()) {
                 float4 *c = cont_state + (size_t)tile * 256;
+                uint32_t l = lane;
+                if constexpr (COMPACT) asm volatile("" : "+v"(l));
 #pragma unroll
                 for (int h = 0; h < NPP; ++h) {
-                    c[128 * h + lane] = make_float4(T[h].x, cr[h].x, cg[h].x, cb[h].x);
-                    c[128 * h + 64 + lane] = make_float4(T[h].y, cr[h].y, cg[h].y, cb[h].y);
+                    c[128 * h + l] = make_float4(T[h].x, cr[h].x, cg[h].x, cb[h].x);
+                    c[128 * h + 64 + l] = make_float4(T[h].y, cr[h].y, cg[h].y, cb[h].y);
                 }
                 continues = true;
             }
@@ -281,12 +383,26 @@
         auto composite_chunk = [&](auto legacy_tag) {
         constexpr bool LEGACY = decltype(legacy_tag)::value;
         uint32_t stop = cnt;
+        uint32_t i = 0;
+        bool hand = false;
+        if (!COMPACT || !compacted) {
 #pragma unroll 1
-        for (uint32_t i = 0; i < cnt; i += GROUP) {
-            if ((i & (LIVE_EVERY - 1)) == 0 && !any_live()) {
-                done = true;
-                stop = i;
-                break;
+        for (; i < cnt; i += GROUP) {
+            if ((i & (LIVE_EVERY - 1)) == 0) {
+                if (!any_live()) {
+                    done = true;
+                    stop = i;
+                    break;
+                }
+                if constexpr (COMPACT) {
+                    if (compact_min && n - (base + i) >= compact_min &&
+                        __popcll(__ballot(T[0].x != 0.f)) + __popcll(__ballot(T[0].y != 0.f)) + __popcll(__ballot(T[1].x != 0.f)) +
+                                __popcll(__ballot(T[1].y != 0.f)) <= KCAP) {
+                        compacted = hand = true;
+                        compact_at = base + i;
+                        break;
+                    }
+                }
             }
             {
             constexpr uint32_t i4 = 0;
@@ -322,6 +438,9 @@
                 G4 = ld4(SM::G);
                 L4 = ld4(SM::BL);
             }
+            f2 fp[NPP], fm[NPP];
+#pragma unroll
+            for (int h = 0; h < NPP; ++h) fp[h] = fm[h] = T[h];
 #pragma unroll
             for (int u = 0; u < (int)GROUP; ++u) {
                 const float gx = X.v[u], gy = Y.v[u], cA = A4.v[u], cB = B4.v[u], cC = C4.v[u], nlop = O4.v[u];
@@ -354,7 +473,14 @@
                         al.y = gs_squash_alpha(al.y);
                     }
                     f2 w;
-                    if constexpr (LEGACY && FRAME && CDIM == 3) {
+                    if constexpr (COMPACT) {
+                        const f2 Tn = u == 0 ? T[h] : fp[h] * fm[h];
+                        if constexpr (LEGACY) {
+                            al.x = Tn.x == 0.f ? 0.f : al.x;
+                            al.y = Tn.y == 0.f ? 0.f : al.y;
+                        }
+                        w = Tn * al;
+                    } else if constexpr (LEGACY && FRAME && CDIM == 3) {
                         al.x = T[h].x == 0.f ? 0.f : al.x;
                         al.y = T[h].y == 0.f ? 0.f : al.y;
                         w = al * T[h];
@@ -388,20 +514,84 @@
                         asm("" : "+v"(wr));
                         ca[h] += wr;
                     }
-                    const f2 t = T[h] - w;
-                    T[h] = t * live_mask(t, live_scale, live_bias);
+                    if constexpr (COMPACT) {
+                        const f2 Tn = u == 0 ? T[h] : fp[h] * fm[h];
+                        const f2 t = u == 0 ? pk_fma(-Tn, al, Tn) : u == 1 ? pk_fma(fp[h], fm[h], -w) : pk_fma(fm[h], fp[h], -w);
+                        fp[h] = t;
+                        fm[h] = live_mask(t, live_scale, live_bias);
+                        if (u == (int)GROUP - 1) T[h] = fp[h] * fm[h];
+                    } else {
+                        const f2 t = T[h] - w;
+                        T[h] = t * live_mask(t, live_scale, live_bias);
+                    }
                 }
             }
+            }
+        }
+        }
+        if constexpr (COMPACT) {
+            if (hand) {
+                asm volatile("" : "+v"(T[0]), "+v"(T[1]));
+                const unsigned long long m[4] = {__ballot(T[0].x != 0.f), __ballot(T[0].y != 0.f), __ballot(T[1].x != 0.f),
+                                                 __ballot(T[1].y != 0.f)};
+                hand_over(m);
+            }
+            if (compacted && !done) {
+                static_assert(GROUP == 4 && LIVE_EVERY == 8, "the compact loop walks two groups of four per liveness test");
+                if (!LEGACY && seen_legacy && i == 0) refresh_vote();
+#pragma unroll 1
+                for (; i < cnt; i += 2 * GROUP) {
+                    if (!compact_live(LEGACY)) {
+                        done = true;
+                        stop = i;
+                        break;
+                    }
+#pragma unroll
+                    for (uint32_t i4 = 0; i4 < 2 * GROUP; i4 += GROUP) {
+                        if (i4 && i + i4 >= cnt) break;
+                        __builtin_amdgcn_sched_barrier(0);
+                        auto ld4 = [&](int q) { return *(const float4 *)__builtin_assume_aligned(&sm.f[buf][q][i + i4], 16); };
+                        const float4 X = ld4(SM::X), Y = ld4(SM::Y), A4 = ld4(SM::A), B4 = ld4(SM::B), C4 = ld4(SM::C);
+                        const float4 O4 = ld4(SM::NLOP), R4 = ld4(SM::R), G4 = ld4(SM::G), L4 = ld4(SM::BL);
+                        auto at = [](const float4 &v, int u) { return u == 0 ? v.x : u == 1 ? v.y : u == 2 ? v.z : v.w; };
+                        f2 tp = T[0], mk = T[0];
+#pragma unroll
+                        for (int u = 0; u < (int)GROUP; ++u) {
+                            const float gx = at(X, u), gy = at(Y, u), cA = at(A4, u), cB = at(B4, u), cC = at(C4, u),
+                                        nlop = at(O4, u);
+                            const f2 dx = px2 - splat(gx);
+                            const f2 bdx = splat(cB) * dx;
+                            const f2 f = pk_fma(splat(cA) * dx, dx, splat(nlop));
+                            const f2 dy = py2c - splat(gy);
+                            const f2 q = pk_fma(pk_fma(splat(cC), dy, -bdx), dy, f);
+                            f2 al = {gs_exp2(-q.x), gs_exp2(-q.y)};
+                            const f2 Tn = u == 0 ? T[0] : tp * mk;
+                            if constexpr (LEGACY) {
+                                al.x = Tn.x == 0.f ? 0.f : al.x;
+                                al.y = Tn.y == 0.f ? 0.f : al.y;
+                            }
+                            const f2 w = Tn * al;
+                            const f2 t = u == 0 ? pk_fma(-Tn, al, Tn) : u == 1 ? pk_fma(tp, mk, -w) : pk_fma(mk, tp, -w);
+                            cr[0] = pk_fma(splat(at(R4, u)), w, cr[0]);
+                            cg[0] = pk_fma(splat(at(G4, u)), w, cg[0]);
+                            cb[0] = pk_fma(splat(at(L4, u)), w, cb[0]);
+                            tp = t;
+                            mk = live_mask(t, live_scale, live_bias);
+                        }
+                        T[0] = tp * mk;
+                    }
+                }
             }
         }
         return stop;
         };
+        if constexpr (COMPACT) seen_legacy = seen_legacy || chunk_legacy;
         steps = base + (chunk_legacy ? composite_chunk(std::true_type{}) : composite_chunk(std::false_type{}));
         nproc = base + cnt;
     }
     if (!staged_next) fetch(nstart, nn, 0);
     if (FRAME && !CKPT && cut_out) {
-        const bool sat = !continues && steps > 0 && (done || !any_live());
+        const bool sat = !continues && steps > 0 && (done || !((COMPACT && compacted) ? compact_live(seen_legacy) : any_live()));
         if (lane == 0) {
             uint32_t c = GS_NO_CUT, dlast = GS_NO_CUT;
             if (sat) {
@@ -412,7 +602,9 @@
             }
             if (cut_in) {
                 const uint32_t ci = cut_in[tile];
-                if (ci != GS_NO_CUT && dlast > ci) *ranpast = 1ull;
+                unsigned long long one = 1ull;
+                if constexpr (COMPACT) asm volatile("" : "+v"(one));
+                if (ci != GS_NO_CUT && dlast > ci) *ranpast = one;
             }
             cut_out[tile] = c;
         }
@@ -424,16 +616,24 @@
         if (steps > (uint32_t)GS_LONGEST_MIN) atomicMax(ranpast + (GS_CNT_MAXWALK - GS_CNT_RANPAST), (unsigned long long)steps);
     }
     if (FRAME && cont_flag && lane == 0) cont_flag[tile] = continues ? 1u : 0u;
-
+    if constexpr (COMPACT) {
+        if (lane == 0) tile_compact[tile] = compact_at;
+    }
+
+    if (COMPACT && compacted) {
+#pragma unroll
+        for (int e = 0; e < 2; ++e) {
+            const uint32_t p = (cidx() >> (16 * e)) & 0xffffu;
+            if (p != 0xffffu)
+                write_pixel(tx * 16 + (p & 15u), ty * 16 + ((p >> 4) & 3u) + 4 * (p >> 6), e ? cr[0].y : cr[0].x,
+                            e ? cg[0].y : cg[0].x, e ? cb[0].y : cb[0].x, 1.0f);
+        }
+    } else {
 #pragma unroll
     for (int h = 0; h < NPP; ++h)
 #pragma unroll
         for (int e = 0; e < 2; ++e) {
             const uint32_t id_y = id_y0 + 8 * h + 4 * e;
-            float aw = e ? accw[h].y : accw[h].x;
-            if (!WN || aw < 0.01f) aw = 1.0f;
-            const float o0 = (e ? cr[h].y : cr[h].x) / aw, o1 = (e ? cg[h].y : cg[h].x) / aw,
-                        o2 = (e ? cb[h].y : cb[h].x) / aw;
             if constexpr (AUX) {
                 const float dv = e ? cd[h].y : cd[h].x, av = e ? ca[h].y : ca[h].x;
                 if (X.padded) X.padded[(size_t)id_y * G.padW + id_x] = make_float2(dv, av);
@@ -443,22 +643,10 @@
                     if (X.alpha) X.alpha[(size_t)oy * G.width + ox] = av;
                 }
             }
-            if (out_padded) {
-                float *o = out_padded + ((size_t)id_y * G.padW + id_x) * 3;
-                o[0] = o0;
-                o[1] = o1;
-                o[2] = o2;
-            }
-            if (out_image) {
-                const int ox = (int)id_x - G.crop_left, oy = (int)id_y - G.crop_top;
-                if (ox >= 0 && ox < G.width && oy >= 0 && oy < G.height) {
-                    float *o = out_image + ((size_t)oy * G.width + ox) * 3;
-                    o[0] = o0 > 1.f ? 1.f : (o0 < 0.f ? 0.f : o0);
-                    o[1] = o1 > 1.f ? 1.f : (o1 < 0.f ? 0.f : o1);
-                    o[2] = o2 > 1.f ? 1.f : (o2 < 0.f ? 0.f : o2);
-                }
-            }
-        }
+            write_pixel(id_x, id_y, e ? cr[h].y : cr[h].x, e ? cg[h].y : cg[h].x, e ? cb[h].y : cb[h].x,
+                        e ? accw[h].y : accw[h].x);
+        }
+    }
     }
 }
 
@@ -471,10 +659,13 @@
                       uint32_t n_tiles, float4 *__restrict__ cont_state, uint32_t *__restrict__ cont_flag,
                       const uint32_t *__restrict__ tile_order, uint32_t *__restrict__ tile_cost, const uint32_t *cut_in,
                       uint32_t *cut_out, unsigned long long *__restrict__ ranpast,
-                      const unsigned long long *__restrict__ gate) {
-    raster_forward_body<CDIM, FRAME, CKPT, SIG, WN, EXACT, false>(S, G, ranges, out_padded, out_image, ckpt, tile_nproc,
-                                                                  n_tiles, cont_state, cont_flag, tile_order, tile_cost,
-                                                                  cut_in, cut_out, ranpast, gate, AuxFwdOut{});
+                      const unsigned long long *__restrict__ gate, uint32_t compact_min,
+                      uint32_t *__restrict__ tile_compact) {
+    constexpr bool COMPACT = CDIM == 3 && FRAME && !CKPT && !SIG && !WN && !EXACT;
+    raster_forward_body<CDIM, FRAME, CKPT, SIG, WN, EXACT, false, COMPACT>(S, G, ranges, out_padded, out_image, ckpt,
+                                                                           tile_nproc, n_tiles, cont_state, cont_flag,
+                                                                           tile_order, tile_cost, cut_in, cut_out, ranpast,
+                                                                           gate, AuxFwdOut{}, compact_min, tile_compact);
 }
 
 #ifndef GS_FWD_AUX_RGB_WPE
@@ -800,18 +991,18 @@
                 float4 *ckpt, uint32_t *tile_nproc, int wn, hipStream_t stream, float4 *cont_state = nullptr,
                 uint32_t *cont_flag = nullptr, const uint32_t *tile_order = nullptr, uint32_t *tile_cost = nullptr,
                 const uint32_t *cut_in = nullptr, uint32_t *cut_out = nullptr, unsigned long long *ranpast = nullptr,
-                const unsigned long long *gate = nullptr) {
+                const unsigned long long *gate = nullptr, uint32_t compact_min = 0, uint32_t *tile_compact = nullptr) {
     if (!fwd_plan().order) tile_order = nullptr;
     const uint32_t T = (uint32_t)(G.ntx * G.nty);
     const uint32_t grid = gate ? (T < 1024u ? T : 1024u) : fwd_grid(T);
     if (wn)
         hipLaunchKernelGGL((raster_forward_kernel<CDIM, FRAME, CKPT, SIG, true, EXACT>), dim3(grid), dim3(FWD_THREADS),
                            0, stream, S, G, ranges, out_padded, out_image, ckpt, tile_nproc, T, cont_state, cont_flag,
-                           tile_order, tile_cost, cut_in, cut_out, ranpast, gate);
+                           tile_order, tile_cost, cut_in, cut_out, ranpast, gate, compact_min, tile_compact);
     else
         hipLaunchKernelGGL((raster_forward_kernel<CDIM, FRAME, CKPT, SIG, false, EXACT>), dim3(grid), dim3(FWD_THREADS),
                            0, stream, S, G, ranges, out_padded, out_image, ckpt, tile_nproc, T, cont_state, cont_flag,
-                           tile_order, tile_cost, cut_in, cut_out, ranpast, gate);
+                           tile_order, tile_cost, cut_in, cut_out, ranpast, gate, compact_min, tile_compact);
 }
 
 }
@@ -919,6 +1110,10 @@
     const uint32_t *cut_in = culled && !second_pass ? gs_frame_cut_table(f, ws) : nullptr;
     unsigned long long *ranpast = ws.counters + GS_CNT_RANPAST;
     const unsigned long long *gate = second_pass ? ranpast : nullptr;
+    uint32_t compact_min = GS_FWD_COMPACT_MIN;
+    if (const char *e = getenv("GS_FWD_COMPACT")) {
+        if (e[0] == '0' && e[1] == 0) compact_min = 0;
+    }
     if (aux) {
         if (!fwd_plan().order) order = nullptr;
         const uint32_t T = (uint32_t)FG.n_tiles;
@@ -944,7 +1139,8 @@
                                                   stream, cs, cf, order, cost, nullptr, nullptr, ranpast, nullptr);
             else
                 launch_fwd<CD, true, false, false>(S, G, ws.tile_ranges, f->image_padded, f->image, nullptr, nullptr, 0, stream,
-                                                   cs, cf, order, cost, cut_in, ws.cut, ranpast, gate);
+                                                   cs, cf, order, cost, cut_in, ws.cut, ranpast, gate, dense ? 0u : compact_min,
+                                                   ws.tile_compact);
         });
     }
     GS_CHECK_LAUNCH();
diff --git a/3d-gaussian-splatting_amd/gaussian/_lib.py b/3d-gaussian-splatting_amd/gaussian/_lib.py
--- a/3d-gaussian-splatting_amd/gaussian/_lib.py
+++ b/3d-gaussian-splatting_amd/gaussian/_lib.py
@@ -122,6 +122,8 @@
 gs_frame_is_occlusion_culled = _sig("gs_frame_is_occlusion_culled", ci, C.POINTER(GsFrame), C.POINTER(C.c_int32))
 gs_frame_cull_second_pass = _sig("gs_frame_cull_second_pass", ci, C.POINTER(GsFrame), C.POINTER(C.c_int32))
 gs_frame_debug_cut_table = _sig("gs_frame_debug_cut_table", ci, C.POINTER(GsFrame), C.POINTER(vp), C.POINTER(C.c_int32))
+gs_frame_debug_tile_compact = _sig("gs_frame_debug_tile_compact", ci, C.POINTER(GsFrame), C.POINTER(vp), C.POINTER(C.c_int32))
+gs_frame_debug_tile_cost = _sig("gs_frame_debug_tile_cost", ci, C.POINTER(GsFrame), C.POINTER(vp), C.POINTER(C.c_int32))
 GS_STATS_TAGGED_N = 15
 gs_frame_debug_views = _sig("gs_frame_debug_views", ci, C.POINTER(GsFrame), C.POINTER(vp), C.POINTER(vp),
                             C.POINTER(vp), C.POINTER(vp), C.POINTER(vp), C.POINTER(vp), C.POINTER(vp))
@@ -329,7 +331,7 @@
     "gs_gather_gaussians", "gs_draw", "gs_draw_backward_workspace_bytes", "gs_draw_backward",
     "gs_sort_pairs_tmp_bytes", "gs_sort_pairs", "gs_sort_pairs_bits", "gs_frame_workspace_bytes",
     "gs_frame_aux_workspace_bytes", "gs_frame_pose_workspace_bytes", "gs_frame_forward",
-    "gs_frame_stats_async", "gs_frame_longest_list_async", "gs_frame_stats_tagged_async", "gs_frame_cull_fallback_async", "gs_frame_is_occlusion_culled", "gs_frame_cull_second_pass", "gs_frame_debug_cut_table", "gs_frame_debug_views", "gs_frame_debug_rects", "gs_frame_debug_cull_stage", "gs_frame_binning_variant", "gs_frame_debug_tile_nproc", "gs_frame_debug_bwd_exec_rows", "gs_frame_backward", "gs_frame_backward_adam", "gs_frame_forward_profile",
+    "gs_frame_stats_async", "gs_frame_longest_list_async", "gs_frame_stats_tagged_async", "gs_frame_cull_fallback_async", "gs_frame_is_occlusion_culled", "gs_frame_cull_second_pass", "gs_frame_debug_cut_table", "gs_frame_debug_tile_compact", "gs_frame_debug_tile_cost", "gs_frame_debug_views", "gs_frame_debug_rects", "gs_frame_debug_cull_stage", "gs_frame_binning_variant", "gs_frame_debug_tile_nproc", "gs_frame_debug_bwd_exec_rows", "gs_frame_backward", "gs_frame_backward_adam", "gs_frame_forward_profile",
     "gs_frame_backward_part", "gs_frame_async_create", "gs_frame_async_wait", "gs_frame_async_destroy",
     "gs_frame_backward_slice", "gs_frame_project_slices", "gs_frame_forward_project", "gs_frame_forward_rest",
     "gs_adam_step_multi",
diff --git a/3d-gaussian-splatting_amd/gs_frame.py b/3d-gaussian-splatting_amd/gs_frame.py
--- a/3d-gaussian-splatting_amd/gs_frame.py
+++ b/3d-gaussian-splatting_amd/gs_frame.py
@@ -892,13 +892,22 @@
         return ptr.value
 
     def cut_table(self) -> torch.Tensor:
+        return self._tile_words("gs_frame_debug_cut_table")
+
+    def _tile_words(self, entry: str) -> torch.Tensor:
         f = self._frame
         if f is None:
             raise RuntimeError("no frame rendered yet")
         ptr, n = C.c_void_p(), C.c_int32()
-        _lib.call("gs_frame_debug_cut_table", C.byref(f), C.byref(ptr), C.byref(n))
+        _lib.call(entry, C.byref(f), C.byref(ptr), C.byref(n))
         off = ptr.value - self._ws.data_ptr()
         return self._ws[off:off + 4 * n.value].view(torch.int32)
+
+    def tile_compact_steps(self) -> torch.Tensor:
+        return self._tile_words("gs_frame_debug_tile_compact")
+
+    def tile_cost(self) -> torch.Tensor:
+        return self._tile_words("gs_frame_debug_tile_cost")
 
     def _rects(self, allow_culled: bool = False) -> torch.Tensor:
         f = self._frame
diff --git a/include/gs_abi.h b/include/gs_abi.h
--- a/include/gs_abi.h
+++ b/include/gs_abi.h
@@ -213,6 +213,10 @@
 
 int gs_frame_debug_cut_table(const gs_frame *f, const uint32_t **cut, int32_t *n_tiles);
 
+int gs_frame_debug_tile_compact(const gs_frame *f, const uint32_t **at, int32_t *n_tiles);
+
+int gs_frame_debug_tile_cost(const gs_frame *f, const uint32_t **cost, int32_t *n_tiles);
+
 int gs_frame_debug_cull_stage(const gs_frame *f, const uint64_t **entries, const uint32_t **tags,
                               const uint32_t **slice_entries, int32_t *slices, int64_t *cap);
 
```

After: 4797 frames/s, median of 6. 1.02x the previous value.
